# kpreid/all-is-cubes

Hardware: AMD Instinct MI355X
Metric: Mrays/s (higher is better)
Workload: dtype f64

## Files before the change

### all_is_cubes_amd/abi.py

```python
from __future__ import annotations

import ctypes as C
import math
from pathlib import Path
from typing import Optional

import numpy as np

_PKG = Path(__file__).resolve().parent
LIB_PATH = _PKG / "libaic_hip.so"

AIC_OK = 0
ERR_NAMES = {1: "AIC_ERR_INVALID", 2: "AIC_ERR_NO_DEVICE", 3: "AIC_ERR_OOM", 4: "AIC_ERR_DEVICE", 5: "AIC_ERR_UNSUPPORTED"}
LAYER_WORLD, LAYER_UI = 0, 1
MAX_IN_FLIGHT = 32
FLAW_UNSUPPORTED, FLAW_NO_BLOOM = 1, 2
FRAME_COUNTERS, FRAME_AUX, FRAME_PIXEL_CENTERS, FRAME_OUT_LINEAR, FRAME_OUT_COLORBUF, FRAME_NO_FEEDBACK = 1, 2, 4, 8, 16, 32
FRAME_BLOOM = 64
RAYS_NO_SKY, RAYS_DEVICE = 128, 256
MAX_RAYS = 2048 * 65535
TUNE_QUEUES_SHIFT, TUNE_SUPER_SHIFT, TUNE_VARIANT_SHIFT = 0, 4, 9
VARIANT_AUTO, VARIANT_PLAIN, VARIANT_EXCHANGING, VARIANT_RECORDING = 0, 1, 2, 3
LIGHT_HOOK_SESSION, LIGHT_HOOK_POOL_SHIFT = 1, 8


def bloom_geometry(width: int, height: int):
    rx, ry = (width + 1) // 2, (height + 1) // 2
    levels = min(6, min(rx, ry).bit_length())
    d = 1 << levels
    return levels, ((rx + d - 1) // d * d, (ry + d - 1) // d * d)


def tuning(queues=None, super_shift=None, variant=None) -> int:
    t = 0
    if queues is not None:
        t |= (int(queues) & 15) << TUNE_QUEUES_SHIFT
    if super_shift is not None:
        t |= ((int(super_shift) + 1) & 31) << TUNE_SUPER_SHIFT
    if variant is not None:
        t |= (int(variant) & 3) << TUNE_VARIANT_SHIFT
    return t

ABI_SYMBOLS = [
    "aic_abi_version", "aic_create", "aic_destroy", "aic_last_error", "aic_device_name", "aic_upload_space",
    "aic_clear_space", "aic_update_cubes", "aic_update_light_volume", "aic_replace_block", "aic_replace_blocks", "aic_compact", "aic_set_options",
    "aic_render", "aic_render_submit", "aic_render_wait", "aic_render_submit_batch", "aic_render_wait_batch", "aic_trace_patches", "aic_trace_rays", "aic_partition_rows", "aic_assemble_strips", "aic_assemble_strips_async", "aic_assemble_strips_on", "aic_read_aux", "aic_synchronize", "aic_stream", "aic_wait_event", "aic_stream_wait_frame",
    "aic_probe_raycast", "aic_probe_light_lut", "aic_probe_powf", "aic_probe_expf", "aic_probe_bloom",
    "aic_ortho_image_size", "aic_render_orthographic",
    "aic_evaluate_light", "aic_evaluate_light_submit", "aic_evaluate_light_wait", "aic_evaluate_light_poll", "aic_light_cubes_changed", "aic_read_light_volume", "aic_read_light_cubes", "aic_light_chart", "aic_probe_derived", "aic_probe_log2f",
    "aic_create_multi", "aic_destroy_multi", "aic_multi_device_count", "aic_multi_context", "aic_multi_last_error", "aic_multi_upload_space",
    "aic_multi_clear_space", "aic_multi_update_cubes", "aic_multi_update_light_volume", "aic_multi_evaluate_light", "aic_multi_light_cubes_changed", "aic_multi_replace_blocks", "aic_multi_set_options",
    "aic_multi_render", "aic_multi_render_submit", "aic_multi_render_wait",
]


class AicError(RuntimeError):

    def __init__(self, code: int, message: str):
        super().__init__(f"{ERR_NAMES.get(code, code)}: {message}")
        self.code = code


class BlockDesc(C.Structure):
    _fields_ = [("resolution", C.c_int32), ("vlo", C.c_int32 * 3), ("vsize", C.c_int32 * 3), ("vox_off", C.c_uint32),
                ("pal_off", C.c_uint32), ("pal_len", C.c_uint32), ("flags", C.c_uint32), ("reserved", C.c_int32)]


class LightParams(C.Structure):
    _fields_ = [("maximum_distance", C.c_int32), ("fast", C.c_int32), ("epsilon", C.c_int32), ("batch", C.c_int32),
                ("queue_order", C.c_int32), ("n_queue", C.c_int32), ("lanes_per_cube", C.c_int32), ("hooks", C.c_int32), ("queue_cubes", C.c_void_p), ("queue_priorities", C.c_void_p),
                ("max_updates", C.c_uint64)]


class LightInfo(C.Structure):
    _fields_ = [("updates", C.c_uint64), ("batches", C.c_uint64), ("cost", C.c_uint64), ("device_ms", C.c_double),
                ("total_ms", C.c_double), ("queue_left", C.c_uint32), ("pad", C.c_uint32), ("bundles_visited", C.c_uint64)]


def light_chart():
    lib = load()
    lib.aic_light_chart.restype = C.c_uint32
    lib.aic_light_chart.argtypes = [C.c_void_p, C.c_void_p, C.POINTER(C.c_uint32)]
    depth = C.c_uint32(0)
    n = lib.aic_light_chart(None, None, C.byref(depth))
    w = np.zeros((n, 6), np.float32)
    ch = np.zeros((n, 6), np.uint32)
    lib.aic_light_chart(w.ctypes.data, ch.ctypes.data, C.byref(depth))
    return w, ch, int(depth.value)


class SpaceDesc(C.Structure):
    _fields_ = [("lo", C.c_int32 * 3), ("size", C.c_int32 * 3), ("block_index", C.c_void_p), ("light", C.c_void_p),
                ("n_blocks", C.c_uint32), ("blocks", C.c_void_p), ("voxels", C.c_void_p), ("n_voxels", C.c_uint64),
                ("palette", C.c_void_p), ("n_palette", C.c_uint64), ("sky_kind", C.c_int32), ("sky", (C.c_float * 3) * 8),
                ("block_sky", (C.c_uint8 * 4) * 7)]


class Options(C.Structure):
    _fields_ = [("fog", C.c_int32), ("transparency", C.c_int32), ("threshold", C.c_float), ("lighting", C.c_int32),
                ("bounce_samples", C.c_int32), ("antialiasing", C.c_int32), ("debug_pixel_cost", C.c_int32),
                ("tone_mapping", C.c_int32), ("maximum_intensity", C.c_float), ("bloom_intensity", C.c_float),
                ("view_distance", C.c_double)]


class Camera(C.Structure):
    _fields_ = [("inverse_projection_view", C.c_double * 16), ("exposure", C.c_float), ("reserved", C.c_int32)]


class Partition(C.Structure):
    _fields_ = [("strip_rows", C.c_uint32), ("n_parts", C.c_uint32), ("part", C.c_uint32), ("reserved", C.c_uint32)]


class FrameDesc(C.Structure):
    _fields_ = [("width", C.c_uint32), ("height", C.c_uint32), ("world", Camera), ("ui", Camera), ("backdrop", C.c_float * 4),
                ("partition", Partition), ("flags", C.c_uint32), ("tuning", C.c_uint32)]


class FrameInfo(C.Structure):
    _fields_ = [("cubes_traced", C.c_uint64), ("n_outer", C.c_uint64), ("n_inner", C.c_uint64), ("n_hits", C.c_uint64),
                ("n_light", C.c_uint64), ("kernel_ms", C.c_float), ("total_ms", C.c_float), ("rows_rendered", C.c_uint32),
                ("flaws", C.c_uint32), ("variant", C.c_uint32), ("tile_queues", C.c_uint32)]


PIXEL_AUX_DTYPE = np.dtype(
    [("hit", "<i4"), ("cube", "<i4", (3,)), ("voxel", "<i4", (3,)), ("resolution", "<i4"), ("face", "<i4"),
     ("block_index", "<i4"), ("cubes_traced", "<u4"), ("layer", "<u4"), ("t_distance", "<f8")],
    align=True,
)
RC_STEP_DTYPE = np.dtype([("cube", "<i4", (3,)), ("face", "<i4"), ("t_distance", "<f8"), ("intersection_point", "<f8", (3,))], align=True)

_lib: Optional[C.CDLL] = None


def load() -> C.CDLL:
    global _lib
    if _lib is None:
        if not LIB_PATH.exists():
            raise ImportError(f"{LIB_PATH} is missing: build it with __graft_entry__.build() (hipcc, gfx950)")
        try:
            import torch
        except ImportError:
            pass
        lib = C.CDLL(str(LIB_PATH))
        lib.aic_create.restype = C.c_void_p
        lib.aic_create.argtypes = [C.c_int, C.POINTER(C.c_int)]
        lib.aic_destroy.argtypes = [C.c_void_p]
        lib.aic_destroy.restype = None
        lib.aic_last_error.restype = C.c_char_p
        lib.aic_last_error.argtypes = [C.c_void_p]
        lib.aic_stream.restype = C.c_void_p
        lib.aic_stream.argtypes = [C.c_void_p]
        lib.aic_partition_rows.restype = C.c_uint32
        lib.aic_partition_rows.argtypes = [C.c_uint32, C.POINTER(Partition)]
        lib.aic_upload_space.argtypes = [C.c_void_p, C.c_int, C.POINTER(SpaceDesc)]
        lib.aic_clear_space.argtypes = [C.c_void_p, C.c_int]
        lib.aic_compact.argtypes = [C.c_void_p, C.c_int]
        lib.aic_update_cubes.argtypes = [C.c_void_p, C.c_int, C.c_uint32, C.c_void_p, C.c_void_p, C.c_void_p]
        lib.aic_update_light_volume.argtypes = [C.c_void_p, C.c_int, C.c_void_p]
        lib.aic_replace_block.argtypes = [C.c_void_p, C.c_int, C.c_uint32, C.POINTER(BlockDesc), C.c_void_p, C.c_void_p]
        lib.aic_replace_blocks.argtypes = [C.c_void_p, C.c_int, C.c_uint32, C.c_void_p, C.c_void_p, C.c_void_p, C.c_void_p]
        lib.aic_set_options.argtypes = [C.c_void_p, C.c_int, C.POINTER(Options)]
        lib.aic_render.argtypes = [C.c_void_p, C.POINTER(FrameDesc), C.c_void_p, C.c_int, C.POINTER(FrameInfo)]
        lib.aic_render_submit.argtypes = [C.c_void_p, C.POINTER(FrameDesc), C.c_void_p, C.c_uint32]
        lib.aic_render_wait.argtypes = [C.c_void_p, C.c_uint32, C.POINTER(FrameInfo)]
        lib.aic_render_submit_batch.argtypes = [C.c_void_p, C.c_uint32, C.POINTER(FrameDesc), C.POINTER(C.c_void_p), C.c_uint32]
        lib.aic_render_wait_batch.argtypes = [C.c_void_p, C.c_uint32, C.c_uint32, C.POINTER(FrameInfo)]
        lib.aic_trace_patches.argtypes = [C.c_void_p, C.POINTER(FrameDesc), C.c_uint32, C.c_void_p, C.c_void_p, C.c_void_p, C.POINTER(FrameInfo)]
        lib.aic_trace_rays.argtypes = [C.c_void_p, C.c_int, C.c_uint32, C.c_void_p, C.c_uint32, C.c_float, C.c_void_p, C.c_void_p, C.POINTER(FrameInfo)]
        lib.aic_assemble_strips.argtypes = [C.c_void_p, C.c_void_p, C.c_void_p, C.c_uint32, C.c_uint32, C.c_uint32, C.c_uint32]
        lib.aic_assemble_strips_async.argtypes = [C.c_void_p, C.c_void_p, C.c_void_p, C.c_uint32, C.c_uint32, C.c_uint32, C.c_uint32]
        lib.aic_read_aux.argtypes = [C.c_void_p, C.c_void_p, C.c_uint64]
        lib.aic_synchronize.argtypes = [C.c_void_p]
        lib.aic_wait_event.argtypes = [C.c_void_p, C.c_void_p]
        lib.aic_stream_wait_frame.argtypes = [C.c_void_p, C.c_uint32, C.c_void_p]
        lib.aic_device_name.argtypes = [C.c_void_p, C.c_char_p, C.c_uint32]
        lib.aic_probe_raycast.argtypes = [C.c_void_p, C.c_void_p, C.c_void_p, C.c_int, C.c_void_p, C.c_void_p, C.c_int,
                                          C.c_uint32, C.c_void_p, C.POINTER(C.c_uint32), C.POINTER(C.c_int)]
        lib.aic_probe_light_lut.argtypes = [C.c_void_p, C.c_void_p]
        lib.aic_probe_powf.argtypes = [C.c_void_p, C.c_void_p, C.c_void_p, C.c_uint32, C.c_void_p]
        lib.aic_probe_expf.argtypes = [C.c_void_p, C.c_void_p, C.c_uint32, C.c_void_p]
        lib.aic_probe_bloom.argtypes = [C.c_void_p, C.c_uint32, C.c_uint32, C.c_void_p, C.c_float, C.POINTER(Options), C.c_void_p, C.c_void_p,
                                        C.POINTER(C.c_uint32 * 2)]
        lib.aic_evaluate_light.argtypes = [C.c_void_p, C.c_int, C.POINTER(LightParams), C.POINTER(LightInfo)]
        lib.aic_evaluate_light_submit.argtypes = [C.c_void_p, C.c_int, C.POINTER(LightParams)]
        lib.aic_evaluate_light_wait.argtypes = [C.c_void_p, C.c_int, C.POINTER(LightInfo)]
        lib.aic_evaluate_light_poll.argtypes = [C.c_void_p, C.c_int, C.POINTER(C.c_int)]
        lib.aic_read_light_volume.argtypes = [C.c_void_p, C.c_int, C.c_void_p]
        lib.aic_read_light_cubes.argtypes = [C.c_void_p, C.c_int, C.c_uint32, C.c_void_p, C.c_void_p]
        lib.aic_light_cubes_changed.argtypes = [C.c_void_p, C.c_int, C.c_uint32, C.c_void_p, C.c_int]
        lib.aic_probe_derived.argtypes = [C.c_void_p, C.c_int, C.c_void_p, C.c_void_p]
        lib.aic_probe_log2f.argtypes = [C.c_void_p, C.c_void_p, C.c_uint32, C.c_void_p]
        assert C.sizeof(BlockDesc) == 48
        _lib = lib
    return _lib


def packed_light_scalar_in(value: float) -> int:
    v = np.float32(value)
    if not v > 0:
        return 0
    x = float(np.float32(np.float32(np.log2(v)) * np.float32(10.0)) + np.float32(144.0))
    x = float(np.float32(x))
    r = math.floor(abs(x) + 0.5) * (1 if x >= 0 else -1)
    return int(min(max(r, 0), 255))


def block_sky_texels(sky_kind: int, sky: np.ndarray) -> np.ndarray:
    sky = np.asarray(sky, np.float32).reshape(8, 3)
    out = np.zeros((7, 4), np.uint8)
    out[:, 3] = 255

    def some(rgb):
        return [packed_light_scalar_in(float(c)) for c in rgb]

    if sky_kind == 0:
        out[:, 0:3] = some(sky[0])
        return out
    bases = {
        0: ((0, 1, 0), (0, 0, 1), (1, 0, 0)),
        1: ((0, 0, 1), (1, 0, 0), (0, 1, 0)),
        2: ((1, 0, 0), (0, 1, 0), (0, 0, 1)),
        3: ((0, -1, 0), (0, 0, 1), (-1, 0, 0)),
        4: ((0, 0, 1), (-1, 0, 0), (0, -1, 0)),
        5: ((1, 0, 0), (0, -1, 0), (0, 0, -1)),
    }
    pts = [(-1, -1, -1), (-1, 1, -1), (1, -1, -1), (1, 1, -1)]
    for f in range(6):
        bx, by, bz = (np.array(v) for v in bases[f])
        acc = np.zeros(3, np.float32)
        for p in pts:
            d = p[0] * bx + p[1] * by + p[2] * bz
            idx = ((1 if d[0] >= 0 else 0) << 2) + ((1 if d[1] >= 0 else 0) << 1) + (1 if d[2] >= 0 else 0)
            acc = (acc + sky[idx]).astype(np.float32)
        out[f, 0:3] = some(acc * np.float32(0.25))
    acc = np.zeros(3, np.float32)
    for k in range(8):
        acc = (acc + sky[k]).astype(np.float32)
    out[6, 0:3] = some(acc * np.float32(1.0 / 8.0))
    return out


def make_options(fog=1, transparency=1, threshold=0.5, lighting=3, bounce_samples=0, antialiasing=0, debug_pixel_cost=False,
                 tone_mapping=0, maximum_intensity=float("inf"), bloom_intensity=0.125, view_distance=200.0) -> Options:
    o = Options()
    o.fog, o.transparency, o.threshold, o.lighting = fog, transparency, threshold, lighting
    o.bounce_samples, o.antialiasing, o.debug_pixel_cost = bounce_samples, antialiasing, int(debug_pixel_cost)
    o.tone_mapping, o.maximum_intensity, o.bloom_intensity = tone_mapping, maximum_intensity, bloom_intensity
    o.view_distance = min(max(view_distance, 1.0), 10000.0)
    return o


def unaltered_colors(**kw) -> Options:
    base = dict(fog=0, lighting=0, transparency=1, bloom_intensity=0.0)
    base.update(kw)
    return make_options(**base)


def _ptr(a: Optional[np.ndarray]):
    return None if a is None or a.size == 0 else a.ctypes.data


class Context:

    def __init__(self, device_id: int = -1):
        self._lib = load()
        st = C.c_int(0)
        self._h = self._lib.aic_create(device_id, C.byref(st))
        if not self._h:
            raise AicError(st.value, "aic_create failed (no usable MI355X / HIP device?)")

    def close(self) -> None:
        if getattr(self, "_h", None):
            self._lib.aic_destroy(self._h)
            self._h = None

    def __del__(self):
        try:
            self.close()
        except Exception:
            pass

    def __enter__(self):
        return self

    def __exit__(self, *exc):
        self.close()

    def _check(self, rc: int) -> None:
        if rc != AIC_OK:
            raise AicError(rc, self._lib.aic_last_error(self._h).decode())

    @property
    def device_name(self) -> str:
        buf = C.create_string_buffer(256)
        self._check(self._lib.aic_device_name(self._h, buf, 256))
        return buf.value.decode()

    @property
    def stream(self) -> int:
        return int(self._lib.aic_stream(self._h) or 0)

    @staticmethod
    def _space_desc(flat_space):
        p = flat_space.pack() if hasattr(flat_space, "pack") else flat_space
# ... 29 lines not shown
        xyz = np.ascontiguousarray(xyz, np.int32).reshape(-1, 3)
        bi = None if block_index is None else np.ascontiguousarray(block_index, np.uint16)
        lt = None if light is None else np.ascontiguousarray(light, np.uint8).reshape(-1, 4)
        self._check(self._lib.aic_update_cubes(self._h, layer, len(xyz), _ptr(xyz), _ptr(bi), _ptr(lt)))

    def update_light_volume(self, layer: int, light: np.ndarray) -> None:
        lt = np.ascontiguousarray(light, np.uint8)
        self._check(self._lib.aic_update_light_volume(self._h, layer, _ptr(lt)))

    def replace_block(self, layer: int, index: int, block) -> None:
        from . import flat

        d = BlockDesc()
        d.resolution = block.resolution
        d.vlo[:] = list(block.vlo)
        d.vsize[:] = list(block.voxels.shape)
        d.pal_len = len(block.palette)
        d.flags = (flat.FLAG_ONE if block.is_one else 0) | (flat.FLAG_AIR if block.is_air else 0)
        vox = np.ascontiguousarray(block.voxels, np.uint16)
        pal = np.ascontiguousarray(block.palette, np.float32)
        self._check(self._lib.aic_replace_block(self._h, layer, index, C.byref(d), _ptr(vox), _ptr(pal)))

    def render_orthographic(self, layer: int = LAYER_WORLD, resolution: int = 32):
        f = self._lib.aic_render_orthographic
        f.argtypes = [C.c_void_p, C.c_int, C.c_int, C.c_void_p, C.c_int, C.POINTER(C.c_uint32), C.POINTER(C.c_uint32), C.c_void_p]
        w, h = C.c_uint32(0), C.c_uint32(0)
        self._check(f(self._h, layer, resolution, None, 0, C.byref(w), C.byref(h), None))
        out = np.zeros((h.value, w.value, 4), np.uint8)
        info = FrameInfo()
        self._check(f(self._h, layer, resolution, _ptr(out), 0, C.byref(w), C.byref(h), C.byref(info)))
        return {"rgba8": out, "info": info}

    def compact(self, layer: int) -> None:
        self._check(self._lib.aic_compact(self._h, C.c_int(layer)))

    def replace_blocks(self, layer: int, items) -> None:
        n = len(items)
        idx = np.ascontiguousarray([i for i, _ in items], np.uint32)
        descs = (BlockDesc * max(n, 1))()
        keep, vp, pp = [], (C.c_void_p * max(n, 1))(), (C.c_void_p * max(n, 1))()
        for k, (_, block) in enumerate(items):
            d = descs[k]
            d.resolution = block.resolution
            d.vlo[:] = list(block.vlo)
            d.vsize[:] = list(block.voxels.shape)
            d.pal_len = len(block.palette)
            d.flags = (flat.FLAG_ONE if block.is_one else 0) | (flat.FLAG_AIR if block.is_air else 0)
            vox = np.ascontiguousarray(block.voxels, np.uint16)
            pal = np.ascontiguousarray(block.palette, np.float32)
            keep += [vox, pal]
            vp[k], pp[k] = vox.ctypes.data, pal.ctypes.data
        self._check(self._lib.aic_replace_blocks(self._h, layer, n, _ptr(idx), C.cast(descs, C.c_void_p), C.cast(vp, C.c_void_p), C.cast(pp, C.c_void_p)))

    def set_options(self, layer: int, options: Options) -> None:
        self._check(self._lib.aic_set_options(self._h, layer, C.byref(options)))

    @staticmethod
    def make_frame(width, height, world_inv=None, ui_inv=None, exposure=1.0, ui_exposure=1.0, backdrop=(0, 0, 0, 0),
                   partition=None, flags=0, tuning=0) -> FrameDesc:
        f = FrameDesc()
        f.width, f.height = int(width), int(height)
        ident = np.eye(4).reshape(16)
        w = ident if world_inv is None else np.ascontiguousarray(world_inv, np.float64).reshape(16)
        u = ident if ui_inv is None else np.ascontiguousarray(ui_inv, np.float64).reshape(16)
        f.world.inverse_projection_view[:] = [float(v) for v in w]
        f.ui.inverse_projection_view[:] = [float(v) for v in u]
        f.world.exposure, f.ui.exposure = exposure, ui_exposure
        f.backdrop[:] = [float(v) for v in backdrop]
        if partition is not None:
            f.partition.strip_rows, f.partition.n_parts, f.partition.part = (int(v) for v in partition)
        f.flags = flags
        f.tuning = int(tuning)
        return f

    def partition_rows(self, height: int, partition) -> int:
        p = Partition(int(partition[0]), int(partition[1]), int(partition[2]), 0)
        return int(self._lib.aic_partition_rows(height, C.byref(p)))

    def render(self, frame: FrameDesc, want_aux: bool = False, counters: bool = False):
        keep_flags = frame.flags
        if want_aux:
            frame.flags |= FRAME_AUX
        if counters:
            frame.flags |= FRAME_COUNTERS
        rows = int(self._lib.aic_partition_rows(frame.height, C.byref(frame.partition)))
        floats = bool(frame.flags & (FRAME_OUT_LINEAR | FRAME_OUT_COLORBUF))
        out = np.zeros((rows, frame.width, 4), np.float32 if floats else np.uint8)
        info = FrameInfo()
        try:
            self._check(self._lib.aic_render(self._h, C.byref(frame), _ptr(out), 0, C.byref(info)))
        finally:
            frame.flags = keep_flags
        aux = None
        if want_aux:
            aux = np.zeros((rows, frame.width), PIXEL_AUX_DTYPE)
            if aux.size:
                self._check(self._lib.aic_read_aux(self._h, _ptr(aux), aux.size))
        return {"rgba8": out, "info": info, "aux": aux}

    def render_to_device(self, frame: FrameDesc, device_ptr: int) -> FrameInfo:
        info = FrameInfo()
        self._check(self._lib.aic_render(self._h, C.byref(frame), C.c_void_p(device_ptr), 1, C.byref(info)))
        return info

    def trace_patches(self, frame: FrameDesc, rects, want_aux: bool = False):
        r = np.ascontiguousarray(rects, np.float64).reshape(-1, 4)
        out = np.zeros((len(r), 4), np.float32 if frame.flags & (FRAME_OUT_LINEAR | FRAME_OUT_COLORBUF) else np.uint8)
        aux = np.zeros(len(r), PIXEL_AUX_DTYPE) if want_aux else None
        info = FrameInfo()
        self._check(self._lib.aic_trace_patches(self._h, C.byref(frame), len(r), _ptr(r), _ptr(out), _ptr(aux), C.byref(info)))
        return {"rgba8": out, "aux": aux, "info": info}

    def trace_rays(self, layer: int, rays, include_sky: bool = True, flags: int = 0, exposure: float = 1.0, want_aux: bool = False):
        r = np.ascontiguousarray(rays, np.float64).reshape(-1, 6)
        flags = (int(flags) & ~RAYS_DEVICE) | (0 if include_sky else RAYS_NO_SKY)
        out = np.zeros((len(r), 4), np.float32 if flags & (FRAME_OUT_LINEAR | FRAME_OUT_COLORBUF) else np.uint8)
        aux = np.zeros(len(r), PIXEL_AUX_DTYPE) if want_aux else None
        info = FrameInfo()
        self._check(self._lib.aic_trace_rays(self._h, int(layer), len(r), _ptr(r), flags, float(exposure), _ptr(out), _ptr(aux), C.byref(info)))
        return {"rgba8": out, "aux": aux, "info": info}

    def trace_rays_device(self, layer: int, n: int, rays_ptr: int, out_ptr: int, aux_ptr: int = 0, include_sky: bool = True, flags: int = 0,
                          exposure: float = 1.0) -> FrameInfo:
        flags = int(flags) | RAYS_DEVICE | (0 if include_sky else RAYS_NO_SKY)
        info = FrameInfo()
        self._check(self._lib.aic_trace_rays(self._h, int(layer), int(n), C.c_void_p(rays_ptr), flags, float(exposure), C.c_void_p(out_ptr),
                                             C.c_void_p(aux_ptr or None), C.byref(info)))
        return info

    def render_submit(self, frame: FrameDesc, device_ptr: int, slot: int) -> None:
        self._check(self._lib.aic_render_submit(self._h, C.byref(frame), C.c_void_p(device_ptr), int(slot)))

    def render_submit_batch(self, frames, device_ptrs, slot: int) -> None:
        arr = (FrameDesc * len(frames))(*frames)
        ptrs = (C.c_void_p * len(frames))(*[int(p) for p in device_ptrs])
        self._check(self._lib.aic_render_submit_batch(self._h, len(frames), arr, ptrs, slot))

    def render_wait_batch(self, slot: int, n_frames: int):
        infos = (FrameInfo * n_frames)()
        self._check(self._lib.aic_render_wait_batch(self._h, slot, n_frames, infos))
        return list(infos)

    def render_wait(self, slot: int) -> FrameInfo:
        info = FrameInfo()
        self._check(self._lib.aic_render_wait(self._h, int(slot), C.byref(info)))
        return info

    def assemble_strips(self, gathered_ptr: int, out_ptr: int, width: int, height: int, strip_rows: int, n_parts: int) -> None:
        self._check(self._lib.aic_assemble_strips(self._h, C.c_void_p(gathered_ptr), C.c_void_p(out_ptr), width, height, strip_rows, n_parts))

    def synchronize(self) -> None:
        self._check(self._lib.aic_synchronize(self._h))

    def stream_wait_frame(self, slot: int, hip_stream: int) -> None:
        self._check(self._lib.aic_stream_wait_frame(self._h, int(slot), C.c_void_p(hip_stream)))

    def wait_event(self, hip_event: int) -> None:
        self._check(self._lib.aic_wait_event(self._h, C.c_void_p(hip_event)))

    def probe_raycast(self, origin, direction, bounds=None, include_exit=True, max_steps=64):
        o = np.ascontiguousarray(origin, np.float64).reshape(3)
        d = np.ascontiguousarray(direction, np.float64).reshape(3)
        lo = np.zeros(3, np.int32) if bounds is None else np.ascontiguousarray(bounds[0], np.int32)
        hi = np.zeros(3, np.int32) if bounds is None else np.ascontiguousarray(bounds[1], np.int32)
        out = np.zeros(max_steps, RC_STEP_DTYPE)
        n = C.c_uint32(0)
        ended = C.c_int(0)
        self._check(self._lib.aic_probe_raycast(self._h, o.ctypes.data, d.ctypes.data, int(bounds is not None), lo.ctypes.data,
                                                hi.ctypes.data, int(include_exit), max_steps, out.ctypes.data, C.byref(n), C.byref(ended)))
        return out[: n.value], bool(ended.value)

    def probe_powf(self, x, y) -> np.ndarray:
        x = np.ascontiguousarray(x, np.float32)
        y = np.ascontiguousarray(y, np.float32)
        out = np.zeros(x.shape, np.float32)
        self._check(self._lib.aic_probe_powf(self._h, _ptr(x), _ptr(y), x.size, _ptr(out)))
        return out

    def probe_expf(self, x) -> np.ndarray:
        x = np.ascontiguousarray(x, np.float32)
        out = np.zeros(x.shape, np.float32)
        self._check(self._lib.aic_probe_expf(self._h, _ptr(x), x.size, _ptr(out)))
        return out

    def probe_bloom(self, colorbuf, exposure: float, options: "Options", want_mip0: bool = False):
        cb = np.ascontiguousarray(colorbuf, np.float32)
        if cb.ndim != 3 or cb.shape[2] != 4:
            raise ValueError("colorbuf must be [h][w][4]")
        h, w = cb.shape[:2]
        out = np.zeros((h, w, 4), np.uint8)
        size = (C.c_uint32 * 2)()
        t0 = bloom_geometry(w, h)[1]
        mip0 = np.zeros((t0[1], t0[0], 4), np.float16) if want_mip0 else None
        self._check(self._lib.aic_probe_bloom(self._h, w, h, _ptr(cb), float(exposure), C.byref(options), _ptr(out),
                                              _ptr(mip0) if mip0 is not None else None, C.byref(size)))
        assert (size[0], size[1]) == t0, ((size[0], size[1]), t0)
        return (out, mip0) if want_mip0 else out

    def evaluate_light(self, layer: int, maximum_distance: int, fast: bool = True, epsilon: int = 1, batch: int = 32,
                       queue_order: int = 16, queue=None, max_updates: int = 0, lanes_per_cube: int = 0, session: bool = False,
                       dep_pool_chunks: int = 0) -> LightInfo:
        hooks = (LIGHT_HOOK_SESSION if session else 0) | ((int(dep_pool_chunks) & 0xffff) << LIGHT_HOOK_POOL_SHIFT)
        p = LightParams(maximum_distance, int(fast), epsilon, batch, queue_order, -1, lanes_per_cube, hooks, None, None, max_updates)
        keep = []
        if queue is not None:
            qc = np.ascontiguousarray([q[0] for q in queue], np.int32).reshape(-1, 3)
            qp = np.ascontiguousarray([q[1] for q in queue], np.int32)
            keep = [qc, qp]
            p.n_queue = len(qp)
            p.queue_cubes = qc.ctypes.data
            p.queue_priorities = qp.ctypes.data
        info = LightInfo()
        self._check(self._lib.aic_evaluate_light(self._h, layer, C.byref(p), C.byref(info)))
        del keep
        return info

    def evaluate_light_submit(self, layer: int, maximum_distance: int, fast: bool = True, epsilon: int = 1, batch: int = 32, queue_order: int = 16,
                              queue=None, max_updates: int = 0, lanes_per_cube: int = 0) -> None:
        p = LightParams(maximum_distance, int(fast), epsilon, batch, queue_order, -1, lanes_per_cube, 0, None, None, max_updates)
        keep = []
        if queue is not None:
            qc = np.ascontiguousarray([q[0] for q in queue], np.int32).reshape(-1, 3)
            qp = np.ascontiguousarray([q[1] for q in queue], np.int32)
            keep = [qc, qp]
            p.n_queue = len(qp)
            p.queue_cubes = qc.ctypes.data
            p.queue_priorities = qp.ctypes.data
        self._check(self._lib.aic_evaluate_light_submit(self._h, layer, C.byref(p)))
        del keep

    def evaluate_light_done(self, layer: int) -> bool:
        d = C.c_int(1)
        self._check(self._lib.aic_evaluate_light_poll(self._h, layer, C.byref(d)))
        return bool(d.value)

    def evaluate_light_wait(self, layer: int) -> LightInfo:
        info = LightInfo()
        self._check(self._lib.aic_evaluate_light_wait(self._h, layer, C.byref(info)))
        return info

    def light_cubes_changed(self, layer: int, xyz, queue_order: int = 16) -> None:
        xyz = np.ascontiguousarray(xyz, np.int32).reshape(-1, 3)
        self._check(self._lib.aic_light_cubes_changed(self._h, layer, len(xyz), _ptr(xyz), queue_order))

    def read_light_volume(self, layer: int, shape) -> np.ndarray:
        out = np.zeros(tuple(shape) + (4,), np.uint8)
        self._check(self._lib.aic_read_light_volume(self._h, layer, out.ctypes.data))
        return out

    def read_light_cubes(self, layer: int, xyz) -> np.ndarray:
        xyz = np.ascontiguousarray(xyz, np.int32).reshape(-1, 3)
        out = np.zeros((len(xyz), 4), np.uint8)
        self._check(self._lib.aic_read_light_cubes(self._h, layer, len(xyz), _ptr(xyz), out.ctypes.data))
        return out

    def probe_derived(self, layer: int, n_blocks: int):
        out = np.zeros((n_blocks, 32), np.float32)
        opq = np.zeros((n_blocks, 6), np.uint8)
        self._check(self._lib.aic_probe_derived(self._h, layer, out.ctypes.data, opq.ctypes.data))
        return out, opq

    def probe_log2f(self, x) -> np.ndarray:
        x = np.ascontiguousarray(x, np.float32)
        out = np.zeros(x.shape, np.float32)
        self._check(self._lib.aic_probe_log2f(self._h, _ptr(x), x.size, _ptr(out)))
        return out

    def probe_light_lut(self) -> np.ndarray:
        out = np.zeros(256, np.float32)
        self._check(self._lib.aic_probe_light_lut(self._h, out.ctypes.data))
        return out


class MultiContext:

    def __init__(self, device_ids):
        self._lib = load()
        lib = self._lib
        lib.aic_create_multi.restype = C.c_void_p
        lib.aic_create_multi.argtypes = [C.c_int, C.c_void_p, C.POINTER(C.c_int)]
        lib.aic_destroy_multi.argtypes = [C.c_void_p]
        lib.aic_multi_last_error.restype = C.c_char_p
        lib.aic_multi_last_error.argtypes = [C.c_void_p]
        lib.aic_multi_device_count.argtypes = [C.c_void_p]
        lib.aic_multi_upload_space.argtypes = [C.c_void_p, C.c_int, C.c_void_p]
        lib.aic_multi_clear_space.argtypes = [C.c_void_p, C.c_int]
        lib.aic_multi_set_options.argtypes = [C.c_void_p, C.c_int, C.c_void_p]
        lib.aic_multi_update_light_volume.argtypes = [C.c_void_p, C.c_int, C.c_void_p]
        lib.aic_multi_evaluate_light.argtypes = [C.c_void_p, C.c_int, C.POINTER(LightParams), C.POINTER(LightInfo)]
        lib.aic_multi_light_cubes_changed.argtypes = [C.c_void_p, C.c_int, C.c_uint32, C.c_void_p, C.c_int]
        lib.aic_multi_update_cubes.argtypes = [C.c_void_p, C.c_int, C.c_uint32, C.c_void_p, C.c_void_p, C.c_void_p]
        lib.aic_multi_render.argtypes = [C.c_void_p, C.c_void_p, C.c_void_p, C.c_int, C.c_void_p]
        lib.aic_multi_render_submit.argtypes = [C.c_void_p, C.c_void_p, C.c_void_p, C.c_int, C.c_uint32]
        lib.aic_multi_render_wait.argtypes = [C.c_void_p, C.c_uint32, C.c_void_p]
        ids = np.ascontiguousarray(device_ids, np.int32)
        st = C.c_int(0)
        self._h = lib.aic_create_multi(len(ids), _ptr(ids), C.byref(st))
        if not self._h:
            raise AicError(st.value, "aic_create_multi failed (no usable MI355X?)")

    def close(self) -> None:
        if self._h:
            self._lib.aic_destroy_multi(self._h)
            self._h = None

    def __enter__(self):
# ... 59 lines not shown
```

### all_is_cubes_amd/csrc/aic_abi.cpp

```cpp

#include <hip/hip_runtime.h>

#include <chrono>
#include <cmath>
#include <condition_variable>
#include <mutex>
#include <thread>
#include <cstdio>
#include <cstdlib>
#include <cstring>
#include <initializer_list>
#include <string>
#include <utility>
#include <vector>

#include "../../include/aic_hip.h"
#include "aic_bloom.h"
#include "aic_ctx.h"
#include "aic_device.h"

namespace aic {
void launch_trace_image(const DevFrame &F, bool diag, hipStream_t stream);
size_t trace_ray_cold_bytes(uint32_t n_cus, uint32_t *groups);
void launch_scatter_cubes(uint16_t *grid, uint32_t *light, const int32_t *xyz, const uint16_t *bi, const uint32_t *lt,
                          uint32_t n, const int lo[3], const int size[3], const uint32_t *cls, hipStream_t stream);
void launch_probe_powf(const float *x, const float *y, float *out, uint32_t n, hipStream_t stream);
void launch_probe_expf(const float *x, float *out, uint32_t n, hipStream_t stream);
void launch_order_tiles(const uint32_t *cost, uint32_t *order, uint32_t n_tiles, uint32_t macros_x, uint32_t sb_shift, uint32_t n_queues, uint32_t *queue_start,
                        hipStream_t stream, bool clear_cost = false, uint32_t *clear_words = nullptr, uint32_t n_clear_words = 0);
void launch_order_tiles_jobs(const OrderJobs &jobs, uint32_t n_jobs, uint32_t n_tiles, uint32_t macros_x, uint32_t sb_shift, uint32_t n_queues, hipStream_t stream,
                             bool clear_cost, uint32_t n_clear_words);
void launch_tag_cubes(uint16_t *grid, size_t n, const uint32_t *cls, int from_tagged, int to_tagged, hipStream_t stream);
void launch_assemble_strips(const uint32_t *gathered, uint32_t *out, uint32_t w, uint32_t h, uint32_t strip_rows,
                            uint32_t n_parts, uint32_t max_rows, hipStream_t stream);
void launch_probe_raycast(const double *od, int use_bounds, const int *lohi, int include_exit, uint32_t max_steps,
                          double *out_rec, uint32_t *n_out, int *ended, hipStream_t stream);
}

using namespace aic;

static_assert(sizeof(aic_pixel_aux) == sizeof(DevAux), "aux record layout");

static_assert(sizeof(aic_block_desc) == 48, "aic_block_desc is 48 bytes");

namespace {

constexpr uint64_t kMaxPoolElems = 0x7ffffff0ull;
constexpr uint64_t kMaxLightTexels = 0x3ffffff0ull;

aic_options default_options() {
    aic_options o;
    std::memset(&o, 0, sizeof(o));
    o.fog = 1;
    o.transparency = 1;
    o.threshold = 0.5f;
    o.lighting = 3;
    o.maximum_intensity = INFINITY;
    o.bloom_intensity = 0.125f;
    o.view_distance = 200.0;
    return o;
}

enum DumpTag : uint32_t { DUMP_UPLOAD = 1, DUMP_CLEAR = 2, DUMP_CUBES = 3, DUMP_LIGHT = 4, DUMP_BLOCK = 5, DUMP_OPTIONS = 6, DUMP_FRAME = 7 };
struct DumpPart { const void *p; size_t n; };
void dump_record(aic_ctx *c, uint32_t tag, uint32_t layer, std::initializer_list<DumpPart> parts) {
    if (!c || !c->dump) return;
    uint64_t total = 0;
    for (const DumpPart &d : parts) total += d.p ? d.n : 0;
    std::fwrite(&tag, 4, 1, c->dump);
    std::fwrite(&layer, 4, 1, c->dump);
    std::fwrite(&total, 8, 1, c->dump);
    for (const DumpPart &d : parts)
        if (d.p && d.n) std::fwrite(d.p, 1, d.n, c->dump);
    std::fflush(c->dump);
}

}

namespace aic {

thread_local std::string *tl_err_sink = nullptr;
int fail(aic_ctx *c, int code, const char *what, hipError_t e) {
    if (c) {
        std::string &dst = tl_err_sink ? *tl_err_sink : c->err;
        dst = what;
        if (e != hipSuccess) {
            dst += ": ";
            dst += hipGetErrorString(e);
        }
    }
    return code;
}

int hip_fail(aic_ctx *c, const char *what, hipError_t e) {
    return fail(c, e == hipErrorOutOfMemory ? AIC_ERR_OOM : AIC_ERR_DEVICE, what, e);
}

int take_light_spare(aic_ctx *c, Layer &l, int layer, size_t n, int *index) {
    auto in_use = [&](const DevBuf<uint32_t> &b) {
        for (uint32_t i = 0; i < AIC_MAX_IN_FLIGHT; i++)
            if (c->slots[i].busy && b.p && c->slots[i].light_used[layer] == (const void *)b.p) return true;
        return false;
    };
    int pick = -1;
    for (int k = 0; k < Layer::kLightSpares && pick < 0; k++)
        if (l.light_spare[k].p && l.light_spare[k].cap >= n && !in_use(l.light_spare[k])) pick = k;
    for (int k = 0; k < Layer::kLightSpares && pick < 0; k++)
        if (!l.light_spare[k].p || (l.light_spare[k].cap < n && !in_use(l.light_spare[k]))) pick = k;
    if (pick < 0) {
        pick = 0;
        for (uint32_t i = 0; i < AIC_MAX_IN_FLIGHT; i++)
            if (c->slots[i].busy && c->slots[i].light_used[layer] == (const void *)l.light_spare[0].p) {
                const hipError_t e = hipStreamSynchronize(c->slots[i].stream);
                if (e != hipSuccess) return fail(c, AIC_ERR_DEVICE, "waiting for a frame that reads a spare light volume", e);
            }
    }
    const hipError_t e = l.light_spare[pick].ensure(n);
    if (e != hipSuccess) return fail(c, e == hipErrorOutOfMemory ? AIC_ERR_OOM : AIC_ERR_DEVICE, "alloc light (spare volume)", e);
    *index = pick;
    return AIC_OK;
}

int quiesce(aic_ctx *c) {
    { const int rc = light_job_finish(c); if (rc != AIC_OK) return rc; }
    for (uint32_t i = 0; i < AIC_MAX_IN_FLIGHT; i++)
        if (c->slots[i].busy) HIP_TRY(c, hipStreamSynchronize(c->slots[i].stream));
    return AIC_OK;
}

}

namespace {

bool valid_resolution(int r) { return r >= 1 && r <= 128 && (r & (r - 1)) == 0; }

inline uint32_t block_class(const DevBlock &b) { return (b.kind & 255u) ? 2u : ((b.kind & 0x80000000u) ? 0u : 1u); }
inline void set_class(std::vector<uint32_t> &cls, uint32_t index, uint32_t c2) {
    if (cls.size() <= index / 16u) cls.resize(index / 16u + 1u, 0u);
    cls[index / 16u] = (cls[index / 16u] & ~(3u << ((index & 15u) * 2u))) | (c2 << ((index & 15u) * 2u));
}

inline bool invisible(const float *e) { return e[3] == 0.f && e[4] == 0.f && e[5] == 0.f && e[6] == 0.f; }

int convert_block(aic_ctx *c, const aic_block_desc &d, const uint16_t *voxels, const float *palette, uint32_t vox_off,
                  uint32_t pal_off, DevBlock *out, std::vector<uint16_t> *vox_out, std::vector<DevPaletteEntry> *pal_out) {
    std::memset(out, 0, sizeof(*out));
    if (!valid_resolution(d.resolution)) return fail(c, AIC_ERR_INVALID, "block resolution must be a power of two in 1..128");
    const bool one = (d.flags & AIC_BLOCK_ONE) != 0;
    size_t nvox = one ? 1 : (size_t)d.vsize[0] * (size_t)d.vsize[1] * (size_t)d.vsize[2];
    for (int a = 0; a < 3 && !one; a++) {
        if (d.vsize[a] < 0 || d.vlo[a] < 0 || d.vlo[a] + d.vsize[a] > d.resolution)
            return fail(c, AIC_ERR_INVALID, "block voxel bounds exceed GridAab::for_block(resolution)");
    }
    if (d.pal_len == 0 && nvox > 0) return fail(c, AIC_ERR_INVALID, "block has voxels but an empty palette");
    if (!palette && (one || d.pal_len > 0)) return fail(c, AIC_ERR_INVALID, "block has a palette length but no palette");
    if (!voxels && !one && nvox > 0) return fail(c, AIC_ERR_INVALID, "block has a voxel volume but no voxels");
    for (uint32_t i = 0; i < (one ? 1u : d.pal_len) && palette; i++) {
        const float *e = palette + 8 * (size_t)i;
        for (int k = 0; k < 7; k++)
            if (!(e[k] >= 0.f)) return fail(c, AIC_ERR_INVALID, "palette entry has a negative or NaN component");
        if (!(e[3] <= 1.f)) return fail(c, AIC_ERR_INVALID, "palette entry has alpha above 1");
    }
    if (one || d.resolution == 1) {
        const float *e = nullptr;
        static const float air[8] = {0, 0, 0, 0, 0, 0, 0, 0};
        if (one) e = palette;
        else {
            bool inb = nvox > 0 && d.vlo[0] <= 0 && d.vlo[1] <= 0 && d.vlo[2] <= 0 && d.vlo[0] + d.vsize[0] > 0 &&
                       d.vlo[1] + d.vsize[1] > 0 && d.vlo[2] + d.vsize[2] > 0;
            if (inb) {
                size_t i = ((size_t)(0 - d.vlo[0]) * d.vsize[1] + (size_t)(0 - d.vlo[1])) * d.vsize[2] + (size_t)(0 - d.vlo[2]);
                uint16_t idx = voxels[i];
                if (idx >= d.pal_len) return fail(c, AIC_ERR_INVALID, "voxel index exceeds palette");
                e = palette + 8 * (size_t)idx;
            } else e = air;
        }
        out->kind = invisible(e) ? 0x80000000u : 0u;
        for (int k = 0; k < 4; k++) out->color[k] = e[k] + 0.0f;
        for (int k = 0; k < 3; k++) out->emission[k] = e[4 + k] + 0.0f;
        return AIC_OK;
    }
    std::vector<uint32_t> remap(d.pal_len);
    uint32_t n_inv = 0;
    for (uint32_t i = 0; i < d.pal_len; i++)
        if (invisible(palette + 8 * (size_t)i)) n_inv++;
    uint32_t next_inv = 0, next_vis = n_inv;
    size_t pal_base = pal_out->size();
    pal_out->resize(pal_base + d.pal_len);
    for (uint32_t i = 0; i < d.pal_len; i++) {
        const float *e = palette + 8 * (size_t)i;
        uint32_t dst = invisible(e) ? next_inv++ : next_vis++;
        remap[i] = dst;
        DevPaletteEntry &pe = (*pal_out)[pal_base + dst];
        for (int k = 0; k < 4; k++) pe.color[k] = e[k] + 0.0f;
        for (int k = 0; k < 3; k++) pe.emission[k] = e[4 + k] + 0.0f;
        pe.pad = 0.f;
    }
    size_t vox_base = vox_out->size();
    vox_out->resize(vox_base + nvox);
    for (size_t i = 0; i < nvox; i++) {
        uint16_t idx = voxels[i];
        if (idx >= d.pal_len) return fail(c, AIC_ERR_INVALID, "voxel index exceeds palette");
        (*vox_out)[vox_base + i] = (uint16_t)remap[idx];
    }
    out->kind = (uint32_t)d.resolution;
    out->vlo_packed = (uint32_t)d.vlo[0] | ((uint32_t)d.vlo[1] << 8) | ((uint32_t)d.vlo[2] << 16);
    out->vsize_packed = (uint32_t)d.vsize[0] | ((uint32_t)d.vsize[1] << 8) | ((uint32_t)d.vsize[2] << 16);
    out->vox_off = vox_off;
    out->pal_off = pal_off;
    out->n_invisible = n_inv;
    return AIC_OK;
}

void fill_dev_layer(const aic_ctx *c, const Layer &l, const aic_camera &cam, DevLayer *d, uint32_t *flaws) {
    std::memset(d, 0, sizeof(*d));
    d->present = l.present ? 1 : 0;
    d->pool = l.pool.p;
    d->cls = l.cls.p;
    d->n_blocks = (uint32_t)l.host_blocks.size();
    d->light = l.light.p;
    d->blocks = l.blocks.p;
    d->palette = l.palette.p;
    for (int a = 0; a < 3; a++) { d->lo[a] = l.lo[a]; d->size[a] = l.size[a]; }
    d->air_index = l.air_index;
    d->sky_kind = l.sky_kind;
    std::memcpy(d->sky, l.sky, sizeof(d->sky));
    std::memcpy(d->block_sky, l.block_sky, sizeof(d->block_sky));
    const aic_options o = l.opt_set ? l.opt : default_options();
    d->opt.fog = o.fog;
    d->opt.transparency = o.transparency;
    d->opt.threshold = o.threshold;
    d->opt.lighting = o.lighting;
    d->opt.bounce_samples = o.bounce_samples;
    d->opt.antialiasing = o.antialiasing;
    d->opt.debug_pixel_cost = o.debug_pixel_cost;
    d->opt.tone_mapping = o.tone_mapping;
    d->opt.maximum_intensity = o.maximum_intensity;
    d->opt.view_distance = o.view_distance;
    std::memcpy(d->inv, cam.inverse_projection_view, sizeof(d->inv));
    d->exposure = cam.exposure + 0.0f;
    d->cls_in_code = l.cls_in_code ? 1u : 0u;
    (void)c;
}

}

extern "C" {

int aic_abi_version(void) { return AIC_ABI_VERSION; }

aic_ctx *aic_create(int device_id, int *status) {
    int st_dummy;
    if (!status) status = &st_dummy;
    int n = 0;
    hipError_t e = hipGetDeviceCount(&n);
    if (e != hipSuccess || n <= 0) {
        *status = AIC_ERR_NO_DEVICE;
        return nullptr;
    }
    if (device_id < 0) {
        if (hipGetDevice(&device_id) != hipSuccess) device_id = 0;
    }
    if (device_id >= n) {
        *status = AIC_ERR_INVALID;
        return nullptr;
    }
    if (hipSetDevice(device_id) != hipSuccess) {
        *status = AIC_ERR_DEVICE;
        return nullptr;
    }
    aic_ctx *c = new aic_ctx();
    c->device = device_id;
    hipDeviceProp_t prop;
    if (hipGetDeviceProperties(&prop, device_id) == hipSuccess) c->n_cus = prop.multiProcessorCount > 0 ? (uint32_t)prop.multiProcessorCount : 256u;
    if (hipGetDeviceProperties(&prop, device_id) == hipSuccess) std::snprintf(c->devname, sizeof(c->devname), "%s (%s)", prop.name, prop.gcnArchName);
    {
        auto env_int = [](const char *name, int dflt) { const char *e = std::getenv(name); return e ? std::atoi(e) : dflt; };
        c->sw.tile = env_int("AIC_TILE", 0);
        c->sw.macro = env_int("AIC_MACRO", 0);
        c->sw.feedback = env_int("AIC_TILE_FEEDBACK", 1) != 0;
        c->sw.wait_whole_stream = env_int("AIC_WAIT_WHOLE_STREAM", 0) != 0;
        c->sw.tiles_per_wave = (uint32_t)std::max(0, env_int("AIC_TILES_PER_WAVE", 0));
        if (const char *p = std::getenv("AIC_WAVE_PROF")) c->sw.wave_prof = p;
    }
    if (const char *path = std::getenv("AIC_DUMP")) {
        static int n_dumps = 0;
        std::string pth = path;
        if (n_dumps > 0) pth += "." + std::to_string(n_dumps);
        n_dumps++;
        c->dump = std::fopen(pth.c_str(), "wb");
        if (c->dump) std::fwrite("AICDUMP1", 1, 8, c->dump);
    }
    bool ok = hipStreamCreateWithFlags(&c->stream, hipStreamNonBlocking) == hipSuccess;
    for (uint32_t i = 0; ok && i < 8u && i < AIC_MAX_IN_FLIGHT; i++) {
        aic_ctx::FrameSlot &fs = c->slots[i];
        if (i == 0) fs.stream = c->stream;
        else ok = hipStreamCreateWithFlags(&fs.stream, hipStreamNonBlocking) == hipSuccess;
        ok = ok && hipEventCreate(&fs.ev0) == hipSuccess && hipEventCreate(&fs.ev1) == hipSuccess && hipEventCreate(&fs.ev2) == hipSuccess && fs.sub[0].counters.ensure(1) == hipSuccess;
    }
    ok = ok && hipStreamCreateWithFlags(&c->upload_stream, hipStreamNonBlocking) == hipSuccess;
    float lut[256];
    lut[0] = 0.f;
    for (int v = 1; v < 256; v++) {
        float arg = ((float)v - 144.0f) / 10.0f;
        lut[v] = (float)std::exp2((double)arg);
    }
    ok = ok && c->lut.ensure(256) == hipSuccess && hipMemcpy(c->lut.p, lut, sizeof(lut), hipMemcpyHostToDevice) == hipSuccess;
    {
        auto enc = [](float cc) -> int {
            float v = cc <= 0.0031308f ? cc * (323.f / 25.f) : (211.f * std::pow(cc, 5.f / 12.f) - 11.f) / 200.f;
            float r = std::round(v * 255.f);
            if (!(r > 0.f)) return 0;
            return r >= 255.f ? 255 : (int)r;
        };
        float thr[256];
        thr[0] = 0.f;
        for (int k = 1; k < 256; k++) {
            uint32_t lo_b = 0u, hi_b = 0x40000000u;
            while (hi_b - lo_b > 1u) {
                const uint32_t mid = lo_b + (hi_b - lo_b) / 2u;
                float f;
                std::memcpy(&f, &mid, 4);
                if (enc(f) >= k) hi_b = mid; else lo_b = mid;
            }
            for (int back = 0; back < 8 && hi_b > 1u; back++) {
                uint32_t probe = hi_b - 1u;
                float f;
                std::memcpy(&f, &probe, 4);
                bool lower_found = false;
                for (uint32_t d = 0; d < 8u && probe > d; d++) {
                    const uint32_t q = probe - d;
                    std::memcpy(&f, &q, 4);
                    if (enc(f) >= k) { hi_b = q; lower_found = true; }
                }
                if (!lower_found) break;
            }
            std::memcpy(&thr[k], &hi_b, 4);
        }
        ok = ok && c->srgb_thr.ensure(256) == hipSuccess && hipMemcpy(c->srgb_thr.p, thr, sizeof(thr), hipMemcpyHostToDevice) == hipSuccess;
    }
    if (!ok) {
        *status = AIC_ERR_DEVICE;
        aic_destroy(c);
        return nullptr;
    }
    for (auto &l : c->layers) l.opt = default_options();
    *status = AIC_OK;
    return c;
}

void aic_destroy(aic_ctx *c) {
    if (!c) return;
    (void)hipSetDevice(c->device);
    (void)light_job_finish(c);
    if (c->ljob.worker.joinable()) {
        { std::lock_guard<std::mutex> lk(c->ljob.mu); c->ljob.quit = true; }
        c->ljob.cv.notify_all();
        c->ljob.worker.join();
    }
    if (c->stream) (void)hipStreamSynchronize(c->stream);
    for (uint32_t i = 0; i < AIC_MAX_IN_FLIGHT; i++) {
        aic_ctx::FrameSlot &fs = c->slots[i];
        if (fs.stream) (void)hipStreamSynchronize(fs.stream);
        for (auto &sb : fs.sub) sb.release();
        fs.ray_cold.release(); fs.edges.release();
        if (fs.ev0) (void)hipEventDestroy(fs.ev0);
        if (fs.ev1) (void)hipEventDestroy(fs.ev1);
        if (fs.ev2) (void)hipEventDestroy(fs.ev2);
        fs.tile_static.release(); fs.queue_static.release();
        if (i > 0 && fs.stream) (void)hipStreamDestroy(fs.stream);
    }
    for (auto &l : c->layers) l.release();
    c->lut.release(); c->srgb_thr.release(); c->out.release(); c->aux.release(); c->staging.release(); c->ortho_views.release();
    if (c->dump) std::fclose(c->dump);
    if (c->upload_stream) (void)hipStreamDestroy(c->upload_stream);
    if (c->stream) (void)hipStreamDestroy(c->stream);
    delete c;
}

const char *aic_last_error(const aic_ctx *c) { return c ? c->err.c_str() : "no context"; }

int aic_device_name(const aic_ctx *c, char *buf, uint32_t buf_len) {
    if (!c || !buf || !buf_len) return AIC_ERR_INVALID;
    std::snprintf(buf, buf_len, "%s", c->devname);
    return AIC_OK;
}

int aic_upload_space(aic_ctx *c, int layer, const aic_space_desc *s) {
    if (!c || !s || !valid_layer(layer)) return fail(c, AIC_ERR_INVALID, "aic_upload_space: bad argument");
    HIP_TRY(c, hipSetDevice(c->device));
    { int qrc = quiesce(c); if (qrc != AIC_OK) return qrc; }
    for (int a = 0; a < 3; a++)
        if (s->size[a] < 0 || (int64_t)s->lo[a] + s->size[a] > 2147483647LL) return fail(c, AIC_ERR_INVALID, "space bounds out of range");
    Layer &l = c->layers[layer];
    const size_t n = (size_t)s->size[0] * (size_t)s->size[1] * (size_t)s->size[2];
    if (n && (!s->block_index || !s->light)) return fail(c, AIC_ERR_INVALID, "space has cubes but no block_index/light");
    if (s->n_blocks > 65536) return fail(c, AIC_ERR_INVALID, "more than 65536 blocks");
    if (n + s->n_voxels > kMaxPoolElems) return fail(c, AIC_ERR_INVALID, "space too large (cube grid + voxel pool must stay within 4 GiB)");
    if (n > kMaxLightTexels) return fail(c, AIC_ERR_INVALID, "space too large (the light volume, 4 bytes per cube, must stay within 4 GiB)");
    if (s->n_blocks && !s->blocks) return fail(c, AIC_ERR_INVALID, "blocks is null");
    for (int o = 0; o < 8; o++)
        for (int k = 0; k < 3; k++)
            if (!(s->sky[o][k] >= 0.f)) return fail(c, AIC_ERR_INVALID, "sky colour has a negative or NaN component");

    std::vector<DevBlock> blocks(s->n_blocks);
    std::vector<uint32_t> vox_cap(s->n_blocks, 0u), pal_cap(s->n_blocks, 0u), vox_base(s->n_blocks, 0u), pal_base(s->n_blocks, 0u);
    std::vector<uint16_t> vox;
    std::vector<DevPaletteEntry> pal;
    vox.reserve((size_t)s->n_voxels);
    pal.reserve((size_t)s->n_palette);
    int32_t air_index = -1;
    for (uint32_t i = 0; i < s->n_blocks; i++) {
        const aic_block_desc &d = s->blocks[i];
        const bool one = (d.flags & AIC_BLOCK_ONE) != 0;
        size_t nvox = one ? 1 : (size_t)(d.vsize[0] > 0 ? d.vsize[0] : 0) * (size_t)(d.vsize[1] > 0 ? d.vsize[1] : 0) * (size_t)(d.vsize[2] > 0 ? d.vsize[2] : 0);
        if ((uint64_t)d.vox_off + nvox > s->n_voxels || (uint64_t)d.pal_off + d.pal_len > s->n_palette)
            return fail(c, AIC_ERR_INVALID, "block voxel/palette range exceeds the pools");
        if (n + vox.size() + nvox > kMaxPoolElems || pal.size() + d.pal_len > 0xfffffff0ull) return fail(c, AIC_ERR_INVALID, "pool too large");
        const size_t vb = vox.size(), pb = pal.size();
        int rc = convert_block(c, d, s->voxels ? s->voxels + d.vox_off : nullptr, s->palette ? s->palette + 8 * (size_t)d.pal_off : nullptr,
                               (uint32_t)(n + vox.size()), (uint32_t)pal.size(), &blocks[i], &vox, &pal);
        if (rc != AIC_OK) return rc;
        vox_cap[i] = (uint32_t)(vox.size() - vb);
        pal_cap[i] = (uint32_t)(pal.size() - pb);
        vox_base[i] = (uint32_t)(n + vb);
        pal_base[i] = (uint32_t)pb;
        if ((d.flags & AIC_BLOCK_AIR) && air_index < 0) air_index = (int32_t)i;
    }
    for (size_t i = 0; i < n; i++)
        if (s->block_index[i] >= s->n_blocks) return fail(c, AIC_ERR_INVALID, "cube block index out of range");

    hipError_t e;
    std::vector<uint32_t> cls;
    for (uint32_t i = 0; i < s->n_blocks; i++) set_class(cls, i, block_class(blocks[i]));
    if (cls.empty()) cls.push_back(0u);
    if ((e = l.pool.ensure(n + vox.size())) != hipSuccess) return hip_fail(c, "alloc pool", e);
    if ((e = l.cls.ensure(cls.size())) != hipSuccess) return hip_fail(c, "alloc classes", e);
    if ((e = l.light.ensure(n)) != hipSuccess) return hip_fail(c, "alloc light", e);
    if ((e = l.blocks.ensure(blocks.size())) != hipSuccess) return hip_fail(c, "alloc blocks", e);
    if ((e = l.palette.ensure(pal.size())) != hipSuccess) return hip_fail(c, "alloc palette", e);
    if (n) {
        HIP_TRY(c, hipMemcpyAsync(l.pool.p, s->block_index, n * sizeof(uint16_t), hipMemcpyHostToDevice, c->stream));
        HIP_TRY(c, hipMemcpyAsync(l.light.p, s->light, n * 4, hipMemcpyHostToDevice, c->stream));
    }
    if (!blocks.empty()) HIP_TRY(c, hipMemcpyAsync(l.blocks.p, blocks.data(), blocks.size() * sizeof(DevBlock), hipMemcpyHostToDevice, c->stream));
    if (!vox.empty()) HIP_TRY(c, hipMemcpyAsync(l.pool.p + n, vox.data(), vox.size() * sizeof(uint16_t), hipMemcpyHostToDevice, c->stream));
    HIP_TRY(c, hipMemcpyAsync(l.cls.p, cls.data(), cls.size() * sizeof(uint32_t), hipMemcpyHostToDevice, c->stream));
    const bool cls_in_code = s->n_blocks <= kCubeIndexMask + 1u;
    if (cls_in_code) launch_tag_cubes(l.pool.p, n, l.cls.p, 0, 1, c->stream);
    if (!pal.empty()) HIP_TRY(c, hipMemcpyAsync(l.palette.p, pal.data(), pal.size() * sizeof(DevPaletteEntry), hipMemcpyHostToDevice, c->stream));
    HIP_TRY(c, hipStreamSynchronize(c->stream));

    for (int a = 0; a < 3; a++) { l.lo[a] = s->lo[a]; l.size[a] = s->size[a]; }
    l.host_blocks.swap(blocks);
    l.host_cls.swap(cls);
    l.vox_cap.swap(vox_cap);
    l.pal_cap.swap(pal_cap);
    l.vox_base.swap(vox_base);
    l.pal_base.swap(pal_base);
    l.garbage_vox = l.garbage_pal = 0;
    l.air_index = air_index;
    l.sky_kind = s->sky_kind;
    for (int o = 0; o < 8; o++)
        for (int k = 0; k < 3; k++) l.sky[o][k] = s->sky[o][k] + 0.0f;
    for (int f = 0; f < 7; f++)
        l.block_sky[f] = (uint32_t)s->block_sky[f][0] | ((uint32_t)s->block_sky[f][1] << 8) | ((uint32_t)s->block_sky[f][2] << 16) |
                         ((uint32_t)s->block_sky[f][3] << 24);
    l.cls_in_code = cls_in_code;
    l.present = true;
    l.version++;
    l.upload_serial++;
    if (c->dump) {
        struct { int32_t lo[3], size[3]; uint32_t n_blocks; int32_t sky_kind; uint64_t n_voxels, n_palette; float sky[8][3]; uint8_t block_sky[7][4]; } h;
        std::memset(&h, 0, sizeof(h));
        for (int a = 0; a < 3; a++) { h.lo[a] = s->lo[a]; h.size[a] = s->size[a]; }
        h.n_blocks = s->n_blocks; h.sky_kind = s->sky_kind; h.n_voxels = s->n_voxels; h.n_palette = s->n_palette;
        std::memcpy(h.sky, s->sky, sizeof(h.sky));
        std::memcpy(h.block_sky, s->block_sky, sizeof(h.block_sky));
        dump_record(c, DUMP_UPLOAD, (uint32_t)layer,
                    {{&h, sizeof(h)}, {s->block_index, n * 2}, {s->light, n * 4}, {s->blocks, (size_t)s->n_blocks * sizeof(aic_block_desc)},
                     {s->voxels, (size_t)s->n_voxels * 2}, {s->palette, (size_t)s->n_palette * 32}});
    }
    return AIC_OK;
}

int aic_clear_space(aic_ctx *c, int layer) {
    if (!c || !valid_layer(layer)) return fail(c, AIC_ERR_INVALID, "aic_clear_space: bad argument");
    { int qrc = quiesce(c); if (qrc != AIC_OK) return qrc; }
    c->layers[layer].present = false;
    dump_record(c, DUMP_CLEAR, (uint32_t)layer, {});
    return AIC_OK;
}

int aic_update_cubes(aic_ctx *c, int layer, uint32_t n, const int32_t *xyz, const uint16_t *block_index, const uint8_t *light) {
    if (!c || !valid_layer(layer) || (n && !xyz)) return fail(c, AIC_ERR_INVALID, "aic_update_cubes: bad argument");
    Layer &l = c->layers[layer];
    if (!l.present) return fail(c, AIC_ERR_INVALID, "aic_update_cubes: no space uploaded for this layer");
    if (!n) return AIC_OK;
    HIP_TRY(c, hipSetDevice(c->device));
    { int qrc = quiesce(c); if (qrc != AIC_OK) return qrc; }
    if (block_index)
        for (uint32_t i = 0; i < n; i++)
            if (block_index[i] >= l.host_blocks.size()) return fail(c, AIC_ERR_INVALID, "cube block index out of range");
    const size_t b_xyz = (size_t)n * 12, b_bi = block_index ? (((size_t)n * 2 + 15) & ~(size_t)15) : 0, b_lt = light ? (size_t)n * 4 : 0;
    hipError_t e = c->staging.ensure(b_xyz + b_bi + b_lt + 64);
    if (e != hipSuccess) return hip_fail(c, "alloc staging", e);
    unsigned char *base = c->staging.p;
    HIP_TRY(c, hipMemcpyAsync(base, xyz, b_xyz, hipMemcpyHostToDevice, c->stream));
    if (block_index) HIP_TRY(c, hipMemcpyAsync(base + b_xyz, block_index, (size_t)n * 2, hipMemcpyHostToDevice, c->stream));
    if (light) HIP_TRY(c, hipMemcpyAsync(base + b_xyz + b_bi, light, b_lt, hipMemcpyHostToDevice, c->stream));
    l.version++;
    light_state_cubes_updated(l.lstate, l.version - 1, l.version, n, xyz, block_index, light);
    launch_scatter_cubes(l.pool.p, l.light.p, (const int32_t *)base, block_index ? (const uint16_t *)(base + b_xyz) : nullptr,
                         light ? (const uint32_t *)(base + b_xyz + b_bi) : nullptr, n, l.lo, l.size, l.cls_in_code ? l.cls.p : nullptr, c->stream);
    HIP_TRY(c, hipGetLastError());
    HIP_TRY(c, hipStreamSynchronize(c->stream));
    {
        const uint32_t h[4] = {n, block_index ? 1u : 0u, light ? 1u : 0u, 0u};
        dump_record(c, DUMP_CUBES, (uint32_t)layer, {{h, sizeof(h)}, {xyz, (size_t)n * 12}, {block_index, (size_t)n * 2}, {light, (size_t)n * 4}});
    }
    return AIC_OK;
}

int aic_update_light_volume(aic_ctx *c, int layer, const uint8_t *light) {
// ... 85 lines not shown
    if (fits) {
        vox_off = l.vox_base[index];
        pal_off = l.pal_base[index];
    } else {
        vox_off = (uint32_t)l.pool.n;
        pal_off = (uint32_t)l.palette.n;
        if ((uint64_t)vox_off + vox.size() > kMaxPoolElems || (uint64_t)pal_off + pal.size() > 0xfffffff0ull)
            return fail(c, AIC_ERR_INVALID, "voxel pool too large");
        if (!vox.empty() && (e = l.pool.ensure(vox_off + vox.size(), true, c->stream)) != hipSuccess) return hip_fail(c, "grow pool", e);
        if (!pal.empty() && (e = l.palette.ensure(pal_off + pal.size(), true, c->stream)) != hipSuccess) return hip_fail(c, "grow palette", e);
        if (exists) { l.garbage_vox += l.vox_cap[index]; l.garbage_pal += l.pal_cap[index]; }
    }
    if (!vox.empty()) {
        db.vox_off = vox_off;
        HIP_TRY(c, hipMemcpy(l.pool.p + vox_off, vox.data(), vox.size() * sizeof(uint16_t), hipMemcpyHostToDevice));
    }
    if (!pal.empty()) {
        db.pal_off = pal_off;
        HIP_TRY(c, hipMemcpy(l.palette.p + pal_off, pal.data(), pal.size() * sizeof(DevPaletteEntry), hipMemcpyHostToDevice));
    }
    bool class_changed = false;
    if (!exists) {
        l.host_blocks.push_back(db);
        l.vox_cap.push_back((uint32_t)vox.size());
        l.pal_cap.push_back((uint32_t)pal.size());
        l.vox_base.push_back(vox_off);
        l.pal_base.push_back(pal_off);
        if ((e = l.blocks.ensure(l.host_blocks.size(), true, c->stream)) != hipSuccess) return hip_fail(c, "grow blocks", e);
    } else {
        class_changed = block_class(l.host_blocks[index]) != block_class(db);
        l.host_blocks[index] = db;
        if (!fits) {
            l.vox_cap[index] = (uint32_t)vox.size(); l.pal_cap[index] = (uint32_t)pal.size();
            l.vox_base[index] = vox_off; l.pal_base[index] = pal_off;
        }
    }
    HIP_TRY(c, hipMemcpy(l.blocks.p + index, &db, sizeof(db), hipMemcpyHostToDevice));
    set_class(l.host_cls, index, block_class(db));
    if ((e = l.cls.ensure(l.host_cls.size(), true, c->stream)) != hipSuccess) return hip_fail(c, "grow classes", e);
    HIP_TRY(c, hipMemcpy(l.cls.p + index / 16u, &l.host_cls[index / 16u], sizeof(uint32_t), hipMemcpyHostToDevice));
    if (l.cls_in_code) {
        if (l.host_blocks.size() > kCubeIndexMask + 1u) {
            launch_tag_cubes(l.pool.p, l.n_cubes(), l.cls.p, 1, 0, c->stream);
            l.cls_in_code = false;
        } else if (class_changed) {
            launch_tag_cubes(l.pool.p, l.n_cubes(), l.cls.p, 1, 1, c->stream);
        }
        HIP_TRY(c, hipGetLastError());
    }
    if (desc->flags & AIC_BLOCK_AIR) {
        if (l.air_index < 0) l.air_index = (int32_t)index;
    } else if (l.air_index == (int32_t)index) {
        l.air_index = -1;
    }
    {
        const bool one = (desc->flags & AIC_BLOCK_ONE) != 0;
        const uint64_t nvox = one ? 0 : (uint64_t)(desc->vsize[0] > 0 ? desc->vsize[0] : 0) * (uint64_t)(desc->vsize[1] > 0 ? desc->vsize[1] : 0) * (uint64_t)(desc->vsize[2] > 0 ? desc->vsize[2] : 0);
        const uint64_t h[2] = {index, nvox};
        dump_record(c, DUMP_BLOCK, (uint32_t)layer, {{h, sizeof(h)}, {desc, sizeof(*desc)}, {voxels, (size_t)nvox * 2}, {palette, (size_t)desc->pal_len * 32}});
    }
    return AIC_OK;
}

}

int aic_replace_blocks(aic_ctx *c, int layer, uint32_t n, const uint32_t *indices, const aic_block_desc *descs, const uint16_t *const *voxels,
                       const float *const *palettes) {
    if (!c || !valid_layer(layer) || (n && (!indices || !descs || !voxels || !palettes))) return fail(c, AIC_ERR_INVALID, "aic_replace_blocks: bad argument");
    Layer &l = c->layers[layer];
    if (!l.present) return fail(c, AIC_ERR_INVALID, "aic_replace_block: no space uploaded for this layer");
    HIP_TRY(c, hipSetDevice(c->device));
    { int qrc = quiesce(c); if (qrc != AIC_OK) return qrc; }
    int rc = AIC_OK;
    for (uint32_t k = 0; k < n && rc == AIC_OK; k++) rc = replace_one(c, layer, l, indices[k], &descs[k], voxels[k], palettes[k]);
    HIP_TRY(c, hipStreamSynchronize(c->stream));
    if (rc != AIC_OK) return rc;
    const bool big_vox = l.garbage_vox * 4 > l.pool.n && l.garbage_vox > (1u << 17);
    const bool big_pal = l.garbage_pal * 4 > l.palette.n && l.garbage_pal > (1u << 13);
    if (big_vox || big_pal) return compact_pools(c, l);
    return AIC_OK;
}

int aic_compact(aic_ctx *c, int layer) {
    if (!c || !valid_layer(layer)) return fail(c, AIC_ERR_INVALID, "aic_compact: bad argument");
    Layer &l = c->layers[layer];
    if (!l.present) return AIC_OK;
    HIP_TRY(c, hipSetDevice(c->device));
    { int qrc = quiesce(c); if (qrc != AIC_OK) return qrc; }
    return compact_pools(c, l);
}

int aic_replace_block(aic_ctx *c, int layer, uint32_t index, const aic_block_desc *desc, const uint16_t *voxels, const float *palette) {
    if (!desc) return fail(c, AIC_ERR_INVALID, "aic_replace_block: bad argument");
    return aic_replace_blocks(c, layer, 1u, &index, desc, &voxels, &palette);
}

int aic_set_options(aic_ctx *c, int layer, const aic_options *o) {
    if (!c || !valid_layer(layer) || !o) return fail(c, AIC_ERR_INVALID, "aic_set_options: bad argument");
    if (o->fog < 0 || o->fog > 3 || o->transparency < 0 || o->transparency > 2 || o->lighting < 0 || o->lighting > 5 ||
        o->antialiasing < 0 || o->antialiasing > 2 || o->tone_mapping < 0 || o->tone_mapping > 1 || !(o->view_distance > 0.0))
        return fail(c, AIC_ERR_INVALID, "aic_set_options: enum or view_distance out of range");
    c->layers[layer].opt = *o;
    c->layers[layer].opt_set = true;
    dump_record(c, DUMP_OPTIONS, (uint32_t)layer, {{o, sizeof(*o)}});
    return AIC_OK;
}

uint32_t aic_partition_rows(uint32_t height, const aic_partition *p) {
    if (!p || p->n_parts <= 1 || p->strip_rows == 0) return height;
    if (p->part >= p->n_parts) return 0;
    uint32_t rows = 0;
    const uint32_t n_strips = (height + p->strip_rows - 1) / p->strip_rows;
    for (uint32_t s = p->part; s < n_strips; s += p->n_parts) {
        uint32_t r0 = s * p->strip_rows;
        uint32_t r1 = r0 + p->strip_rows;
        if (r1 > height) r1 = height;
        rows += r1 - r0;
    }
    return rows;
}

namespace {

bool cameras_close(const double a[16], const double b[16]) {
    auto unproject = [](const double m[16], double x, double y, double z, double out[3]) {
        const double w = x * m[3] + y * m[7] + z * m[11] + m[15];
        for (int k = 0; k < 3; k++) out[k] = (x * m[k] + y * m[4 + k] + z * m[8 + k] + m[12 + k]) / w;
    };
    static const double pts[3][2] = {{0.0, 0.0}, {1.0, 1.0}, {-1.0, -1.0}};
    for (const auto &p : pts) {
        double na[3], fa[3], nb[3], fb[3];
        unproject(a, p[0], p[1], 0.0, na); unproject(a, p[0], p[1], 1.0, fa);
        unproject(b, p[0], p[1], 0.0, nb); unproject(b, p[0], p[1], 1.0, fb);
        double da[3], db[3], la = 0, lb = 0, dot = 0, move = 0;
        for (int k = 0; k < 3; k++) {
            da[k] = fa[k] - na[k]; db[k] = fb[k] - nb[k];
            la += da[k] * da[k]; lb += db[k] * db[k]; dot += da[k] * db[k];
            move += (na[k] - nb[k]) * (na[k] - nb[k]);
        }
        if (!(la > 0) || !(lb > 0)) return false;
        if (!(dot / std::sqrt(la * lb) >= 0.99985)) return false;
        if (!(move <= 0.0625)) return false;
    }
    return true;
}

struct RayBatch {
    const double *rays;
    uint32_t n;
    bool no_sky;
    uint32_t layer;
    DevAux *aux_target;
};
int submit_frames(aic_ctx *c, uint32_t k, const aic_frame_desc *frames, uint32_t *const *out_devices, uint32_t slot, bool allow_aux, const double *patches = nullptr,
                  uint32_t n_patches = 0, const DevOrthoView *ortho = nullptr, int32_t ortho_n = 0, const RayBatch *rb = nullptr) {
    if (rb) n_patches = rb->n;
    aic_ctx::FrameSlot &fs = c->slots[slot];
    const aic_frame_desc *f = &frames[0];
    fs.t_begin = std::chrono::steady_clock::now();
    fs.n_sub = k;
    aic_partition part = f->partition;
    if (part.n_parts <= 1 || part.strip_rows == 0) {
        part.n_parts = 1;
        part.part = 0;
        part.strip_rows = f->height ? f->height : 1;
    }
    if (part.part >= part.n_parts) return fail(c, AIC_ERR_INVALID, "aic_render: partition.part >= n_parts");
    if (f->flags & AIC_FRAME_BLOOM) {
        if (f->flags & (AIC_FRAME_OUT_LINEAR | AIC_FRAME_OUT_COLORBUF)) return fail(c, AIC_ERR_INVALID, "aic_render: AIC_FRAME_BLOOM is for RGBA8 output only");
        if (part.n_parts > 1u) return fail(c, AIC_ERR_UNSUPPORTED, "aic_render: AIC_FRAME_BLOOM needs the whole frame (partition.n_parts = 1)");
        if (patches || ortho_n || rb) return fail(c, AIC_ERR_UNSUPPORTED, "AIC_FRAME_BLOOM: not for patches, rays or orthographic views");
    }
    const uint32_t local_rows = aic_partition_rows(f->height, &part);
    const size_t npix = (size_t)f->width * local_rows;
    for (uint32_t j = 0; j < k; j++)
        if (npix && !out_devices[j]) return fail(c, AIC_ERR_INVALID, "aic_render: output buffer is null");
    if (!patches && !rb)
        for (uint32_t j = 0; j < k; j++) dump_record(c, DUMP_FRAME, slot, {{&frames[j], sizeof(frames[j])}});
    if (f->width > 65535u || local_rows > 65535u) return fail(c, AIC_ERR_INVALID, "aic_render: frame dimensions above 65535 are not supported");
    for (uint32_t j = 0; j < k; j++)
        if (!(frames[j].world.exposure >= 0.f) || !(frames[j].ui.exposure >= 0.f)) return fail(c, AIC_ERR_INVALID, "aic_render: exposure is negative or NaN");

    uint32_t flaws = 0;
    DevFrame F;
    std::memset(&F, 0, sizeof(F));
    DevLayer hl[2];
    fill_dev_layer(c, c->layers[AIC_LAYER_WORLD], f->world, &hl[0], &flaws);
    fill_dev_layer(c, c->layers[AIC_LAYER_UI], f->ui, &hl[1], &flaws);
    const aic_options &bloom_opt = c->layers[AIC_LAYER_WORLD].opt;
    const bool bloom = (f->flags & AIC_FRAME_BLOOM) && bloom_opt.bloom_intensity > 0.0f;
    if (bloom_opt.bloom_intensity != 0.0f && !bloom) flaws |= AIC_FLAW_NO_BLOOM;
    F.width = f->width;
    F.height = f->height;
    F.n_sub = k;
    F.pixel_centers = (f->flags & AIC_FRAME_PIXEL_CENTERS) && !patches ? 1 : 0;
    F.out_mode = (f->flags & AIC_FRAME_OUT_LINEAR) ? 1 : ((f->flags & AIC_FRAME_OUT_COLORBUF) || bloom ? 2 : 0);
    F.patches = patches;
    F.n_patches = n_patches;
    F.ortho = ortho;
    F.ortho_n = ortho_n;
    F.rays = rb ? rb->rays : nullptr;
    F.bare_trace = (ortho_n || rb) ? 1 : 0;
    if (rb) hl[1].present = 0;
    if (ortho_n) {
        hl[1].present = 0;
        DevOptions &o = hl[0].opt;
        o.fog = 0; o.transparency = 1; o.lighting = 0; o.antialiasing = 0; o.debug_pixel_cost = 0; o.tone_mapping = 0;
        o.maximum_intensity = INFINITY; o.view_distance = 200.0;
        hl[0].exposure = 1.0f;
        flaws = 0;
    }
    F.antialias = (hl[0].opt.antialiasing == 2 && !F.pixel_centers && !rb) ? 1 : 0;
    F.maximum_intensity = hl[0].opt.maximum_intensity;
    F.tone_mapping = hl[0].opt.tone_mapping;
    F.strip_rows = part.strip_rows;
    F.n_parts = part.n_parts;
    F.part = part.part;
    F.local_rows = local_rows;
    {
        const int forced = c->sw.tile;
        F.tile = (forced == 8 || forced == 16) ? (uint32_t)forced : 8u;
        F.tiles_x = (f->width + F.tile - 1) / F.tile;
        F.tiles_y = (local_rows + F.tile - 1) / F.tile;
        const int macro_env = c->sw.macro;
        F.macro = (macro_env == 1 || macro_env == 2 || macro_env == 4 || macro_env == 8 || macro_env == 16) ? (uint32_t)macro_env : 2u;
        F.macros_x = (F.tiles_x + F.macro - 1) / F.macro;
        F.macros_y = (F.tiles_y + F.macro - 1) / F.macro;
    }
    F.light_lut = c->lut.p;
    F.n_cus = c->n_cus;
    F.tiles_per_wave = c->sw.tiles_per_wave ? c->sw.tiles_per_wave : (c->streaming_submit ? 4u : 1u);
    if (!c->sw.tiles_per_wave && c->streaming_submit && k == 1u) {
        uint32_t busy_others = 0;
        for (uint32_t i = 0; i < AIC_MAX_IN_FLIGHT; i++) busy_others += (i != slot && c->slots[i].busy) ? 1u : 0u;
        const uint32_t resident_waves = (uint32_t)c->n_cus * 16u;
        const uint32_t tpw_full = (F.tiles_x * F.tiles_y + resident_waves - 1u) / resident_waves;
        if (tpw_full >= 4u && busy_others > 0u) {
            const uint32_t t = tpw_full * (busy_others < 4u ? busy_others : 4u);
            F.tiles_per_wave = t < 32u ? t : (tpw_full > 32u ? tpw_full : 32u);
        }
    }
    F.srgb_thr = c->srgb_thr.p;

    const bool want_aux = allow_aux && (f->flags & AIC_FRAME_AUX) != 0;
    const bool diag = want_aux || (f->flags & AIC_FRAME_COUNTERS) != 0;
    fs.diag = diag;
    fs.flaws = flaws;
    fs.light_used[0] = hl[0].light;
    fs.light_used[1] = hl[1].light;
    fs.local_rows = local_rows;
    fs.npix = npix;
    fs.variant = fs.tile_queues = 0;
    if (allow_aux) c->aux_records = 0;
    if (!npix) return AIC_OK;
    hipError_t e;
    if (want_aux) {
        if (rb && rb->aux_target) {
            F.aux = rb->aux_target;
        } else {
            if ((e = c->aux.ensure(npix)) != hipSuccess) return hip_fail(c, "alloc aux", e);
            F.aux = c->aux.p;
        }
    }
    const bool ui = hl[1].present != 0;
    const uint32_t n_tiles = F.macros_x * F.macros_y;
    const int queues_env = (int)((f->tuning >> AIC_TUNE_QUEUES_SHIFT) & 15u);
    const int super_env = (int)((f->tuning >> AIC_TUNE_SUPER_SHIFT) & 31u) - 1;
    uint32_t n_queues = queues_env > 0 ? (uint32_t)queues_env : (uint32_t)c->n_cus / 32u;
    if (n_queues > kMaxTileQueues) n_queues = kMaxTileQueues;
    if (n_queues < 2u || patches || rb || ortho_n || !n_tiles) n_queues = 0u;
    const uint32_t macro_log2 = F.macro >= 16 ? 4u : (F.macro >= 8 ? 3u : (F.macro >= 4 ? 2u : (F.macro >= 2 ? 1u : 0u)));
    const uint32_t tile_log2 = F.tile >= 16 ? 4u : 3u;
    uint32_t sb_px_log2 = 0;
    while ((2u << sb_px_log2) <= std::max(1u, local_rows / 8u)) sb_px_log2++;
    const uint32_t sb_shift = super_env >= 0 ? (uint32_t)std::min(super_env, 12) : (sb_px_log2 > macro_log2 + tile_log2 ? sb_px_log2 - macro_log2 - tile_log2 : 0u);
    const bool use_feedback = c->sw.feedback && n_tiles && !patches && !rb && !ortho_n && !(f->flags & AIC_FRAME_NO_FEEDBACK);
    const uint32_t sig[4] = {f->width, local_rows, (part.n_parts << 16) | part.part, (part.strip_rows << 8) | (F.macro << 4) | (F.tile >> 3)};
    uint32_t order_key[6] = {sig[0], sig[1], sig[2], sig[3], n_queues, sb_shift};
    const bool ordered = use_feedback || n_queues;
    F.n_queues = ordered ? n_queues : 0u;
    if (ordered && n_queues) {
        bool any_static = false;
        for (uint32_t j = 0; j < k; j++) {
            aic_ctx::SubSlot &sb = fs.sub[j];
            const bool same = use_feedback && sb.record_ready && std::memcmp(order_key, sb.order_key, sizeof(order_key)) == 0 && sb.tile_order.n >= n_tiles &&
                              cameras_close(frames[j].world.inverse_projection_view, sb.cost_cam);
            any_static = any_static || !same;
        }
        if (any_static && (!fs.static_ready || std::memcmp(order_key, fs.static_key, sizeof(order_key)) != 0 || fs.tile_static.n < n_tiles)) {
            fs.static_ready = false;
            if ((e = fs.tile_static.ensure(n_tiles)) != hipSuccess || (e = fs.queue_static.ensure(kMaxTileQueues + 1)) != hipSuccess) return hip_fail(c, "alloc tile queues", e);
            launch_order_tiles(nullptr, fs.tile_static.p, n_tiles, F.macros_x, sb_shift, n_queues, fs.queue_static.p, fs.stream);
            HIP_TRY(c, hipGetLastError());
            std::memcpy(fs.static_key, order_key, sizeof(order_key));
            fs.static_ready = true;
        }
    }
    for (uint32_t j = 0; j < k; j++) {
        aic_ctx::SubSlot &sb = fs.sub[j];
        DevSub &S = F.sub[j];
        std::memcpy(S.backdrop, frames[j].backdrop, sizeof(S.backdrop));
        S.has_backdrop = !(frames[j].backdrop[0] == 0.f && frames[j].backdrop[1] == 0.f && frames[j].backdrop[2] == 0.f && frames[j].backdrop[3] == 0.f);
        S.exposure = ortho_n ? 1.0f : frames[j].world.exposure + 0.0f;
        S.out = out_devices[j];
        if (bloom) {
            if ((e = sb.bloom_cb.ensure(npix)) != hipSuccess || (e = sb.bloom_mips.ensure(bloom_geometry(f->width, f->height).texels)) != hipSuccess)
                return hip_fail(c, "alloc bloom scratch", e);
            S.out = reinterpret_cast<uint32_t *>(sb.bloom_cb.p);
        }
        if ((e = sb.counters.ensure(1)) != hipSuccess) return hip_fail(c, "alloc frame counters", e);
        S.counters = sb.counters.p;
        if (!sb.host_counters) {
            HIP_TRY(c, hipHostMalloc((void **)&sb.host_counters, sizeof(DevCounters), hipHostMallocDefault));
            std::memset(sb.host_counters, 0, sizeof(DevCounters));
        }
        if (!sb.counters_clean) HIP_TRY(c, hipMemsetAsync(sb.counters.p, 0, sizeof(DevCounters), fs.stream));
        sb.counters_clean = false;
        if (ordered) {
            bool same = use_feedback && sb.record_ready && std::memcmp(order_key, sb.order_key, sizeof(order_key)) == 0 && sb.tile_order.n >= n_tiles;
            if (same) {
                same = cameras_close(frames[j].world.inverse_projection_view, sb.cost_cam);
            }
            if (same) {
                S.tile_order = sb.tile_order.p;
                S.queue_start = n_queues ? sb.queue_start.p : nullptr;
            } else if (n_queues) {
                S.tile_order = fs.tile_static.p;
                S.queue_start = fs.queue_static.p;
            }
            if (use_feedback) {
                const uint32_t *const before = sb.tile_cost.p;
                if ((e = sb.tile_cost.ensure(n_tiles)) != hipSuccess) return hip_fail(c, "alloc tile feedback", e);
                if (sb.tile_cost.p != before) sb.cost_clean_n = 0;
                if (sb.cost_clean_n < n_tiles) HIP_TRY(c, hipMemsetAsync(sb.tile_cost.p, 0, (size_t)n_tiles * sizeof(uint32_t), fs.stream));
                sb.cost_clean_n = 0;
                S.tile_cost = sb.tile_cost.p;
                std::memcpy(sb.cost_sig, sig, sizeof(sig));
            }
        }
        if (ui) {
            const size_t samples = F.antialias ? 4 : 1;
            if ((e = sb.acc.ensure(samples * npix)) != hipSuccess) return hip_fail(c, "alloc accumulators", e);
            S.acc_buf = sb.acc.p;
        }
    }
    if (!patches && !rb && !ortho_n) {
        if (fs.edges_w != f->width || fs.edges_h != f->height || !fs.edges.p) {
            std::vector<double> host((size_t)f->width + 1 + (size_t)f->height + 1);
            for (uint32_t x = 0; x <= f->width; x++) host[x] = ((double)x) / (double)f->width * 2.0 - 1.0;
            for (uint32_t y = 0; y <= f->height; y++) host[(size_t)f->width + 1 + y] = -(((double)y) / (double)f->height * 2.0 - 1.0);
            fs.edges_w = fs.edges_h = 0;
            if ((e = fs.edges.ensure(host.size())) != hipSuccess) return hip_fail(c, "alloc pixel edges", e);
            HIP_TRY(c, hipMemcpyAsync(fs.edges.p, host.data(), host.size() * sizeof(double), hipMemcpyHostToDevice, fs.stream));
            HIP_TRY(c, hipStreamSynchronize(fs.stream));
            fs.edges_w = f->width; fs.edges_h = f->height;
        }
        F.edge_x = fs.edges.p;
        F.edge_y = fs.edges.p + (size_t)f->width + 1;
    }
    if (!diag) {
        uint32_t groups = 0;
        const size_t bytes = trace_ray_cold_bytes(c->n_cus, &groups);
        if (bytes) {
            const uint32_t asked = (f->tuning >> AIC_TUNE_VARIANT_SHIFT) & 3u;
            const double resident_waves = (double)c->n_cus * 16.0 / (double)k;
            const double need = c->streaming_submit ? 1.9 : 5.0;
            F.exchange = asked == AIC_VARIANT_EXCHANGING ? 1u : (asked == AIC_VARIANT_PLAIN ? 0u : (((double)F.tiles_x * (double)F.tiles_y >= need * resident_waves) ? 1u : 0u));
            if (F.exchange && F.antialias) {
                if ((e = fs.ray_cold.ensure(bytes / sizeof(uint4))) != hipSuccess) return hip_fail(c, "alloc ray state", e);
                F.ray_cold = fs.ray_cold.p;
                F.ray_cold_groups = groups;
            }
        }
    }
    HIP_TRY(c, hipEventRecord(fs.ev0, fs.stream));
    if (ui) {
        F.pass = 1;
        F.hit_layer = 1u;
        F.use_init = 0;
        F.layer = hl[1];
        F.layer_transparency = hl[1].opt.transparency;
        F.layer_lighting = hl[1].opt.lighting;
        DevSub keep[kMaxSub];
        std::memcpy(keep, F.sub, sizeof(keep));
        const uint32_t queues_keep = F.n_queues;
        for (uint32_t j = 0; j < k; j++) {
            std::memcpy(F.sub[j].inv, frames[j].ui.inverse_projection_view, sizeof(F.sub[j].inv));
            F.sub[j].tile_order = nullptr;
            F.sub[j].tile_cost = nullptr;
            F.sub[j].queue_start = nullptr;
            F.sub[j].host_counters = nullptr;
        }
        F.n_queues = 0u;
        launch_trace_image(F, diag, fs.stream);
        std::memcpy(F.sub, keep, sizeof(keep));
        F.n_queues = queues_keep;
        for (uint32_t j = 0; j < k; j++) HIP_TRY(c, hipMemsetAsync(&fs.sub[j].counters.p->tile_next, 0, sizeof(uint32_t), fs.stream));
        F.use_init = 1;
    }
    F.pass = (rb && rb->no_sky) ? 2 : 0;
    F.hit_layer = rb ? rb->layer : 0u;
    for (uint32_t j = 0; j < k; j++) {
        std::memcpy(F.sub[j].inv, ortho_n ? hl[0].inv : frames[j].world.inverse_projection_view, sizeof(F.sub[j].inv));
#ifndef AIC_PROFILE
        F.sub[j].host_counters = reinterpret_cast<unsigned long long *>(fs.sub[j].host_counters);
#endif
    }
    F.layer = hl[0];
    F.layer_transparency = hl[0].opt.transparency;
    F.layer_lighting = hl[0].opt.lighting;
    fs.variant = diag ? AIC_VARIANT_RECORDING : ((F.exchange && hl[0].opt.lighting != 5 && (F.ray_cold || !F.antialias)) ? AIC_VARIANT_EXCHANGING : AIC_VARIANT_PLAIN);
    fs.tile_queues = F.n_queues;
    launch_trace_image(F, diag, fs.stream);
    HIP_TRY(c, hipGetLastError());
    if (bloom) {
        const BloomGeom geom = bloom_geometry(f->width, f->height);
        for (uint32_t j = 0; j < k; j++) {
            BloomParams bp;
            bp.colorbuf = fs.sub[j].bloom_cb.p;
            bp.mips = fs.sub[j].bloom_mips.p;
            bp.out = out_devices[j];
            bp.exposure = F.sub[j].exposure;
            bp.intensity = bloom_opt.bloom_intensity;
            bp.tone_mapping = F.tone_mapping;
            bp.maximum_intensity = F.maximum_intensity;
            bp.srgb_thr = c->srgb_thr.p;
            launch_bloom(geom, bp, fs.stream);
        }
        HIP_TRY(c, hipGetLastError());
    }
    HIP_TRY(c, hipEventRecord(fs.ev1, fs.stream));
#ifdef AIC_PROFILE
    for (uint32_t j = 0; j < k; j++) HIP_TRY(c, hipMemcpyAsync(fs.sub[j].host_counters, fs.sub[j].counters.p, sizeof(DevCounters), hipMemcpyDeviceToHost, fs.stream));
#endif
    HIP_TRY(c, hipEventRecord(fs.ev2, fs.stream));
    fs.busy = true;
    bool cleared = false;
    if (use_feedback && n_tiles) {
        OrderJobs jobs;
        std::memset(&jobs, 0, sizeof(jobs));
        bool ok = true;
        for (uint32_t j = 0; j < k; j++) {
            aic_ctx::SubSlot &sb = fs.sub[j];
            sb.record_ready = false;
            sb.cost_clean_n = 0;
            ok = ok && sb.tile_order.ensure(n_tiles) == hipSuccess && sb.queue_start.ensure(kMaxTileQueues + 1) == hipSuccess;
            jobs.cost[j] = sb.tile_cost.p; jobs.order[j] = sb.tile_order.p; jobs.queue_start[j] = sb.queue_start.p;
            jobs.clear_words[j] = reinterpret_cast<uint32_t *>(sb.counters.p);
        }
        if (ok) {
            launch_order_tiles_jobs(jobs, k, n_tiles, F.macros_x, sb_shift, n_queues ? n_queues : 1u, fs.stream, true, (uint32_t)(sizeof(DevCounters) / 4));
            if (hipGetLastError() == hipSuccess) {
                cleared = true;
                for (uint32_t j = 0; j < k; j++) {
                    aic_ctx::SubSlot &sb = fs.sub[j];
                    sb.cost_clean_n = n_tiles;
                    std::memcpy(sb.order_key, order_key, sizeof(order_key));
                    std::memcpy(sb.cost_cam, frames[j].world.inverse_projection_view, sizeof(sb.cost_cam));
                    sb.record_ready = true;
                }
            }
        }
    }
    if (!cleared) {
        cleared = true;
        for (uint32_t j = 0; j < k; j++) cleared = (hipMemsetAsync(fs.sub[j].counters.p, 0, sizeof(DevCounters), fs.stream) == hipSuccess) && cleared;
    }
    for (uint32_t j = 0; j < k; j++) fs.sub[j].counters_clean = cleared;
    if (want_aux && !(rb && rb->aux_target)) c->aux_records = npix;
    return AIC_OK;
}
int submit_frame(aic_ctx *c, const aic_frame_desc *f, uint32_t *out_device, uint32_t slot, bool allow_aux, const double *patches = nullptr,
                 uint32_t n_patches = 0, const DevOrthoView *ortho = nullptr, int32_t ortho_n = 0) {
    uint32_t *const outs[1] = {out_device};
    return submit_frames(c, 1, f, outs, slot, allow_aux, patches, n_patches, ortho, ortho_n);
}

int wait_frame(aic_ctx *c, uint32_t slot, aic_frame_info *info, bool whole_stream = false, aic_frame_info *infos = nullptr, uint32_t n_infos = 0) {
    aic_ctx::FrameSlot &fs = c->slots[slot];
    if (info) std::memset(info, 0, sizeof(*info));
    for (uint32_t j = 0; infos && j < n_infos; j++) std::memset(&infos[j], 0, sizeof(infos[j]));
    float kernel_ms = 0.f;
    const uint32_t k = fs.n_sub ? fs.n_sub : 1u;
    if (fs.busy) {
        fs.busy = false;
        if (whole_stream || c->sw.wait_whole_stream) HIP_TRY(c, hipStreamSynchronize(fs.stream));
        else HIP_TRY(c, hipEventSynchronize(fs.ev2));
        HIP_TRY(c, hipEventElapsedTime(&kernel_ms, fs.ev0, fs.ev1));
        for (uint32_t j = 0; j < k; j++) {
            DevCounters hc;
            std::memcpy(&hc, fs.sub[j].host_counters, sizeof(hc));
            if (hc.bailed) return fail(c, AIC_ERR_DEVICE, "trace kernel: a wave gave up waiting for rays in transit between waves; the frame has unwritten pixels");
            if (info) {
                info->cubes_traced += hc.cubes_traced;
                info->n_outer += hc.n_outer;
                info->n_inner += hc.n_inner;
                info->n_hits += hc.n_hits;
                info->n_light += hc.n_light;
            }
            if (infos && j < n_infos) {
                infos[j].cubes_traced = hc.cubes_traced; infos[j].n_outer = hc.n_outer; infos[j].n_inner = hc.n_inner;
                infos[j].n_hits = hc.n_hits; infos[j].n_light = hc.n_light;
            }
#ifdef AIC_PROFILE
            { static const char *names[40] = {"max_lifetime","max_until_dry","cyc_until_dry","cyc_lifetime","shade_ph","shade_ln","enter_ph","enter_ln","ray_ph","ray_ln","step_iters","step_lanes","cyc_step","cyc_shade_rest","cyc_enter","cyc_newray","cyc_finish","cyc_refill","cyc_shade_light","cyc_sched","fast_iters","fast_lanes","trips","trip_lanes","pass_hl_lanes","pass_fast_eligible","leave_blocks","leave_lanes","apply_blocks","apply_lanes","pass_needed_lanes","xchg_rounds","xchg_lanes","cyc_xchg","xchg_picked","xchg_parked","idle_spins","xchg_claims_lost","xchg_empty","-"};
              if (!fs.diag) for (int i = 0; i < 39; i++) std::fprintf(stderr, "PROF %s %llu\n", names[i], hc.prof[i]);
              if (const char *path = (fs.diag || c->sw.wave_prof.empty()) ? nullptr : c->sw.wave_prof.c_str()) {
                  if (FILE *fp = std::fopen(path, "w")) {
                      for (int w = 0; w < 2048; w++) std::fprintf(fp, "%u %u %u %u\n", hc.wave_prof[w][0], hc.wave_prof[w][1], hc.wave_prof[w][2], hc.wave_prof[w][3]);
                      std::fclose(fp);
                  }
              } }
#endif
        }
    }
    const float total_ms = std::chrono::duration<float, std::milli>(std::chrono::steady_clock::now() - fs.t_begin).count();
    auto fill = [&](aic_frame_info *o) {
        o->kernel_ms = kernel_ms;
        o->rows_rendered = fs.local_rows;
        o->flaws = fs.flaws;
        o->variant = fs.npix ? fs.variant : 0u;
        o->tile_queues = fs.npix ? fs.tile_queues : 0u;
        o->total_ms = total_ms;
    };
    if (info) fill(info);
    for (uint32_t j = 0; infos && j < n_infos && j < k; j++) fill(&infos[j]);
    return AIC_OK;
}

}

int aic_render(aic_ctx *c, const aic_frame_desc *f, void *out_rgba8, int out_is_device, aic_frame_info *info) {
    if (!c || !f) return fail(c, AIC_ERR_INVALID, "aic_render: bad argument");
    if (info) std::memset(info, 0, sizeof(*info));
    HIP_TRY(c, hipSetDevice(c->device));
    if (c->slots[0].busy) return fail(c, AIC_ERR_INVALID, "aic_render: a submitted frame still occupies slot 0 (aic_render_wait it first)");
    uint32_t *target = (uint32_t *)out_rgba8;
    const size_t px_words = (f->flags & (AIC_FRAME_OUT_LINEAR | AIC_FRAME_OUT_COLORBUF)) ? 4 : 1;
    if (!out_is_device && out_rgba8) {
        aic_partition part = f->partition;
        if (part.n_parts <= 1 || part.strip_rows == 0) { part.n_parts = 1; part.part = 0; part.strip_rows = f->height ? f->height : 1; }
        const size_t npix = (size_t)f->width * (part.part < part.n_parts ? aic_partition_rows(f->height, &part) : 0);
        hipError_t e;
        if (npix && (e = c->out.ensure(npix * px_words)) != hipSuccess) return hip_fail(c, "alloc output", e);
        target = c->out.p;
    }
    int rc = submit_frame(c, f, target, 0, true);
    if (rc != AIC_OK) return rc;
    if (!out_is_device && c->slots[0].npix)
        HIP_TRY(c, hipMemcpyAsync(out_rgba8, c->out.p, c->slots[0].npix * px_words * 4, hipMemcpyDeviceToHost, c->slots[0].stream));
    return wait_frame(c, 0, info, !out_is_device);
}

namespace {

struct Mat4h { double m[16]; };
Mat4h mat_identity() { Mat4h t{}; t.m[0] = t.m[5] = t.m[10] = t.m[15] = 1.0; return t; }
Mat4h mat_then(const Mat4h &a, const Mat4h &b) {
    Mat4h o{};
    for (int r = 0; r < 4; r++)
        for (int cc = 0; cc < 4; cc++)
            o.m[r * 4 + cc] = a.m[r * 4 + 0] * b.m[0 * 4 + cc] + a.m[r * 4 + 1] * b.m[1 * 4 + cc] + a.m[r * 4 + 2] * b.m[2 * 4 + cc] + a.m[r * 4 + 3] * b.m[3 * 4 + cc];
    return o;
}
void ortho_view(int resolution, const int32_t lo[3], const int32_t size[3], int viewed_face , DevOrthoView *out) {
    const int axis = (viewed_face - 1) % 3;
    const int32_t ub[3] = {lo[0] + size[0], lo[1] + size[1], lo[2] + size[2]};
    out->w = (uint32_t)(axis == 0 ? size[2] : size[0]) * (uint32_t)resolution;
    out->h = (uint32_t)(axis == 1 ? size[2] : size[1]) * (uint32_t)resolution;
    double ot[3];
    int bx[3], by[3], bz[3];
    auto set = [](int v[3], int x, int y, int z) { v[0] = x; v[1] = y; v[2] = z; };
    switch (viewed_face) {
        case 1: ot[0] = lo[0]; ot[1] = ub[1]; ot[2] = lo[2]; set(bx, 0, 0, 1); set(by, 0, 1, 0); set(bz, -1, 0, 0); break;
        case 2: ot[0] = lo[0]; ot[1] = lo[1]; ot[2] = ub[2]; set(bx, 1, 0, 0); set(by, 0, 0, 1); set(bz, 0, -1, 0); break;
        case 3: ot[0] = ub[0]; ot[1] = ub[1]; ot[2] = lo[2]; set(bx, -1, 0, 0); set(by, 0, 1, 0); set(bz, 0, 0, -1); break;
        case 4: ot[0] = ub[0]; ot[1] = ub[1]; ot[2] = ub[2]; set(bx, 0, 0, -1); set(by, 0, 1, 0); set(bz, 1, 0, 0); break;
        case 5: ot[0] = lo[0]; ot[1] = ub[1]; ot[2] = lo[2]; set(bx, 1, 0, 0); set(by, 0, 0, -1); set(bz, 0, 1, 0); break;
        default: ot[0] = lo[0]; ot[1] = ub[1]; ot[2] = ub[2]; set(bx, 1, 0, 0); set(by, 0, 1, 0); set(bz, 0, 0, 1); break;
    }
    Mat4h t = mat_identity();
    t.m[12] = 0.5; t.m[13] = 0.5;
    Mat4h flip = mat_identity();
    flip.m[5] = -1.0;
    t = mat_then(t, flip);
    Mat4h sc = mat_identity();
    sc.m[0] = sc.m[5] = sc.m[10] = 1.0 / (double)resolution;
    t = mat_then(t, sc);
    Mat4h rot{};
    for (int a = 0; a < 3; a++) { rot.m[0 + a] = bx[a]; rot.m[4 + a] = by[a]; rot.m[8 + a] = bz[a]; }
    rot.m[15] = 1.0;
    t = mat_then(t, rot);
    Mat4h tr = mat_identity();
    tr.m[12] = ot[0]; tr.m[13] = ot[1]; tr.m[14] = ot[2];
    t = mat_then(t, tr);
    std::memcpy(out->m, t.m, sizeof(t.m));
    for (int a = 0; a < 3; a++) { const double d = -t.m[8 + a]; out->dir[a] = d > 0.0 ? 1.0 : (d < 0.0 ? -1.0 : 0.0); }
}
void multi_ortho(int resolution, const int32_t lo[3], const int32_t size[3], DevOrthoView v[5], uint32_t *w, uint32_t *h) {
    ortho_view(resolution, lo, size, 5, &v[0]);
    ortho_view(resolution, lo, size, 1, &v[1]);
    ortho_view(resolution, lo, size, 6, &v[2]);
    ortho_view(resolution, lo, size, 4, &v[3]);
    ortho_view(resolution, lo, size, 2, &v[4]);
    v[0].x0 = v[1].w + 1; v[0].y0 = 0;
    v[1].x0 = 0; v[1].y0 = v[0].h + 1;
    v[2].x0 = v[1].w + 1; v[2].y0 = v[0].h + 1;
    v[3].x0 = v[1].w + v[2].w + 2; v[3].y0 = v[0].h + 1;
    v[4].x0 = v[1].w + 1; v[4].y0 = v[0].h + v[2].h + 2;
    *w = *h = 0;
    for (int i = 0; i < 5; i++) {
        if (v[i].x0 + v[i].w > *w) *w = v[i].x0 + v[i].w;
        if (v[i].y0 + v[i].h > *h) *h = v[i].y0 + v[i].h;
    }
}
bool valid_ortho_resolution(int r) { return r >= 1 && r <= 128 && (r & (r - 1)) == 0; }

}

int aic_ortho_image_size(const int32_t lo[3], const int32_t size[3], int resolution, uint32_t *width, uint32_t *height) {
    if (!lo || !size || !width || !height || !valid_ortho_resolution(resolution) || size[0] < 0 || size[1] < 0 || size[2] < 0) return AIC_ERR_INVALID;
    DevOrthoView v[5];
    multi_ortho(resolution, lo, size, v, width, height);
    return AIC_OK;
}

int aic_render_orthographic(aic_ctx *c, int layer, int resolution, void *out_rgba8, int out_is_device, uint32_t *width, uint32_t *height,
                            aic_frame_info *info) {
    if (!c || !valid_layer(layer) || !valid_ortho_resolution(resolution)) return fail(c, AIC_ERR_INVALID, "aic_render_orthographic: bad argument");
    if (info) std::memset(info, 0, sizeof(*info));
    Layer &l = c->layers[layer];
    if (!l.present) return fail(c, AIC_ERR_INVALID, "aic_render_orthographic: no space uploaded for this layer");
    HIP_TRY(c, hipSetDevice(c->device));
    if (c->slots[0].busy) return fail(c, AIC_ERR_INVALID, "aic_render_orthographic: a submitted frame still occupies slot 0");
    DevOrthoView v[5];
    uint32_t w = 0, h = 0;
    multi_ortho(resolution, l.lo, l.size, v, &w, &h);
    if (width) *width = w;
    if (height) *height = h;
    if (!out_rgba8 || !w || !h) return AIC_OK;
    hipError_t e;
    if ((e = c->ortho_views.ensure(5)) != hipSuccess) return hip_fail(c, "alloc ortho views", e);
    HIP_TRY(c, hipMemcpy(c->ortho_views.p, v, sizeof(v), hipMemcpyHostToDevice));
    aic_frame_desc f;
    std::memset(&f, 0, sizeof(f));
    f.width = w;
    f.height = h;
    static const double ident[16] = {1, 0, 0, 0, 0, 1, 0, 0, 0, 0, 1, 0, 0, 0, 0, 1};
    std::memcpy(f.world.inverse_projection_view, ident, sizeof(ident));
    std::memcpy(f.ui.inverse_projection_view, ident, sizeof(ident));
    f.world.exposure = f.ui.exposure = 1.0f;
    uint32_t *target = (uint32_t *)out_rgba8;
    const size_t npix = (size_t)w * h;
    if (!out_is_device) {
        if ((e = c->out.ensure(npix)) != hipSuccess) return hip_fail(c, "alloc output", e);
        target = c->out.p;
    }
    const bool swap_layers = layer != AIC_LAYER_WORLD;
    if (swap_layers) std::swap(c->layers[AIC_LAYER_WORLD], c->layers[layer]);
    int rc = submit_frame(c, &f, target, 0, false, nullptr, 0, c->ortho_views.p, 5);
    if (swap_layers) std::swap(c->layers[AIC_LAYER_WORLD], c->layers[layer]);
    if (rc != AIC_OK) return rc;
    if (!out_is_device) HIP_TRY(c, hipMemcpyAsync(out_rgba8, c->out.p, npix * 4, hipMemcpyDeviceToHost, c->slots[0].stream));
    return wait_frame(c, 0, info, !out_is_device);
}

int aic_trace_patches(aic_ctx *c, const aic_frame_desc *f, uint32_t n, const double *rects, void *out_rgba8, aic_pixel_aux *aux,
                      aic_frame_info *info) {
    if (!c || !f || (n && (!rects || !out_rgba8))) return fail(c, AIC_ERR_INVALID, "aic_trace_patches: bad argument");
    if (info) std::memset(info, 0, sizeof(*info));
    if (!n) return AIC_OK;
    HIP_TRY(c, hipSetDevice(c->device));
    if (c->slots[0].busy) return fail(c, AIC_ERR_INVALID, "aic_trace_patches: a submitted frame still occupies slot 0 (aic_render_wait it first)");
    if (f->flags & AIC_FRAME_BLOOM) return fail(c, AIC_ERR_UNSUPPORTED, "aic_trace_patches: AIC_FRAME_BLOOM needs a whole frame");
    aic_frame_desc g = *f;
    g.width = n < 2048u ? n : 2048u;
    g.height = (n + g.width - 1u) / g.width;
    if (g.height > 65535u) return fail(c, AIC_ERR_INVALID, "aic_trace_patches: more than 2048 x 65535 rectangles in one call");
    g.partition = aic_partition{0, 1, 0, 0};
    g.flags = (f->flags & (AIC_FRAME_COUNTERS | AIC_FRAME_OUT_LINEAR | AIC_FRAME_OUT_COLORBUF)) | (aux ? AIC_FRAME_AUX : 0u);
    const size_t npix = (size_t)g.width * g.height;
    hipError_t e;
    const size_t px_words = (f->flags & (AIC_FRAME_OUT_LINEAR | AIC_FRAME_OUT_COLORBUF)) ? 4 : 1;
    if ((e = c->out.ensure(npix * px_words)) != hipSuccess) return hip_fail(c, "alloc output", e);
    if ((e = c->staging.ensure((size_t)n * 32)) != hipSuccess) return hip_fail(c, "alloc staging", e);
    HIP_TRY(c, hipMemcpyAsync(c->staging.p, rects, (size_t)n * 32, hipMemcpyHostToDevice, c->slots[0].stream));
    int rc = submit_frame(c, &g, c->out.p, 0, true, (const double *)c->staging.p, n);
    if (rc != AIC_OK) return rc;
    HIP_TRY(c, hipMemcpyAsync(out_rgba8, c->out.p, (size_t)n * px_words * 4, hipMemcpyDeviceToHost, c->slots[0].stream));
    rc = wait_frame(c, 0, info, true);
    if (rc != AIC_OK) return rc;
    if (aux) {
        HIP_TRY(c, hipMemcpy(aux, c->aux.p, (size_t)n * sizeof(aic_pixel_aux), hipMemcpyDeviceToHost));
    }
    if (info) info->rows_rendered = n;
    return AIC_OK;
}

int aic_trace_rays(aic_ctx *c, int layer, uint32_t n, const double *rays, uint32_t flags, float exposure, void *out, aic_pixel_aux *aux,
                   aic_frame_info *info) {
    if (!c || !valid_layer(layer) || (n && (!rays || !out))) return fail(c, AIC_ERR_INVALID, "aic_trace_rays: bad argument");
    if (info) std::memset(info, 0, sizeof(*info));
    if (flags & AIC_FRAME_BLOOM) return fail(c, AIC_ERR_UNSUPPORTED, "aic_trace_rays: AIC_FRAME_BLOOM needs a whole frame");
    if ((flags & AIC_FRAME_OUT_LINEAR) && (flags & AIC_FRAME_OUT_COLORBUF)) return fail(c, AIC_ERR_INVALID, "aic_trace_rays: AIC_FRAME_OUT_LINEAR and AIC_FRAME_OUT_COLORBUF exclude each other");
    if (!(exposure >= 0.f)) return fail(c, AIC_ERR_INVALID, "aic_trace_rays: exposure is negative or NaN");
    if (!n) return AIC_OK;
    HIP_TRY(c, hipSetDevice(c->device));
    if (c->slots[0].busy) return fail(c, AIC_ERR_INVALID, "aic_trace_rays: a submitted frame still occupies slot 0 (aic_render_wait it first)");
    if (!c->layers[layer].present) return fail(c, AIC_ERR_INVALID, "aic_trace_rays: no space uploaded for this layer");
    const bool on_device = (flags & AIC_RAYS_DEVICE) != 0;
    const size_t px_words = (flags & (AIC_FRAME_OUT_LINEAR | AIC_FRAME_OUT_COLORBUF)) ? 4 : 1;
    if (on_device && (((uintptr_t)rays & 15u) || ((uintptr_t)out & (px_words * 4u - 1u)) || ((uintptr_t)aux & 7u)))
        return fail(c, AIC_ERR_INVALID, "aic_trace_rays: AIC_RAYS_DEVICE wants rays at a 16-byte boundary, out and aux at their element's");
    aic_frame_desc g;
    std::memset(&g, 0, sizeof(g));
    g.width = n < 2048u ? n : 2048u;
    g.height = (n + g.width - 1u) / g.width;
    if (g.height > 65535u) return fail(c, AIC_ERR_INVALID, "aic_trace_rays: more than 2048 x 65535 rays in one call");
    g.partition = aic_partition{0, 1, 0, 0};
    g.flags = (flags & (AIC_FRAME_COUNTERS | AIC_FRAME_OUT_LINEAR | AIC_FRAME_OUT_COLORBUF)) | (aux ? AIC_FRAME_AUX : 0u);
    g.tuning = flags & (3u << AIC_TUNE_VARIANT_SHIFT);
    g.world.exposure = exposure;
    g.ui.exposure = 1.0f;
    hipError_t e;
    RayBatch rb{rays, n, (flags & AIC_RAYS_NO_SKY) != 0, (uint32_t)layer, on_device ? reinterpret_cast<DevAux *>(aux) : nullptr};
    uint32_t *target = (uint32_t *)out;
    hipStream_t stream = c->slots[0].stream;
    if (!on_device) {
        if ((e = c->out.ensure((size_t)n * px_words)) != hipSuccess) return hip_fail(c, "alloc output", e);
        if ((e = c->staging.ensure((size_t)n * 48)) != hipSuccess) return hip_fail(c, "alloc staging", e);
        HIP_TRY(c, hipMemcpyAsync(c->staging.p, rays, (size_t)n * 48, hipMemcpyHostToDevice, stream));
        rb.rays = (const double *)c->staging.p;
        target = c->out.p;
    }
    const bool swap_layers = layer != AIC_LAYER_WORLD;
    if (swap_layers) std::swap(c->layers[AIC_LAYER_WORLD], c->layers[layer]);
    int rc = submit_frames(c, 1, &g, &target, 0, true, nullptr, 0, nullptr, 0, &rb);
    if (swap_layers) std::swap(c->layers[AIC_LAYER_WORLD], c->layers[layer]);
    if (rc != AIC_OK) return rc;
    if (!on_device) HIP_TRY(c, hipMemcpyAsync(out, c->out.p, (size_t)n * px_words * 4, hipMemcpyDeviceToHost, stream));
    rc = wait_frame(c, 0, info, !on_device);
    if (rc != AIC_OK) return rc;
    if (aux && !on_device) HIP_TRY(c, hipMemcpy(aux, c->aux.p, (size_t)n * sizeof(aic_pixel_aux), hipMemcpyDeviceToHost));
    if (info) info->rows_rendered = n;
    return AIC_OK;
}

static int ensure_slot(aic_ctx *c, uint32_t slot) {
    aic_ctx::FrameSlot &fs = c->slots[slot];
    if (fs.stream && fs.ev0 && fs.ev1 && fs.ev2 && fs.sub[0].counters.p) return AIC_OK;
    if (!fs.stream) {
        HIP_TRY(c, hipStreamCreateWithFlags(&fs.stream, hipStreamNonBlocking));
        hipEvent_t ev = nullptr;
        HIP_TRY(c, hipEventCreateWithFlags(&ev, hipEventDisableTiming));
        hipError_t e1 = hipEventRecord(ev, c->stream);
        if (e1 == hipSuccess) e1 = hipStreamWaitEvent(fs.stream, ev, 0);
        (void)hipEventDestroy(ev);
        if (e1 != hipSuccess) return hip_fail(c, "order a new slot's stream behind the context's waits", e1);
    }
    if (!fs.ev0) HIP_TRY(c, hipEventCreate(&fs.ev0));
    if (!fs.ev1) HIP_TRY(c, hipEventCreate(&fs.ev1));
    if (!fs.ev2) HIP_TRY(c, hipEventCreate(&fs.ev2));
    hipError_t e = fs.sub[0].counters.ensure(1);
    if (e != hipSuccess) return hip_fail(c, "alloc frame counters", e);
    return AIC_OK;
}

int aic_render_submit(aic_ctx *c, const aic_frame_desc *f, void *out_device, uint32_t slot) {
    if (!c || !f || slot >= AIC_MAX_IN_FLIGHT) return fail(c, AIC_ERR_INVALID, "aic_render_submit: bad argument");
    HIP_TRY(c, hipSetDevice(c->device));
    if (c->slots[slot].busy) return fail(c, AIC_ERR_INVALID, "aic_render_submit: slot busy (aic_render_wait it first)");
    { const int rs = ensure_slot(c, slot); if (rs != AIC_OK) return rs; }
    c->streaming_submit = true;
    const int rc = submit_frame(c, f, (uint32_t *)out_device, slot, false);
    c->streaming_submit = false;
    return rc;
}

int aic_render_submit_batch(aic_ctx *c, uint32_t n_frames, const aic_frame_desc *frames, void *const *out_devices, uint32_t slot) {
    if (!c || !frames || !out_devices || slot >= AIC_MAX_IN_FLIGHT) return fail(c, AIC_ERR_INVALID, "aic_render_submit_batch: bad argument");
    if (n_frames != 1u && n_frames != 2u && n_frames != 4u && n_frames != 8u) return fail(c, AIC_ERR_INVALID, "aic_render_submit_batch: 1, 2, 4 or 8 frames per launch");
    for (uint32_t j = 1; j < n_frames; j++) {
        const aic_frame_desc &a = frames[0], &b = frames[j];
        if (a.width != b.width || a.height != b.height || a.flags != b.flags || a.tuning != b.tuning || std::memcmp(&a.partition, &b.partition, sizeof(a.partition)) != 0)
            return fail(c, AIC_ERR_INVALID, "aic_render_submit_batch: the frames of a batch share size, partition, flags and tuning");
    }
    HIP_TRY(c, hipSetDevice(c->device));
    if (c->slots[slot].busy) return fail(c, AIC_ERR_INVALID, "aic_render_submit_batch: slot busy (aic_render_wait it first)");
    { const int rs = ensure_slot(c, slot); if (rs != AIC_OK) return rs; }
    uint32_t *outs[kMaxSub];
    for (uint32_t j = 0; j < n_frames; j++) outs[j] = (uint32_t *)out_devices[j];
    c->streaming_submit = true;
    const int rc = submit_frames(c, n_frames, frames, outs, slot, false);
    c->streaming_submit = false;
    return rc;
}

int aic_render_wait(aic_ctx *c, uint32_t slot, aic_frame_info *info) {
    if (!c || slot >= AIC_MAX_IN_FLIGHT) return fail(c, AIC_ERR_INVALID, "aic_render_wait: bad argument");
    HIP_TRY(c, hipSetDevice(c->device));
    return wait_frame(c, slot, info);
}

int aic_render_wait_batch(aic_ctx *c, uint32_t slot, uint32_t n_frames, aic_frame_info *infos) {
    if (!c || slot >= AIC_MAX_IN_FLIGHT || (n_frames && !infos)) return fail(c, AIC_ERR_INVALID, "aic_render_wait_batch: bad argument");
    HIP_TRY(c, hipSetDevice(c->device));
    return wait_frame(c, slot, nullptr, false, infos, n_frames);
}

int aic_assemble_strips_on(aic_ctx *c, const void *gathered_device, void *out_device, uint32_t width, uint32_t height,
                           uint32_t strip_rows, uint32_t n_parts, void *hip_stream) {
    if (!c || !gathered_device || !out_device || !strip_rows || !n_parts) return fail(c, AIC_ERR_INVALID, "aic_assemble_strips: bad argument");
    HIP_TRY(c, hipSetDevice(c->device));
    uint32_t max_rows = 0;
    for (uint32_t p = 0; p < n_parts; p++) {
        aic_partition pp = {strip_rows, n_parts, p, 0};
        uint32_t r = aic_partition_rows(height, &pp);
        if (r > max_rows) max_rows = r;
    }
    launch_assemble_strips((const uint32_t *)gathered_device, (uint32_t *)out_device, width, height, strip_rows, n_parts, max_rows, hip_stream ? (hipStream_t)hip_stream : c->stream);
    HIP_TRY(c, hipGetLastError());
    return AIC_OK;
}

int aic_assemble_strips_async(aic_ctx *c, const void *gathered_device, void *out_device, uint32_t width, uint32_t height,
                              uint32_t strip_rows, uint32_t n_parts) {
    return aic_assemble_strips_on(c, gathered_device, out_device, width, height, strip_rows, n_parts, nullptr);
}

int aic_assemble_strips(aic_ctx *c, const void *gathered_device, void *out_device, uint32_t width, uint32_t height,
                        uint32_t strip_rows, uint32_t n_parts) {
    const int rc = aic_assemble_strips_async(c, gathered_device, out_device, width, height, strip_rows, n_parts);
    if (rc != AIC_OK) return rc;
    HIP_TRY(c, hipStreamSynchronize(c->stream));
    return AIC_OK;
}

int aic_read_aux(aic_ctx *c, aic_pixel_aux *out, uint64_t n_records) {
    if (!c || !out) return fail(c, AIC_ERR_INVALID, "aic_read_aux: bad argument");
    if (n_records > c->aux_records) return fail(c, AIC_ERR_INVALID, "aic_read_aux: more records requested than the last frame produced");
    HIP_TRY(c, hipSetDevice(c->device));
    HIP_TRY(c, hipMemcpy(out, c->aux.p, n_records * sizeof(aic_pixel_aux), hipMemcpyDeviceToHost));
    return AIC_OK;
}

int aic_synchronize(aic_ctx *c) {
    if (!c) return AIC_ERR_INVALID;
    HIP_TRY(c, hipSetDevice(c->device));
    HIP_TRY(c, hipStreamSynchronize(c->stream));
    for (uint32_t i = 1; i < AIC_MAX_IN_FLIGHT; i++)
        if (c->slots[i].stream) HIP_TRY(c, hipStreamSynchronize(c->slots[i].stream));
    return AIC_OK;
}

void *aic_stream(aic_ctx *c) { return c ? (void *)c->stream : nullptr; }

int aic_wait_event(aic_ctx *c, void *hip_event) {
    if (!c || !hip_event) return fail(c, AIC_ERR_INVALID, "aic_wait_event: bad argument");
    HIP_TRY(c, hipSetDevice(c->device));
    HIP_TRY(c, hipStreamWaitEvent(c->stream, (hipEvent_t)hip_event, 0));
    for (uint32_t i = 1; i < AIC_MAX_IN_FLIGHT; i++)
        if (c->slots[i].stream) HIP_TRY(c, hipStreamWaitEvent(c->slots[i].stream, (hipEvent_t)hip_event, 0));
    return AIC_OK;
}

int aic_stream_wait_frame(aic_ctx *c, uint32_t slot, void *hip_stream) {
    if (!c || slot >= AIC_MAX_IN_FLIGHT) return fail(c, AIC_ERR_INVALID, "aic_stream_wait_frame: bad argument");
    HIP_TRY(c, hipSetDevice(c->device));
    aic_ctx::FrameSlot &fs = c->slots[slot];
    if (!fs.busy || !fs.npix) return AIC_OK;
    HIP_TRY(c, hipStreamWaitEvent((hipStream_t)hip_stream, fs.ev1, 0));
    return AIC_OK;
}

int aic_probe_raycast(aic_ctx *c, const double origin[3], const double direction[3], int use_bounds, const int32_t lo[3],
                      const int32_t hi[3], int include_exit, uint32_t max_steps, aic_rc_step *out, uint32_t *n_out, int *ended) {
    if (!c || !origin || !direction || !out || !n_out || !ended) return fail(c, AIC_ERR_INVALID, "aic_probe_raycast: bad argument");
    HIP_TRY(c, hipSetDevice(c->device));
    const size_t bytes = 6 * sizeof(double) + 8 * sizeof(int) + (size_t)max_steps * 8 * sizeof(double) + 64;
    hipError_t e = c->staging.ensure(bytes);
    if (e != hipSuccess) return hip_fail(c, "alloc staging", e);
    unsigned char *base = c->staging.p;
    double od[6] = {origin[0], origin[1], origin[2], direction[0], direction[1], direction[2]};
    int lohi[8] = {0, 0, 0, 0, 0, 0, 0, 0};
    if (use_bounds && lo && hi) {
        for (int a = 0; a < 3; a++) { lohi[a] = lo[a]; lohi[3 + a] = hi[a]; }
    }
    double *d_od = (double *)base;
    int *d_lohi = (int *)(base + 48);
    uint32_t *d_n = (uint32_t *)(base + 48 + 24);
    int *d_end = (int *)(base + 48 + 28);
    double *d_rec = (double *)(base + 48 + 32);
    HIP_TRY(c, hipMemcpyAsync(d_od, od, sizeof(od), hipMemcpyHostToDevice, c->stream));
    HIP_TRY(c, hipMemcpyAsync(d_lohi, lohi, 24, hipMemcpyHostToDevice, c->stream));
    launch_probe_raycast(d_od, use_bounds, d_lohi, include_exit, max_steps, d_rec, d_n, d_end, c->stream);
    HIP_TRY(c, hipGetLastError());
    std::vector<double> rec((size_t)max_steps * 8);
    uint32_t n = 0;
    int en = 0;
    HIP_TRY(c, hipMemcpyAsync(&n, d_n, 4, hipMemcpyDeviceToHost, c->stream));
    HIP_TRY(c, hipMemcpyAsync(&en, d_end, 4, hipMemcpyDeviceToHost, c->stream));
    if (max_steps) HIP_TRY(c, hipMemcpyAsync(rec.data(), d_rec, rec.size() * sizeof(double), hipMemcpyDeviceToHost, c->stream));
    HIP_TRY(c, hipStreamSynchronize(c->stream));
    for (uint32_t i = 0; i < n && i < max_steps; i++) {
        const double *r = rec.data() + 8 * (size_t)i;
        out[i].cube[0] = (int32_t)r[0]; out[i].cube[1] = (int32_t)r[1]; out[i].cube[2] = (int32_t)r[2];
        out[i].face = (int32_t)r[3];
        out[i].t_distance = r[4];
        out[i].intersection_point[0] = r[5]; out[i].intersection_point[1] = r[6]; out[i].intersection_point[2] = r[7];
    }
    *n_out = n;
    *ended = en;
    return AIC_OK;
}

int aic_probe_powf(aic_ctx *c, const float *x, const float *y, uint32_t n, float *out) {
    if (!c || (n && (!x || !y || !out))) return fail(c, AIC_ERR_INVALID, "aic_probe_powf: bad argument");
    if (!n) return AIC_OK;
    HIP_TRY(c, hipSetDevice(c->device));
    hipError_t e = c->staging.ensure((size_t)n * 12);
    if (e != hipSuccess) return hip_fail(c, "alloc staging", e);
    float *dx = (float *)c->staging.p, *dy = dx + n, *dout = dy + n;
    HIP_TRY(c, hipMemcpyAsync(dx, x, (size_t)n * 4, hipMemcpyHostToDevice, c->stream));
    HIP_TRY(c, hipMemcpyAsync(dy, y, (size_t)n * 4, hipMemcpyHostToDevice, c->stream));
    launch_probe_powf(dx, dy, dout, n, c->stream);
    HIP_TRY(c, hipGetLastError());
    HIP_TRY(c, hipMemcpyAsync(out, dout, (size_t)n * 4, hipMemcpyDeviceToHost, c->stream));
    HIP_TRY(c, hipStreamSynchronize(c->stream));
    return AIC_OK;
}

int aic_probe_expf(aic_ctx *c, const float *x, uint32_t n, float *out) {
    if (!c || (n && (!x || !out))) return fail(c, AIC_ERR_INVALID, "aic_probe_expf: bad argument");
    if (!n) return AIC_OK;
    for (uint32_t i = 0; i < n; i++)
        if (!(std::fabs(x[i]) < 88.0f)) return fail(c, AIC_ERR_INVALID, "aic_probe_expf: x outside (-88, 88)");
    HIP_TRY(c, hipSetDevice(c->device));
    hipError_t e = c->staging.ensure((size_t)n * 8);
    if (e != hipSuccess) return hip_fail(c, "alloc staging", e);
    float *dx = (float *)c->staging.p, *dout = dx + n;
    HIP_TRY(c, hipMemcpyAsync(dx, x, (size_t)n * 4, hipMemcpyHostToDevice, c->stream));
    launch_probe_expf(dx, dout, n, c->stream);
    HIP_TRY(c, hipGetLastError());
    HIP_TRY(c, hipMemcpyAsync(out, dout, (size_t)n * 4, hipMemcpyDeviceToHost, c->stream));
    HIP_TRY(c, hipStreamSynchronize(c->stream));
    return AIC_OK;
}

int aic_probe_bloom(aic_ctx *c, uint32_t width, uint32_t height, const float *colorbuf, float exposure, const aic_options *options, uint8_t *out_rgba8,
                    uint16_t *out_mip0, uint32_t mip0_size[2]) {
    if (!c || !colorbuf || !options || !out_rgba8 || !width || !height) return fail(c, AIC_ERR_INVALID, "aic_probe_bloom: bad argument");
    if (width > 65535u || height > 65535u) return fail(c, AIC_ERR_INVALID, "aic_probe_bloom: frame dimensions above 65535 are not supported");
    if (!(exposure >= 0.f) || !(options->bloom_intensity >= 0.f)) return fail(c, AIC_ERR_INVALID, "aic_probe_bloom: exposure or bloom_intensity is negative or NaN");
    HIP_TRY(c, hipSetDevice(c->device));
    if (c->slots[0].busy) return fail(c, AIC_ERR_INVALID, "aic_probe_bloom: a submitted frame still occupies slot 0 (aic_render_wait it first)");
    const BloomGeom geom = bloom_geometry(width, height);
    const size_t npix = (size_t)width * height;
    aic_ctx::SubSlot &sb = c->slots[0].sub[0];
    hipError_t e;
    if ((e = sb.bloom_cb.ensure(npix)) != hipSuccess || (e = sb.bloom_mips.ensure(geom.texels)) != hipSuccess || (e = c->out.ensure(npix)) != hipSuccess)
        return hip_fail(c, "alloc bloom scratch", e);
    HIP_TRY(c, hipMemcpyAsync(sb.bloom_cb.p, colorbuf, npix * 16, hipMemcpyHostToDevice, c->stream));
    BloomParams bp;
    bp.colorbuf = sb.bloom_cb.p;
    bp.mips = sb.bloom_mips.p;
    bp.out = c->out.p;
    bp.exposure = exposure + 0.0f;
    bp.intensity = options->bloom_intensity;
    bp.tone_mapping = options->tone_mapping;
    bp.maximum_intensity = options->maximum_intensity;
    bp.srgb_thr = c->srgb_thr.p;
    launch_bloom(geom, bp, c->stream);
    HIP_TRY(c, hipGetLastError());
    HIP_TRY(c, hipMemcpyAsync(out_rgba8, c->out.p, npix * 4, hipMemcpyDeviceToHost, c->stream));
    if (out_mip0) HIP_TRY(c, hipMemcpyAsync(out_mip0, sb.bloom_mips.p, (size_t)geom.mw[0] * geom.mh[0] * 8, hipMemcpyDeviceToHost, c->stream));
    HIP_TRY(c, hipStreamSynchronize(c->stream));
    if (mip0_size) { mip0_size[0] = geom.mw[0]; mip0_size[1] = geom.mh[0]; }
    return AIC_OK;
}

int aic_probe_light_lut(aic_ctx *c, float out[256]) {
    if (!c || !out) return AIC_ERR_INVALID;
    HIP_TRY(c, hipSetDevice(c->device));
    HIP_TRY(c, hipMemcpy(out, c->lut.p, 256 * sizeof(float), hipMemcpyDeviceToHost));
    return AIC_OK;
}

}
```

### all_is_cubes_amd/csrc/aic_ctx.h

```cpp
#pragma once

#include <hip/hip_runtime.h>

#include <chrono>
#include <condition_variable>
#include <cstdio>
#include <mutex>
#include <string>
#include <thread>
#include <vector>

#include "../../include/aic_hip.h"
#include "aic_device.h"

namespace aic {

template <typename T>
struct DevBuf {
    T *p = nullptr;
    size_t n = 0;
    size_t cap = 0;
    hipError_t ensure(size_t count, bool keep = false, hipStream_t stream = nullptr) {
        if (count <= cap) { n = count; return hipSuccess; }
        size_t new_cap = count + count / 4 + 16;
        T *np_ = nullptr;
        hipError_t e = hipMalloc((void **)&np_, new_cap * sizeof(T));
        if (e != hipSuccess) return e;
        if (keep && p && cap) {
            e = hipMemcpyAsync(np_, p, cap * sizeof(T), hipMemcpyDeviceToDevice, stream);
            if (e == hipSuccess) e = hipStreamSynchronize(stream);
            if (e != hipSuccess) {
                (void)hipFree(np_);
                return e;
            }
        }
        if (p) (void)hipFree(p);
        p = np_;
        cap = new_cap;
        n = count;
        return hipSuccess;
    }
    void release() {
        if (p) (void)hipFree(p);
        p = nullptr;
        n = cap = 0;
    }
};

struct LightState;
void light_state_free(LightState *s);
void light_state_cubes_updated(LightState *s, uint64_t version_before, uint64_t version_after, uint32_t n, const int32_t *xyz, const uint16_t *block_index,
                               const uint8_t *light);

struct Layer {
    bool present = false;
    int32_t lo[3] = {0, 0, 0}, size[3] = {0, 0, 0};
    DevBuf<uint16_t> pool;
    DevBuf<uint32_t> cls;
    std::vector<uint32_t> host_cls;
    DevBuf<uint32_t> light;
    static constexpr int kLightSpares = 7;
    DevBuf<uint32_t> light_spare[kLightSpares];
    DevBuf<DevBlock> blocks;
    DevBuf<DevPaletteEntry> palette;
    std::vector<DevBlock> host_blocks;
    std::vector<uint32_t> vox_cap, pal_cap, vox_base, pal_base;
    uint64_t garbage_vox = 0, garbage_pal = 0;
    int32_t air_index = -1;
    int32_t sky_kind = 0;
    float sky[8][3] = {};
    uint32_t block_sky[7] = {};
    aic_options opt;
    bool opt_set = false;
    bool cls_in_code = false;
    uint64_t version = 0;
    uint64_t upload_serial = 0;
    LightState *lstate = nullptr;
    size_t n_cubes() const { return (size_t)size[0] * (size_t)size[1] * (size_t)size[2]; }
    void release() {
        pool.release(); cls.release(); light.release(); blocks.release(); palette.release();
        for (auto &sp : light_spare) sp.release();
        host_blocks.clear(); host_cls.clear(); vox_cap.clear(); pal_cap.clear(); vox_base.clear(); pal_base.clear();
        garbage_vox = garbage_pal = 0;
        present = false;
        version++;
        light_state_free(lstate);
        lstate = nullptr;
    }
};

}

using namespace aic;

struct aic_ctx {
    int device = 0;
    hipStream_t stream = nullptr;
    hipStream_t upload_stream = nullptr;
    Layer layers[2];
    DevBuf<float> lut;
    DevBuf<float> srgb_thr;
    DevBuf<uint32_t> out;
    DevBuf<DevAux> aux;
    DevBuf<unsigned char> staging;
    DevBuf<DevOrthoView> ortho_views;
    uint64_t aux_records = 0;
    bool streaming_submit = false;
    struct SubSlot {
        DevBuf<DevCounters> counters;
        DevCounters *host_counters = nullptr;
        bool counters_clean = false;
        size_t cost_clean_n = 0;
        bool record_ready = false;
        uint32_t order_key[6] = {0, 0, 0, 0, 0, 0};
        DevBuf<float4> acc;
        DevBuf<uint32_t> tile_cost, tile_order, queue_start;
        DevBuf<float4> bloom_cb;
        DevBuf<uint2> bloom_mips;
        uint32_t cost_sig[4] = {0, 0, 0, 0};
        double cost_cam[16] = {0};
        void release() {
            counters.release(); acc.release(); tile_cost.release(); tile_order.release(); queue_start.release(); bloom_cb.release(); bloom_mips.release();
            if (host_counters) (void)hipHostFree(host_counters);
            host_counters = nullptr;
            counters_clean = record_ready = false; cost_clean_n = 0;
        }
    };
    struct FrameSlot {
        hipStream_t stream = nullptr;
        hipEvent_t ev0 = nullptr, ev1 = nullptr;
        hipEvent_t ev2 = nullptr;
        SubSlot sub[kMaxSub];
        uint32_t n_sub = 1;
        bool static_ready = false;
        uint32_t static_key[6] = {0, 0, 0, 0, 0, 0};
        DevBuf<uint32_t> tile_static, queue_static;
        DevBuf<uint4> ray_cold;
        DevBuf<double> edges;
        uint32_t edges_w = 0, edges_h = 0;
        bool busy = false;
        bool diag = false;
        uint32_t variant = 0, tile_queues = 0;
        const void *light_used[2] = {nullptr, nullptr};
        uint32_t flaws = 0, local_rows = 0;
        size_t npix = 0;
        std::chrono::steady_clock::time_point t_begin;
    } slots[AIC_MAX_IN_FLIGHT];
    std::string err;
    std::FILE *dump = nullptr;
    char devname[256] = {0};
    uint32_t n_cus = 256;
    struct LightJob {
        std::thread worker;
        std::mutex mu;
        std::condition_variable cv;
        bool has_work = false, quit = false;
        bool running = false;
        bool pending = false;
        bool result_ready = false;
        int layer = 0, spare = -1;
        aic_light_params params;
        std::vector<int32_t> queue_cubes, queue_priorities;
        int rc = AIC_OK;
        aic_light_info info;
        std::string err;
    } ljob;
    struct Switches {
        int tile = 0, macro = 0;
        bool feedback = true;
        bool wait_whole_stream = false;
        uint32_t tiles_per_wave = 0;
        std::string wave_prof;
    } sw;
};

namespace aic {

extern thread_local std::string *tl_err_sink;
int fail(aic_ctx *c, int code, const char *what, hipError_t e = hipSuccess);
int hip_fail(aic_ctx *c, const char *what, hipError_t e);
#define HIP_TRY(ctx, expr)                                    \
    do {                                                      \
        hipError_t e_ = (expr);                               \
        if (e_ != hipSuccess) return hip_fail(ctx, #expr, e_); \
    } while (0)

inline bool valid_layer(int l) { return l == AIC_LAYER_WORLD || l == AIC_LAYER_UI; }

int take_light_spare(aic_ctx *c, Layer &l, int layer, size_t n, int *index);
int quiesce(aic_ctx *c);
int light_job_finish(aic_ctx *c);

}
```

### all_is_cubes_amd/host/aic_host.hpp

```cpp
#pragma once

#include <array>
#include <cstdint>
#include <functional>
#include <limits>
#include <memory>
#include <set>
#include <stdexcept>
#include <string>
#include <vector>

#include "../../include/aic_hip.h"

namespace aic::host {

struct Vec3 {
    double x = 0, y = 0, z = 0;
};
struct Quat {
    double i = 0, j = 0, k = 0, r = 1;
};
struct Mat4 {
    double m[16] = {1, 0, 0, 0, 0, 1, 0, 0, 0, 0, 1, 0, 0, 0, 0, 1};
    Mat4 then(const Mat4 &other) const;
// ... 112 lines not shown
    static PackedLight some(float r, float g, float b);
    static uint8_t scalar_in(float value);
    static PackedLight one() { return PackedLight{144, 144, 144, 255}; }
    bool operator==(const PackedLight &o) const { return r == o.r && g == o.g && b == o.b && status == o.status; }
};
struct Sky {
    int kind = 0;
    float colors[8][3] = {};
    void for_blocks(uint8_t out[7][4]) const;
};
struct Evoxel {
    float color[4] = {0, 0, 0, 0};
    float emission[3] = {0, 0, 0};
};
struct Evoxels {
    int32_t resolution = 1;
    int32_t vlo[3] = {0, 0, 0}, vsize[3] = {1, 1, 1};
    std::vector<uint16_t> indices;
    std::vector<Evoxel> palette;
    bool is_one = true;
    bool is_air = false;
    std::string display_name;
    static Evoxels from_one(const Evoxel &v);
    static Evoxels air();
};

enum class SpaceChangeKind { EveryBlock, CubeBlock, CubeLight, BlockIndex, BlockEvaluation, EveryLight };
struct SpaceChange {
    SpaceChangeKind kind;
    int32_t cube[3];
    uint32_t block_index;
};
struct SpaceRendererTodo {
    bool everything = true;
    bool every_light = false;
    std::set<uint32_t> blocks;
    std::set<std::array<int32_t, 3>> cubes;
    void receive(const SpaceChange &c);
    void clear() { everything = false; every_light = false; blocks.clear(); cubes.clear(); }
};

class Space {
  public:
    Space(const GridAab &bounds);
    const GridAab &bounds() const { return bounds_; }
    Sky sky;
    uint32_t add_block(const Evoxels &e);
    void set_block_data(uint32_t index, const Evoxels &e);
    size_t n_blocks() const { return blocks_.size(); }
    const Evoxels &block(uint32_t i) const { return blocks_.at(i); }
    void set(int32_t x, int32_t y, int32_t z, uint32_t block_index);
    void set_light(int32_t x, int32_t y, int32_t z, PackedLight l);
    void fill_all(uint32_t block_index);
    void load_contents(const uint16_t *block_index, const uint8_t *light);
    void load_light(const uint8_t *light);
    uint16_t get_block_index(int32_t x, int32_t y, int32_t z) const;
    PackedLight get_light(int32_t x, int32_t y, int32_t z) const;
    const std::vector<uint16_t> &contents() const { return contents_; }
    const std::vector<PackedLight> &light() const { return light_; }
    void listen(const std::shared_ptr<SpaceRendererTodo> &todo);
    size_t index(int32_t x, int32_t y, int32_t z) const;

  private:
    void notify(const SpaceChange &c);
    GridAab bounds_;
    std::vector<uint16_t> contents_;
    std::vector<PackedLight> light_;
    std::vector<Evoxels> blocks_;
    std::vector<std::weak_ptr<SpaceRendererTodo>> listeners_;
};

namespace Flaws {
constexpr uint16_t OTHER = 1 << 0, TOO_COMPLEX = 1 << 1, UNFINISHED = 1 << 2, UNSUPPORTED = 1 << 3;
constexpr uint16_t OUT_OF_TIME = UNFINISHED | (1 << 4), OUT_OF_MEMORY = UNFINISHED | (1 << 5);
constexpr uint16_t NO_ANTIALIASING = UNSUPPORTED | (1 << 7), NO_BLOOM = UNSUPPORTED | (1 << 8), NO_CURSOR = UNSUPPORTED | (1 << 9);
}

struct RenderError : std::runtime_error {
    int code;
    RenderError(int c, const std::string &what) : std::runtime_error(what), code(c) {}
};

struct ImageInfo {
    uint64_t cubes_traced = 0;
    uint64_t n_outer = 0, n_inner = 0, n_hits = 0, n_light = 0;
    float kernel_ms = 0, total_ms = 0;
    uint32_t width = 0, height = 0, rows_rendered = 0;
    std::string status_text() const;
};
struct Rendering {
    uint32_t width = 0, height = 0;
    std::vector<uint8_t> data;
    uint16_t flaws = 0;
    ImageInfo info;
};

void draw_info_text(uint8_t *rgba, uint32_t width, uint32_t height, const uint8_t outline[4], const uint8_t foreground[4], const std::string &text);
void encode_paint(const class Camera &camera, float exposure, const float rgb[3], uint8_t out[4]);

struct UiViewState {
    std::shared_ptr<Space> space;
    ViewTransform view_transform;
    float backdrop[4] = {0, 0, 0, 0};
    GraphicsOptions graphics_options;
};
struct StandardCameras {
    GraphicsOptions graphics_options;
    Viewport viewport;
    std::shared_ptr<Space> world_space;
    ViewTransform world_view_transform;
    float measured_exposure = 1.0f;
    UiViewState ui;
};
struct Cursor {};

class HeadlessRenderer {
  public:
    virtual ~HeadlessRenderer() = default;
    virtual void update(const Cursor *cursor) = 0;
    virtual Rendering draw(const std::string &info_text) = 0;
};

class HipRtRenderer : public HeadlessRenderer {
  public:
    using SizePolicy = std::function<Viewport(Viewport)>;
    HipRtRenderer(std::shared_ptr<StandardCameras> cameras, SizePolicy size_policy = nullptr, int device_id = -1);
    ~HipRtRenderer() override;
    HipRtRenderer(const HipRtRenderer &) = delete;
    HipRtRenderer &operator=(const HipRtRenderer &) = delete;

    bool update_scene(const Cursor *cursor);
    void update(const Cursor *cursor) override { (void)update_scene(cursor); }
    Rendering draw(const std::string &info_text) override { return draw_rgba(info_text); }
    Rendering draw_rgba(const std::string &info_text);
    void set_bloom(bool on) { bloom_ = on; }
    bool bloom() const { return bloom_; }
    void set_world_camera_override(const double *inverse_projection_view, float exposure);
    std::string draw_text(const std::string &line_ending = "\n");
    struct RayResults {
        std::vector<std::array<float, 4>> colors;
        std::vector<aic_pixel_aux> hits;
        ImageInfo info;
    };
    RayResults trace_rays(int layer, const std::vector<Ray> &rays, bool include_sky = true);
    ImageInfo draw_rows_to_device(void *device_out, uint32_t strip_rows, uint32_t n_parts, uint32_t part, bool counters = false,
                                  bool no_feedback = false);
    uint32_t partition_rows(uint32_t strip_rows, uint32_t n_parts, uint32_t part) const;
    void assemble_strips(const void *gathered_device, void *out_device, uint32_t strip_rows, uint32_t n_parts, bool wait = true);
    void submit_rows_to_device(void *device_out, uint32_t strip_rows, uint32_t n_parts, uint32_t part, uint32_t slot);
    void submit_rows_batch_to_device(const std::vector<void *> &device_outs, uint32_t strip_rows, uint32_t n_parts, uint32_t part, uint32_t slot,
                                     const std::vector<std::array<double, 16>> &inverse_projection_views = {});
    ImageInfo wait_rows(uint32_t slot);
    void synchronize();
    Viewport modified_viewport() const;
    const StandardCameras &cameras() const { return *cameras_; }
    std::string device_name() const;
    void *stream() const;
    void wait_event(void *hip_event);
    void stream_wait_rows(uint32_t slot, void *hip_stream);
    struct LightUpdateInfo { uint64_t updates, batches, cost; double device_ms, total_ms; uint32_t queue_left; uint64_t bundles_visited; };
    void evaluate_light_submit(int maximum_distance, bool fast, int epsilon, int batch, int queue_order, int lanes_per_cube = 0, bool continue_queue = false,
                               uint64_t max_updates = 0);
    LightUpdateInfo evaluate_light_wait();
    bool evaluate_light_done();
    LightUpdateInfo evaluate_light(int maximum_distance, bool fast = true, int epsilon = 1, int batch = 32, int queue_order = 16, int lanes_per_cube = 0,
                                   bool continue_queue = false, uint64_t max_updates = 0);
    bool device_light = false;
    int device_light_queue_order = 16;
    bool enable_counters = false;

  private:
    struct LayerState {
        std::shared_ptr<Space> space;
        std::shared_ptr<SpaceRendererTodo> todo;
        GraphicsOptions options;
        bool options_valid = false;
    };
    bool sync_space(int layer, const std::shared_ptr<Space> &space, const GraphicsOptions &options);
    void upload_full(int layer, const Space &space);
    void check(int rc, const char *what);
    aic_frame_desc make_frame() const;
    std::shared_ptr<StandardCameras> cameras_;
    SizePolicy size_policy_;
    aic_ctx *ctx_ = nullptr;
    LayerState layers_[2];
    bool cam_override_ = false;
    double cam_override_inv_[16] = {0};
    float cam_override_exposure_ = 1.0f;
    bool had_cursor_ = false;
    bool bloom_ = false;
    Camera world_camera_, ui_camera_;
    float backdrop_[4] = {0, 0, 0, 0};
    bool show_ui_ = true;
};

inline HipRtRenderer::RayResults HipRtRenderer::trace_rays(int layer, const std::vector<Ray> &rays, bool include_sky) {
    static_assert(sizeof(Ray) == 6 * sizeof(double), "a Ray is the ABI's six doubles: origin, then direction");
    if (rays.size() > 2048u * 65535u) throw RenderError(AIC_ERR_INVALID, "trace_rays: more than 2048 x 65535 rays in one call");
    RayResults out;
    out.colors.resize(rays.size());
    out.hits.resize(rays.size());
    aic_frame_info fi;
    const uint32_t flags = AIC_FRAME_OUT_COLORBUF | (enable_counters ? AIC_FRAME_COUNTERS : 0u) | (include_sky ? 0u : AIC_RAYS_NO_SKY);
    check(aic_trace_rays(ctx_, layer, (uint32_t)rays.size(), rays.empty() ? nullptr : &rays[0].origin.x, flags, 1.0f, out.colors.data(), out.hits.data(), &fi),
          "aic_trace_rays");
    ImageInfo &i = out.info;
    i.cubes_traced = fi.cubes_traced; i.n_outer = fi.n_outer; i.n_inner = fi.n_inner; i.n_hits = fi.n_hits; i.n_light = fi.n_light;
    i.kernel_ms = fi.kernel_ms; i.total_ms = fi.total_ms; i.width = (uint32_t)rays.size(); i.height = 1; i.rows_rendered = fi.rows_rendered;
    return out;
}

}
```

### all_is_cubes_amd/host/py_module.cpp

```cpp
#include <pybind11/functional.h>
#include <pybind11/numpy.h>
#include <pybind11/pybind11.h>
#include <pybind11/stl.h>

#include <cstring>

#include "aic_host.hpp"

namespace py = pybind11;
using namespace aic::host;

static Vec3 v3(const std::array<double, 3> &a) { return Vec3{a[0], a[1], a[2]}; }
static std::array<double, 3> a3(const Vec3 &v) { return {v.x, v.y, v.z}; }
static py::array_t<double> mat(const Mat4 &m) {
    py::array_t<double> out({4, 4});
    std::memcpy(out.mutable_data(), m.m, sizeof(m.m));
    return out;
}

PYBIND11_MODULE(_host, m) {
    m.doc() = "C++ host mirror of the all-is-cubes raytracer interface above the MI355X C ABI";

    py::register_exception<RenderError>(m, "RenderError");

// ... 82 lines not shown
        .def("as_texel", [](const PackedLight &p) { return std::array<int, 4>{p.r, p.g, p.b, p.status}; });

    py::class_<Sky>(m, "Sky")
        .def(py::init<>())
        .def_readwrite("kind", &Sky::kind)
        .def("set_uniform", [](Sky &s, const std::array<float, 3> &c) { s.kind = 0; std::memset(s.colors, 0, sizeof(s.colors)); for (int i = 0; i < 3; i++) s.colors[0][i] = c[i]; })
        .def("set_octants", [](Sky &s, py::array_t<float, py::array::c_style | py::array::forcecast> c) {
            if (c.size() != 24) throw std::invalid_argument("octants needs 8x3 floats");
            s.kind = 1;
            std::memcpy(s.colors, c.data(), sizeof(s.colors));
        })
        .def("for_blocks", [](const Sky &s) {
            uint8_t out[7][4];
            s.for_blocks(out);
            py::array_t<uint8_t> a({7, 4});
            std::memcpy(a.mutable_data(), out, sizeof(out));
            return a;
        });

    py::class_<Evoxels>(m, "Evoxels")
        .def_static("from_one", [](const std::array<float, 4> &rgba, const std::array<float, 3> &em) {
            Evoxel v;
            for (int i = 0; i < 4; i++) v.color[i] = rgba[i];
            for (int i = 0; i < 3; i++) v.emission[i] = em[i];
            return Evoxels::from_one(v);
        }, py::arg("rgba"), py::arg("emission") = std::array<float, 3>{0, 0, 0})
        .def_static("air", &Evoxels::air)
        .def_static("paletted", [](int resolution, const std::array<int32_t, 3> &vlo, py::array_t<uint16_t, py::array::c_style | py::array::forcecast> idx,
                                   py::array_t<float, py::array::c_style | py::array::forcecast> pal) {
            if (idx.ndim() != 3) throw std::invalid_argument("indices must be 3-D");
            if (pal.ndim() != 2 || pal.shape(1) != 8) throw std::invalid_argument("palette must be [n][8]");
            Evoxels e;
            e.resolution = resolution;
            e.is_one = false;
            for (int a = 0; a < 3; a++) { e.vlo[a] = vlo[a]; e.vsize[a] = (int32_t)idx.shape(a); }
            e.indices.assign(idx.data(), idx.data() + idx.size());
            e.palette.resize((size_t)pal.shape(0));
            for (size_t i = 0; i < e.palette.size(); i++) {
                const float *p = pal.data() + 8 * i;
                std::memcpy(e.palette[i].color, p, 16);
                std::memcpy(e.palette[i].emission, p + 4, 12);
            }
            return e;
        })
        .def_readwrite("resolution", &Evoxels::resolution).def_readwrite("is_air", &Evoxels::is_air).def_readwrite("is_one", &Evoxels::is_one)
        .def_readwrite("display_name", &Evoxels::display_name);

    py::class_<Space, std::shared_ptr<Space>>(m, "Space")
        .def(py::init([](const std::array<int32_t, 3> &lo, const std::array<int32_t, 3> &size) {
            return std::make_shared<Space>(GridAab::from_lower_size(lo.data(), size.data()));
        }))
        .def_readwrite("sky", &Space::sky)
        .def("add_block", &Space::add_block).def("set_block_data", &Space::set_block_data).def("n_blocks", &Space::n_blocks)
        .def("set", &Space::set).def("set_light", &Space::set_light).def("fill_all", &Space::fill_all)
        .def("get_block_index", &Space::get_block_index)
        .def("load_contents", [](Space &s, py::array_t<uint16_t, py::array::c_style | py::array::forcecast> bi, py::object light) {
            if ((size_t)bi.size() != s.contents().size()) throw std::invalid_argument("block_index size mismatch");
            const uint8_t *lp = nullptr;
            py::array_t<uint8_t, py::array::c_style | py::array::forcecast> la;
            if (!light.is_none()) {
                la = light.cast<py::array_t<uint8_t, py::array::c_style | py::array::forcecast>>();
                if ((size_t)la.size() != s.contents().size() * 4) throw std::invalid_argument("light size mismatch");
                lp = la.data();
            }
            s.load_contents(bi.data(), lp);
        }, py::arg("block_index"), py::arg("light") = py::none())
        .def("load_light", [](Space &s, py::array_t<uint8_t, py::array::c_style | py::array::forcecast> la) {
            if ((size_t)la.size() != s.contents().size() * 4) throw std::invalid_argument("light size mismatch");
            s.load_light(la.data());
        }, py::arg("light"))
        .def("bounds", [](const Space &s) { const GridAab &b = s.bounds(); return py::make_tuple(std::array<int32_t, 3>{b.lo[0], b.lo[1], b.lo[2]}, std::array<int32_t, 3>{b.hi[0], b.hi[1], b.hi[2]}); });

    py::class_<UiViewState>(m, "UiViewState")
        .def(py::init<>())
        .def_readwrite("space", &UiViewState::space).def_readwrite("view_transform", &UiViewState::view_transform)
        .def_readwrite("graphics_options", &UiViewState::graphics_options)
        .def_property("backdrop", [](const UiViewState &u) { return std::array<float, 4>{u.backdrop[0], u.backdrop[1], u.backdrop[2], u.backdrop[3]}; },
                      [](UiViewState &u, const std::array<float, 4> &b) { for (int i = 0; i < 4; i++) u.backdrop[i] = b[i]; });
    py::class_<StandardCameras, std::shared_ptr<StandardCameras>>(m, "StandardCameras")
        .def(py::init([]() { return std::make_shared<StandardCameras>(); }))
        .def_readwrite("graphics_options", &StandardCameras::graphics_options).def_readwrite("viewport", &StandardCameras::viewport)
        .def_readwrite("world_space", &StandardCameras::world_space).def_readwrite("world_view_transform", &StandardCameras::world_view_transform)
        .def_readwrite("measured_exposure", &StandardCameras::measured_exposure).def_readwrite("ui", &StandardCameras::ui);

    py::class_<ImageInfo>(m, "ImageInfo")
        .def_readonly("cubes_traced", &ImageInfo::cubes_traced).def_readonly("n_outer", &ImageInfo::n_outer).def_readonly("n_inner", &ImageInfo::n_inner)
        .def_readonly("n_hits", &ImageInfo::n_hits).def_readonly("n_light", &ImageInfo::n_light).def_readonly("kernel_ms", &ImageInfo::kernel_ms)
        .def_readonly("total_ms", &ImageInfo::total_ms).def_readonly("width", &ImageInfo::width).def_readonly("height", &ImageInfo::height)
        .def_readonly("rows_rendered", &ImageInfo::rows_rendered).def("status_text", &ImageInfo::status_text);
    py::class_<Rendering>(m, "Rendering")
        .def_readonly("width", &Rendering::width).def_readonly("height", &Rendering::height).def_readonly("flaws", &Rendering::flaws)
        .def_readonly("info", &Rendering::info)
        .def_property_readonly("data", [](const Rendering &r) {
            py::array_t<uint8_t> a({(py::ssize_t)r.height, (py::ssize_t)r.width, (py::ssize_t)4});
            if (!r.data.empty()) std::memcpy(a.mutable_data(), r.data.data(), r.data.size());
            return a;
        });

    auto flaws = m.def_submodule("Flaws");
    flaws.attr("OTHER") = Flaws::OTHER; flaws.attr("UNSUPPORTED") = Flaws::UNSUPPORTED; flaws.attr("NO_BLOOM") = Flaws::NO_BLOOM;
    flaws.attr("NO_CURSOR") = Flaws::NO_CURSOR; flaws.attr("OUT_OF_MEMORY") = Flaws::OUT_OF_MEMORY;

    py::class_<Cursor>(m, "Cursor").def(py::init<>());

    py::class_<HipRtRenderer>(m, "HipRtRenderer")
        .def(py::init([](std::shared_ptr<StandardCameras> cams, py::object policy, int device_id) {
            HipRtRenderer::SizePolicy sp = nullptr;
            if (!policy.is_none()) sp = policy.cast<HipRtRenderer::SizePolicy>();
            return std::make_unique<HipRtRenderer>(std::move(cams), sp, device_id);
        }), py::arg("cameras"), py::arg("size_policy") = py::none(), py::arg("device_id") = -1)
        .def("update", [](HipRtRenderer &r, py::object cursor) { Cursor c; return r.update_scene(cursor.is_none() ? nullptr : &c); }, py::arg("cursor") = py::none())
        .def("draw", [](HipRtRenderer &r, const std::string &t) { py::gil_scoped_release rel; return r.draw(t); }, py::arg("info_text") = "")
        .def("draw_text", [](HipRtRenderer &r, const std::string &le) { py::gil_scoped_release rel; return r.draw_text(le); }, py::arg("line_ending") = "\n")
        .def("trace_rays", [](HipRtRenderer &r, int layer, py::array_t<double, py::array::c_style | py::array::forcecast> rays, bool include_sky) {
            if (rays.size() % 6 != 0) throw std::invalid_argument("rays: [n, 6] doubles");
            std::vector<Ray> v((size_t)rays.size() / 6);
            if (!v.empty()) std::memcpy(&v[0], rays.data(), v.size() * sizeof(Ray));
            HipRtRenderer::RayResults res;
            { py::gil_scoped_release rel; res = r.trace_rays(layer, v, include_sky); }
            py::array_t<float> colors({(py::ssize_t)v.size(), (py::ssize_t)4});
            py::array_t<uint8_t> hits({(py::ssize_t)v.size(), (py::ssize_t)sizeof(aic_pixel_aux)});
            if (!v.empty()) {
                std::memcpy(colors.mutable_data(), res.colors.data(), v.size() * 16);
                std::memcpy(hits.mutable_data(), res.hits.data(), v.size() * sizeof(aic_pixel_aux));
            }
            py::dict d;
            d["colorbuf"] = colors; d["hits"] = hits; d["info"] = res.info;
            return d;
        }, py::arg("layer"), py::arg("rays"), py::arg("include_sky") = true)
        .def("set_world_camera_override", [](HipRtRenderer &r, py::object inv, float exposure) {
            if (inv.is_none()) { r.set_world_camera_override(nullptr, 1.0f); return; }
            const auto m = inv.cast<std::array<double, 16>>();
            r.set_world_camera_override(m.data(), exposure);
        }, py::arg("inverse_projection_view"), py::arg("exposure") = 1.0f)
        .def("draw_rgba", [](HipRtRenderer &r, const std::string &t) { py::gil_scoped_release rel; return r.draw_rgba(t); }, py::arg("info_text") = "")
        .def("set_bloom", &HipRtRenderer::set_bloom, py::arg("on"))
        .def_property_readonly("bloom", &HipRtRenderer::bloom)
        .def("draw_rows_to_device", [](HipRtRenderer &r, uintptr_t ptr, uint32_t strip_rows, uint32_t n_parts, uint32_t part, bool counters, bool no_feedback) {
            py::gil_scoped_release rel;
            return r.draw_rows_to_device(reinterpret_cast<void *>(ptr), strip_rows, n_parts, part, counters, no_feedback);
        }, py::arg("device_ptr"), py::arg("strip_rows"), py::arg("n_parts"), py::arg("part"), py::arg("counters") = false, py::arg("no_feedback") = false)
        .def("partition_rows", &HipRtRenderer::partition_rows)
        .def("submit_rows_to_device", [](HipRtRenderer &r, uintptr_t ptr, uint32_t strip_rows, uint32_t n_parts, uint32_t part, uint32_t slot) {
            r.submit_rows_to_device(reinterpret_cast<void *>(ptr), strip_rows, n_parts, part, slot);
        }, py::arg("device_ptr"), py::arg("strip_rows"), py::arg("n_parts"), py::arg("part"), py::arg("slot"))
        .def("submit_rows_batch_to_device", [](HipRtRenderer &r, const std::vector<uintptr_t> &ptrs, uint32_t strip_rows, uint32_t n_parts, uint32_t part, uint32_t slot,
                                               const std::vector<std::array<double, 16>> &views) {
            std::vector<void *> outs;
            for (uintptr_t p : ptrs) outs.push_back(reinterpret_cast<void *>(p));
            r.submit_rows_batch_to_device(outs, strip_rows, n_parts, part, slot, views);
        }, py::arg("device_ptrs"), py::arg("strip_rows"), py::arg("n_parts"), py::arg("part"), py::arg("slot"), py::arg("inverse_projection_views") = std::vector<std::array<double, 16>>())
        .def("wait_rows", [](HipRtRenderer &r, uint32_t slot) { py::gil_scoped_release rel; return r.wait_rows(slot); }, py::arg("slot"))
        .def("synchronize", [](HipRtRenderer &r) { py::gil_scoped_release rel; r.synchronize(); })
        .def("assemble_strips", [](HipRtRenderer &r, uintptr_t gathered, uintptr_t out, uint32_t strip_rows, uint32_t n_parts, bool wait) {
            r.assemble_strips(reinterpret_cast<const void *>(gathered), reinterpret_cast<void *>(out), strip_rows, n_parts, wait);
        }, py::arg("gathered"), py::arg("out"), py::arg("strip_rows"), py::arg("n_parts"), py::arg("wait") = true)
        .def("modified_viewport", &HipRtRenderer::modified_viewport)
        .def("device_name", &HipRtRenderer::device_name)
        .def("stream", [](const HipRtRenderer &r) { return reinterpret_cast<uintptr_t>(r.stream()); })
        .def("wait_event", [](HipRtRenderer &r, uintptr_t ev) { r.wait_event(reinterpret_cast<void *>(ev)); })
        .def("stream_wait_rows", [](HipRtRenderer &r, uint32_t slot, uintptr_t stream) { r.stream_wait_rows(slot, reinterpret_cast<void *>(stream)); },
             py::arg("slot"), py::arg("hip_stream"))
        .def("evaluate_light", [](HipRtRenderer &r, int maximum_distance, bool fast, int epsilon, int batch, int queue_order, int lanes_per_cube, bool continue_queue,
                                  uint64_t max_updates) {
            const HipRtRenderer::LightUpdateInfo i = r.evaluate_light(maximum_distance, fast, epsilon, batch, queue_order, lanes_per_cube, continue_queue, max_updates);
            py::dict d;
            d["updates"] = i.updates; d["batches"] = i.batches; d["cost"] = i.cost; d["device_ms"] = i.device_ms;
            d["total_ms"] = i.total_ms; d["queue_left"] = i.queue_left; d["bundles_visited"] = i.bundles_visited;
            return d;
        }, py::arg("maximum_distance"), py::arg("fast") = true, py::arg("epsilon") = 1, py::arg("batch") = 32, py::arg("queue_order") = 16, py::arg("lanes_per_cube") = 0, py::arg("continue_queue") = false,
           py::arg("max_updates") = 0)
        .def("evaluate_light_submit", [](HipRtRenderer &r, int maximum_distance, bool fast, int epsilon, int batch, int queue_order, int lanes_per_cube, bool continue_queue,
                                         uint64_t max_updates) { r.evaluate_light_submit(maximum_distance, fast, epsilon, batch, queue_order, lanes_per_cube, continue_queue, max_updates); },
             py::arg("maximum_distance"), py::arg("fast") = true, py::arg("epsilon") = 1, py::arg("batch") = 32, py::arg("queue_order") = 16, py::arg("lanes_per_cube") = 0,
             py::arg("continue_queue") = false, py::arg("max_updates") = 0)
        .def("evaluate_light_done", &HipRtRenderer::evaluate_light_done)
        .def("evaluate_light_wait", [](HipRtRenderer &r) {
            py::gil_scoped_release rel;
            const HipRtRenderer::LightUpdateInfo i = r.evaluate_light_wait();
            py::gil_scoped_acquire acq;
            py::dict d;
            d["updates"] = i.updates; d["batches"] = i.batches; d["cost"] = i.cost; d["device_ms"] = i.device_ms;
            d["total_ms"] = i.total_ms; d["queue_left"] = i.queue_left; d["bundles_visited"] = i.bundles_visited;
            return d;
        })
        .def_readwrite("device_light", &HipRtRenderer::device_light)
        .def_readwrite("device_light_queue_order", &HipRtRenderer::device_light_queue_order)
        .def_readwrite("enable_counters", &HipRtRenderer::enable_counters);
}
```

### include/aic_hip.h

```cpp
#ifndef AIC_HIP_H
#define AIC_HIP_H

#include <stdint.h>

#ifdef __cplusplus
extern "C" {
#endif

#define AIC_ABI_VERSION 3

#define AIC_OK 0
#define AIC_ERR_INVALID 1
#define AIC_ERR_NO_DEVICE 2
#define AIC_ERR_OOM 3
#define AIC_ERR_DEVICE 4
#define AIC_ERR_UNSUPPORTED 5

#define AIC_LAYER_WORLD 0
#define AIC_LAYER_UI 1

#define AIC_FLAW_UNSUPPORTED 1u
#define AIC_FLAW_NO_BLOOM 2u

#define AIC_BLOCK_ONE 1u
#define AIC_BLOCK_AIR 2u

typedef struct aic_block_desc {
    int32_t resolution;
    int32_t vlo[3];
    int32_t vsize[3];
    uint32_t vox_off;
    uint32_t pal_off;
    uint32_t pal_len;
    uint32_t flags;
    int32_t reserved;
} aic_block_desc;

typedef struct aic_space_desc {
    int32_t lo[3];
    int32_t size[3];
    const uint16_t *block_index;
    const uint8_t *light;
    uint32_t n_blocks;
    const aic_block_desc *blocks;
    const uint16_t *voxels;
    uint64_t n_voxels;
    const float *palette;
    uint64_t n_palette;
    int32_t sky_kind;
    float sky[8][3];
    uint8_t block_sky[7][4];
} aic_space_desc;

typedef struct aic_options {
    int32_t fog;
    int32_t transparency;
    float threshold;
    int32_t lighting;
    int32_t bounce_samples;
    int32_t antialiasing;
    int32_t debug_pixel_cost;
    int32_t tone_mapping;
    float maximum_intensity;
    float bloom_intensity;
    double view_distance;
} aic_options;

typedef struct aic_camera {
    double inverse_projection_view[16];
    float exposure;
    int32_t reserved;
} aic_camera;

typedef struct aic_partition {
    uint32_t strip_rows;
    uint32_t n_parts;
    uint32_t part;
    uint32_t reserved;
} aic_partition;

typedef struct aic_frame_desc {
    uint32_t width, height;
    aic_camera world;
    aic_camera ui;
    float backdrop[4];
    aic_partition partition;
    uint32_t flags;
    uint32_t tuning;
} aic_frame_desc;

#define AIC_TUNE_QUEUES_SHIFT 0
#define AIC_TUNE_SUPER_SHIFT 4
#define AIC_TUNE_VARIANT_SHIFT 9
#define AIC_VARIANT_AUTO 0
#define AIC_VARIANT_PLAIN 1
#define AIC_VARIANT_EXCHANGING 2
#define AIC_VARIANT_RECORDING 3

#define AIC_FRAME_COUNTERS 1u
#define AIC_FRAME_AUX 2u
#define AIC_FRAME_OUT_LINEAR 8u
#define AIC_FRAME_OUT_COLORBUF 16u
#define AIC_FRAME_NO_FEEDBACK 32u
#define AIC_FRAME_BLOOM 64u
#define AIC_FRAME_PIXEL_CENTERS 4u

typedef struct aic_frame_info {
    uint64_t cubes_traced;
    uint64_t n_outer;
    uint64_t n_inner;
    uint64_t n_hits;
    uint64_t n_light;
    float kernel_ms;
    float total_ms;
    uint32_t rows_rendered;
    uint32_t flaws;
    uint32_t variant;
    uint32_t tile_queues;
} aic_frame_info;

typedef struct aic_pixel_aux {
    int32_t hit;
    int32_t cube[3];
    int32_t voxel[3];
    int32_t resolution;
    int32_t face;
    int32_t block_index;
    uint32_t cubes_traced;
    uint32_t layer;
    double t_distance;
} aic_pixel_aux;

typedef struct aic_ctx aic_ctx;

aic_ctx *aic_create(int device_id, int *status);
void aic_destroy(aic_ctx *ctx);
const char *aic_last_error(const aic_ctx *ctx);
int aic_abi_version(void);
int aic_device_name(const aic_ctx *ctx, char *buf, uint32_t buf_len);

int aic_upload_space(aic_ctx *ctx, int layer, const aic_space_desc *space);
int aic_clear_space(aic_ctx *ctx, int layer);
int aic_update_cubes(aic_ctx *ctx, int layer, uint32_t n, const int32_t *xyz, const uint16_t *block_index,
                     const uint8_t *light);
int aic_update_light_volume(aic_ctx *ctx, int layer, const uint8_t *light);
int aic_replace_block(aic_ctx *ctx, int layer, uint32_t index, const aic_block_desc *desc, const uint16_t *voxels,
                      const float *palette);
int aic_replace_blocks(aic_ctx *ctx, int layer, uint32_t n, const uint32_t *indices, const aic_block_desc *descs,
                       const uint16_t *const *voxels, const float *const *palettes);
int aic_compact(aic_ctx *ctx, int layer);
int aic_set_options(aic_ctx *ctx, int layer, const aic_options *options);

int aic_render(aic_ctx *ctx, const aic_frame_desc *frame, void *out_rgba8, int out_is_device, aic_frame_info *info);
#define AIC_MAX_IN_FLIGHT 32u
int aic_render_submit(aic_ctx *ctx, const aic_frame_desc *frame, void *out_device, uint32_t slot);
int aic_render_wait(aic_ctx *ctx, uint32_t slot, aic_frame_info *info);
int aic_render_submit_batch(aic_ctx *ctx, uint32_t n_frames, const aic_frame_desc *frames, void *const *out_devices, uint32_t slot);
int aic_render_wait_batch(aic_ctx *ctx, uint32_t slot, uint32_t n_frames, aic_frame_info *infos);
int aic_trace_patches(aic_ctx *ctx, const aic_frame_desc *frame, uint32_t n, const double *rects, void *out_rgba8,
                      aic_pixel_aux *aux, aic_frame_info *info);
#define AIC_RAYS_NO_SKY 128u
#define AIC_RAYS_DEVICE 256u
int aic_trace_rays(aic_ctx *ctx, int layer, uint32_t n, const double *rays, uint32_t flags, float exposure, void *out, aic_pixel_aux *aux,
                   aic_frame_info *info);
uint32_t aic_partition_rows(uint32_t height, const aic_partition *partition);
int aic_assemble_strips(aic_ctx *ctx, const void *gathered_device, void *out_device, uint32_t width, uint32_t height,
                        uint32_t strip_rows, uint32_t n_parts);
int aic_assemble_strips_async(aic_ctx *ctx, const void *gathered_device, void *out_device, uint32_t width, uint32_t height,
                              uint32_t strip_rows, uint32_t n_parts);
int aic_assemble_strips_on(aic_ctx *ctx, const void *gathered_device, void *out_device, uint32_t width, uint32_t height,
                           uint32_t strip_rows, uint32_t n_parts, void *hip_stream);
int aic_read_aux(aic_ctx *ctx, aic_pixel_aux *out, uint64_t n_records);
int aic_synchronize(aic_ctx *ctx);
void *aic_stream(aic_ctx *ctx);
int aic_wait_event(aic_ctx *ctx, void *hip_event);
int aic_stream_wait_frame(aic_ctx *ctx, uint32_t slot, void *hip_stream);

int aic_ortho_image_size(const int32_t lo[3], const int32_t size[3], int resolution, uint32_t *width, uint32_t *height);
int aic_render_orthographic(aic_ctx *ctx, int layer, int resolution, void *out_rgba8, int out_is_device, uint32_t *width,
                            uint32_t *height, aic_frame_info *info);

typedef struct aic_multi aic_multi;
aic_multi *aic_create_multi(int n_devices, const int *device_ids, int *status);
void aic_destroy_multi(aic_multi *m);
int aic_multi_device_count(const aic_multi *m);
aic_ctx *aic_multi_context(aic_multi *m, int i);
const char *aic_multi_last_error(const aic_multi *m);
int aic_multi_upload_space(aic_multi *m, int layer, const aic_space_desc *space);
int aic_multi_clear_space(aic_multi *m, int layer);
int aic_multi_update_cubes(aic_multi *m, int layer, uint32_t n, const int32_t *xyz, const uint16_t *block_index, const uint8_t *light);
int aic_multi_update_light_volume(aic_multi *m, int layer, const uint8_t *light);
int aic_multi_replace_blocks(aic_multi *m, int layer, uint32_t n, const uint32_t *indices, const aic_block_desc *descs,
                             const uint16_t *const *voxels, const float *const *palettes);
int aic_multi_set_options(aic_multi *m, int layer, const aic_options *options);
int aic_multi_render(aic_multi *m, const aic_frame_desc *frame, void *out_rgba8, int out_is_device, aic_frame_info *info);
#define AIC_MULTI_MAX_IN_FLIGHT 8u
int aic_multi_render_submit(aic_multi *m, const aic_frame_desc *frame, void *out_rgba8, int out_is_device, uint32_t slot);
int aic_multi_render_wait(aic_multi *m, uint32_t slot, aic_frame_info *info);

typedef struct aic_rc_step {
    int32_t cube[3];
    int32_t face;
    double t_distance;
    double intersection_point[3];
} aic_rc_step;
int aic_probe_raycast(aic_ctx *ctx, const double origin[3], const double direction[3], int use_bounds,
                      const int32_t lo[3], const int32_t hi[3], int include_exit, uint32_t max_steps,
                      aic_rc_step *out, uint32_t *n_out, int *ended);
int aic_probe_powf(aic_ctx *ctx, const float *x, const float *y, uint32_t n, float *out);
int aic_probe_expf(aic_ctx *ctx, const float *x, uint32_t n, float *out);
int aic_probe_bloom(aic_ctx *ctx, uint32_t width, uint32_t height, const float *colorbuf, float exposure, const aic_options *options,
                    uint8_t *out_rgba8, uint16_t *out_mip0, uint32_t mip0_size[2]);
int aic_probe_light_lut(aic_ctx *ctx, float out[256]);

typedef struct aic_light_params {
    int32_t maximum_distance;
    int32_t fast;
    int32_t epsilon;
    int32_t batch;
    int32_t queue_order;
    int32_t n_queue;
    int32_t lanes_per_cube;
    int32_t hooks;
    const int32_t *queue_cubes;
    const int32_t *queue_priorities;
    uint64_t max_updates;
} aic_light_params;
#define AIC_LIGHT_HOOK_SESSION 1
#define AIC_LIGHT_HOOK_POOL_SHIFT 8
typedef struct aic_light_info {
    uint64_t updates;
    uint64_t batches;
    uint64_t cost;
    double device_ms;
    double total_ms;
    uint32_t queue_left;
    uint32_t pad;
    uint64_t bundles_visited;
} aic_light_info;
int aic_evaluate_light(aic_ctx *ctx, int layer, const aic_light_params *params, aic_light_info *info);
int aic_evaluate_light_submit(aic_ctx *ctx, int layer, const aic_light_params *params);
int aic_evaluate_light_wait(aic_ctx *ctx, int layer, aic_light_info *info);
int aic_evaluate_light_poll(aic_ctx *ctx, int layer, int *done);
int aic_light_cubes_changed(aic_ctx *ctx, int layer, uint32_t n, const int32_t *xyz, int queue_order);
int aic_read_light_volume(aic_ctx *ctx, int layer, uint8_t *out);
int aic_read_light_cubes(aic_ctx *ctx, int layer, uint32_t n, const int32_t *xyz, uint8_t *out);
uint32_t aic_light_chart(float *weights, uint32_t *children, uint32_t *depth);
int aic_probe_derived(aic_ctx *ctx, int layer, float *out, uint8_t *out_opaque);
int aic_probe_log2f(aic_ctx *ctx, const float *x, uint32_t n, float *out);
int aic_multi_evaluate_light(aic_multi *m, int layer, const aic_light_params *params, aic_light_info *info);
int aic_multi_light_cubes_changed(aic_multi *m, int layer, uint32_t n, const int32_t *xyz, int queue_order);

#ifdef __cplusplus
}
#endif
#endif
```

### rust/all-is-cubes-hip/src/ffi.rs

```rust
#![allow(non_camel_case_types, missing_docs, clippy::missing_safety_doc)]

use core::ffi::{c_char, c_int, c_void};

pub const AIC_ABI_VERSION: c_int = 3;
pub const AIC_OK: c_int = 0;
pub const AIC_ERR_INVALID: c_int = 1;
pub const AIC_ERR_NO_DEVICE: c_int = 2;
pub const AIC_ERR_OOM: c_int = 3;
pub const AIC_ERR_DEVICE: c_int = 4;
pub const AIC_ERR_UNSUPPORTED: c_int = 5;
pub const AIC_LAYER_WORLD: c_int = 0;
pub const AIC_LAYER_UI: c_int = 1;
pub const AIC_BLOCK_ONE: u32 = 1;
pub const AIC_BLOCK_AIR: u32 = 2;
pub const AIC_FLAW_UNSUPPORTED: u32 = 1;
pub const AIC_FLAW_NO_BLOOM: u32 = 2;
pub const AIC_FRAME_COUNTERS: u32 = 1;
pub const AIC_FRAME_AUX: u32 = 2;
pub const AIC_FRAME_PIXEL_CENTERS: u32 = 4;
pub const AIC_FRAME_OUT_LINEAR: u32 = 8;
pub const AIC_FRAME_OUT_COLORBUF: u32 = 16;
pub const AIC_FRAME_NO_FEEDBACK: u32 = 32;
pub const AIC_FRAME_BLOOM: u32 = 64;
pub const AIC_RAYS_NO_SKY: u32 = 128;
// ... 41 lines not shown
    pub block_sky: [[u8; 4]; 7],
}

#[repr(C)]
#[derive(Clone, Copy, Debug)]
pub struct aic_options {
    pub fog: i32,
    pub transparency: i32,
    pub threshold: f32,
    pub lighting: i32,
    pub bounce_samples: i32,
    pub antialiasing: i32,
    pub debug_pixel_cost: i32,
    pub tone_mapping: i32,
    pub maximum_intensity: f32,
    pub bloom_intensity: f32,
    pub view_distance: f64,
}

#[repr(C)]
#[derive(Clone, Copy, Debug)]
pub struct aic_camera {
    pub inverse_projection_view: [f64; 16],
    pub exposure: f32,
    pub reserved: i32,
}

#[repr(C)]
#[derive(Clone, Copy, Debug, Default)]
pub struct aic_partition {
    pub strip_rows: u32,
    pub n_parts: u32,
    pub part: u32,
    pub reserved: u32,
}

#[repr(C)]
#[derive(Clone, Copy, Debug)]
pub struct aic_frame_desc {
    pub width: u32,
    pub height: u32,
    pub world: aic_camera,
    pub ui: aic_camera,
    pub backdrop: [f32; 4],
    pub partition: aic_partition,
    pub flags: u32,
    pub tuning: u32,
}

#[repr(C)]
#[derive(Clone, Copy, Debug, Default)]
pub struct aic_frame_info {
    pub cubes_traced: u64,
    pub n_outer: u64,
    pub n_inner: u64,
    pub n_hits: u64,
    pub n_light: u64,
    pub kernel_ms: f32,
    pub total_ms: f32,
    pub rows_rendered: u32,
    pub flaws: u32,
    pub variant: u32,
    pub tile_queues: u32,
}

#[repr(C)]
#[derive(Clone, Copy, Debug, Default)]
pub struct aic_pixel_aux {
    pub hit: i32,
    pub cube: [i32; 3],
    pub voxel: [i32; 3],
    pub resolution: i32,
    pub face: i32,
    pub block_index: i32,
    pub cubes_traced: u32,
    pub layer: u32,
    pub t_distance: f64,
}

#[repr(C)]
#[derive(Clone, Copy, Debug, Default)]
pub struct aic_rc_step {
    pub cube: [i32; 3],
    pub face: i32,
    pub t_distance: f64,
    pub intersection_point: [f64; 3],
}

#[repr(C)]
pub struct aic_ctx {
    _private: [u8; 0],
}
#[repr(C)]
pub struct aic_multi {
    _private: [u8; 0],
}

#[repr(C)]
#[derive(Clone, Copy, Debug)]
pub struct aic_light_params {
    pub maximum_distance: i32,
    pub fast: i32,
    pub epsilon: i32,
    pub batch: i32,
    pub queue_order: i32,
    pub n_queue: i32,
    pub lanes_per_cube: i32,
    pub hooks: i32,
    pub queue_cubes: *const i32,
    pub queue_priorities: *const i32,
    pub max_updates: u64,
}

#[repr(C)]
#[derive(Clone, Copy, Debug, Default)]
pub struct aic_light_info {
    pub updates: u64,
    pub batches: u64,
    pub cost: u64,
    pub device_ms: f64,
    pub total_ms: f64,
    pub queue_left: u32,
    pub pad: u32,
    pub bundles_visited: u64,
}

unsafe extern "C" {
    pub fn aic_create(device_id: c_int, status: *mut c_int) -> *mut aic_ctx;
    pub fn aic_destroy(ctx: *mut aic_ctx);
    pub fn aic_last_error(ctx: *const aic_ctx) -> *const c_char;
    pub fn aic_abi_version() -> c_int;
    pub fn aic_device_name(ctx: *const aic_ctx, buf: *mut c_char, buf_len: u32) -> c_int;
    pub fn aic_upload_space(ctx: *mut aic_ctx, layer: c_int, space: *const aic_space_desc) -> c_int;
    pub fn aic_clear_space(ctx: *mut aic_ctx, layer: c_int) -> c_int;
    pub fn aic_update_cubes(ctx: *mut aic_ctx, layer: c_int, n: u32, xyz: *const i32, block_index: *const u16, light: *const u8) -> c_int;
    pub fn aic_update_light_volume(ctx: *mut aic_ctx, layer: c_int, light: *const u8) -> c_int;
    pub fn aic_replace_block(ctx: *mut aic_ctx, layer: c_int, index: u32, desc: *const aic_block_desc, voxels: *const u16, palette: *const f32) -> c_int;
    pub fn aic_replace_blocks(ctx: *mut aic_ctx, layer: c_int, n: u32, indices: *const u32, descs: *const aic_block_desc, voxels: *const *const u16, palettes: *const *const f32) -> c_int;
    pub fn aic_compact(ctx: *mut aic_ctx, layer: c_int) -> c_int;
    pub fn aic_set_options(ctx: *mut aic_ctx, layer: c_int, options: *const aic_options) -> c_int;
    pub fn aic_render(ctx: *mut aic_ctx, frame: *const aic_frame_desc, out_rgba8: *mut c_void, out_is_device: c_int, info: *mut aic_frame_info) -> c_int;
    pub fn aic_render_submit(ctx: *mut aic_ctx, frame: *const aic_frame_desc, out_device: *mut c_void, slot: u32) -> c_int;
    pub fn aic_render_wait(ctx: *mut aic_ctx, slot: u32, info: *mut aic_frame_info) -> c_int;
    pub fn aic_render_submit_batch(ctx: *mut aic_ctx, n_frames: u32, frames: *const aic_frame_desc, out_devices: *const *mut c_void, slot: u32) -> c_int;
    pub fn aic_render_wait_batch(ctx: *mut aic_ctx, slot: u32, n_frames: u32, infos: *mut aic_frame_info) -> c_int;
    pub fn aic_trace_patches(ctx: *mut aic_ctx, frame: *const aic_frame_desc, n: u32, rects: *const f64, out_rgba8: *mut c_void, aux: *mut aic_pixel_aux, info: *mut aic_frame_info) -> c_int;
    pub fn aic_partition_rows(height: u32, partition: *const aic_partition) -> u32;
    pub fn aic_assemble_strips(ctx: *mut aic_ctx, gathered_device: *const c_void, out_device: *mut c_void, width: u32, height: u32, strip_rows: u32, n_parts: u32) -> c_int;
    pub fn aic_assemble_strips_async(ctx: *mut aic_ctx, gathered_device: *const c_void, out_device: *mut c_void, width: u32, height: u32, strip_rows: u32, n_parts: u32) -> c_int;
    pub fn aic_assemble_strips_on(ctx: *mut aic_ctx, gathered_device: *const c_void, out_device: *mut c_void, width: u32, height: u32, strip_rows: u32, n_parts: u32, hip_stream: *mut c_void) -> c_int;
    pub fn aic_trace_rays(ctx: *mut aic_ctx, layer: c_int, n: u32, rays: *const f64, flags: u32, exposure: f32, out: *mut c_void, aux: *mut aic_pixel_aux, info: *mut aic_frame_info) -> c_int;
    pub fn aic_read_aux(ctx: *mut aic_ctx, out: *mut aic_pixel_aux, n_records: u64) -> c_int;
    pub fn aic_synchronize(ctx: *mut aic_ctx) -> c_int;
    pub fn aic_stream(ctx: *mut aic_ctx) -> *mut c_void;
    pub fn aic_wait_event(ctx: *mut aic_ctx, hip_event: *mut c_void) -> c_int;
    pub fn aic_stream_wait_frame(ctx: *mut aic_ctx, slot: u32, hip_stream: *mut c_void) -> c_int;
    pub fn aic_ortho_image_size(lo: *const i32, size: *const i32, resolution: c_int, width: *mut u32, height: *mut u32) -> c_int;
    pub fn aic_render_orthographic(ctx: *mut aic_ctx, layer: c_int, resolution: c_int, out_rgba8: *mut c_void, out_is_device: c_int, width: *mut u32, height: *mut u32, info: *mut aic_frame_info) -> c_int;
    pub fn aic_create_multi(n_devices: c_int, device_ids: *const c_int, status: *mut c_int) -> *mut aic_multi;
    pub fn aic_destroy_multi(m: *mut aic_multi);
    pub fn aic_multi_device_count(m: *const aic_multi) -> c_int;
    pub fn aic_multi_context(m: *mut aic_multi, i: c_int) -> *mut aic_ctx;
    pub fn aic_multi_last_error(m: *const aic_multi) -> *const c_char;
    pub fn aic_multi_upload_space(m: *mut aic_multi, layer: c_int, space: *const aic_space_desc) -> c_int;
    pub fn aic_multi_clear_space(m: *mut aic_multi, layer: c_int) -> c_int;
    pub fn aic_multi_update_cubes(m: *mut aic_multi, layer: c_int, n: u32, xyz: *const i32, block_index: *const u16, light: *const u8) -> c_int;
    pub fn aic_multi_update_light_volume(m: *mut aic_multi, layer: c_int, light: *const u8) -> c_int;
    pub fn aic_multi_replace_blocks(m: *mut aic_multi, layer: c_int, n: u32, indices: *const u32, descs: *const aic_block_desc, voxels: *const *const u16, palettes: *const *const f32) -> c_int;
    pub fn aic_multi_set_options(m: *mut aic_multi, layer: c_int, options: *const aic_options) -> c_int;
    pub fn aic_multi_render(m: *mut aic_multi, frame: *const aic_frame_desc, out_rgba8: *mut c_void, out_is_device: c_int, info: *mut aic_frame_info) -> c_int;
    pub fn aic_multi_render_submit(m: *mut aic_multi, frame: *const aic_frame_desc, out_rgba8: *mut c_void, out_is_device: c_int, slot: u32) -> c_int;
    pub fn aic_multi_render_wait(m: *mut aic_multi, slot: u32, info: *mut aic_frame_info) -> c_int;
    pub fn aic_probe_raycast(ctx: *mut aic_ctx, origin: *const f64, direction: *const f64, use_bounds: c_int, lo: *const i32, hi: *const i32, include_exit: c_int, max_steps: u32, out: *mut aic_rc_step, n_out: *mut u32, ended: *mut c_int) -> c_int;
    pub fn aic_probe_powf(ctx: *mut aic_ctx, x: *const f32, y: *const f32, n: u32, out: *mut f32) -> c_int;
    pub fn aic_probe_expf(ctx: *mut aic_ctx, x: *const f32, n: u32, out: *mut f32) -> c_int;
    pub fn aic_probe_bloom(ctx: *mut aic_ctx, width: u32, height: u32, colorbuf: *const f32, exposure: f32, options: *const aic_options, out_rgba8: *mut u8, out_mip0: *mut u16, mip0_size: *mut u32) -> c_int;
    pub fn aic_probe_light_lut(ctx: *mut aic_ctx, out: *mut f32) -> c_int;
    pub fn aic_evaluate_light(ctx: *mut aic_ctx, layer: c_int, params: *const aic_light_params, info: *mut aic_light_info) -> c_int;
    pub fn aic_evaluate_light_submit(ctx: *mut aic_ctx, layer: c_int, params: *const aic_light_params) -> c_int;
    pub fn aic_evaluate_light_wait(ctx: *mut aic_ctx, layer: c_int, info: *mut aic_light_info) -> c_int;
    pub fn aic_evaluate_light_poll(ctx: *mut aic_ctx, layer: c_int, done: *mut c_int) -> c_int;
    pub fn aic_light_cubes_changed(ctx: *mut aic_ctx, layer: c_int, n: u32, xyz: *const i32, queue_order: c_int) -> c_int;
    pub fn aic_read_light_volume(ctx: *mut aic_ctx, layer: c_int, out: *mut u8) -> c_int;
    pub fn aic_read_light_cubes(ctx: *mut aic_ctx, layer: c_int, n: u32, xyz: *const i32, out: *mut u8) -> c_int;
    pub fn aic_light_chart(weights: *mut f32, children: *mut u32, depth: *mut u32) -> u32;
    pub fn aic_probe_derived(ctx: *mut aic_ctx, layer: c_int, out: *mut f32, out_opaque: *mut u8) -> c_int;
    pub fn aic_probe_log2f(ctx: *mut aic_ctx, x: *const f32, n: u32, out: *mut f32) -> c_int;
    pub fn aic_multi_evaluate_light(m: *mut aic_multi, layer: c_int, params: *const aic_light_params, info: *mut aic_light_info) -> c_int;
    pub fn aic_multi_light_cubes_changed(m: *mut aic_multi, layer: c_int, n: u32, xyz: *const i32, queue_order: c_int) -> c_int;
}
```

Measured before the change: 6227.

## Probe hardware-concurrent streams at startup and schedule in-flight frames across lanes

At context creation, sleep kernels are launched on candidate streams and their wall-clock intervals compared, which groups streams that actually run concurrently. Distinct groups become "lanes". Each streamed frame is assigned to the least-loaded lane, and completion is detected by polling host-visible counters. The tiles-per-wave sizing now uses the lane count and unfinished frames in place of a fixed cap of 4. Cross-lane housekeeping dependencies are enforced with events. The aim is real overlap of concurrent frames on separate hardware queues, at the cost of a startup probe and more complex event ordering.

Result: no change. 6224, median of 2 (-0.1%).

```diff
diff --git a/all_is_cubes_amd/abi.py b/all_is_cubes_amd/abi.py
--- a/all_is_cubes_amd/abi.py
+++ b/all_is_cubes_amd/abi.py
@@ -44,7 +44,7 @@
 ABI_SYMBOLS = [
     "aic_abi_version", "aic_create", "aic_destroy", "aic_last_error", "aic_device_name", "aic_upload_space",
     "aic_clear_space", "aic_update_cubes", "aic_update_light_volume", "aic_replace_block", "aic_replace_blocks", "aic_compact", "aic_set_options",
-    "aic_render", "aic_render_submit", "aic_render_wait", "aic_render_submit_batch", "aic_render_wait_batch", "aic_trace_patches", "aic_trace_rays", "aic_partition_rows", "aic_assemble_strips", "aic_assemble_strips_async", "aic_assemble_strips_on", "aic_read_aux", "aic_synchronize", "aic_stream", "aic_wait_event", "aic_stream_wait_frame",
+    "aic_render", "aic_render_submit", "aic_render_wait", "aic_render_submit_batch", "aic_render_wait_batch", "aic_trace_patches", "aic_trace_rays", "aic_partition_rows", "aic_assemble_strips", "aic_assemble_strips_async", "aic_assemble_strips_on", "aic_read_aux", "aic_synchronize", "aic_stream", "aic_stream_lanes", "aic_slot_chip_parts", "aic_lane_probe_ms", "aic_wait_event", "aic_stream_wait_frame",
     "aic_probe_raycast", "aic_probe_light_lut", "aic_probe_powf", "aic_probe_expf", "aic_probe_bloom",
     "aic_ortho_image_size", "aic_render_orthographic",
     "aic_evaluate_light", "aic_evaluate_light_submit", "aic_evaluate_light_wait", "aic_evaluate_light_poll", "aic_light_cubes_changed", "aic_read_light_volume", "aic_read_light_cubes", "aic_light_chart", "aic_probe_derived", "aic_probe_log2f",
@@ -150,6 +150,12 @@
         lib.aic_last_error.argtypes = [C.c_void_p]
         lib.aic_stream.restype = C.c_void_p
         lib.aic_stream.argtypes = [C.c_void_p]
+        lib.aic_stream_lanes.restype = C.c_uint32
+        lib.aic_stream_lanes.argtypes = [C.c_void_p]
+        lib.aic_slot_chip_parts.restype = C.c_uint32
+        lib.aic_slot_chip_parts.argtypes = [C.c_void_p, C.c_uint32]
+        lib.aic_lane_probe_ms.restype = C.c_float
+        lib.aic_lane_probe_ms.argtypes = [C.c_void_p]
         lib.aic_partition_rows.restype = C.c_uint32
         lib.aic_partition_rows.argtypes = [C.c_uint32, C.POINTER(Partition)]
         lib.aic_upload_space.argtypes = [C.c_void_p, C.c_int, C.POINTER(SpaceDesc)]
@@ -485,6 +491,15 @@
     def synchronize(self) -> None:
         self._check(self._lib.aic_synchronize(self._h))
 
+    def stream_lanes(self) -> int:
+        return int(self._lib.aic_stream_lanes(self._h))
+
+    def slot_chip_parts(self, slot: int) -> int:
+        return int(self._lib.aic_slot_chip_parts(self._h, int(slot)))
+
+    def lane_probe_ms(self) -> float:
+        return float(self._lib.aic_lane_probe_ms(self._h))
+
     def stream_wait_frame(self, slot: int, hip_stream: int) -> None:
         self._check(self._lib.aic_stream_wait_frame(self._h, int(slot), C.c_void_p(hip_stream)))
 
diff --git a/all_is_cubes_amd/csrc/aic_abi.cpp b/all_is_cubes_amd/csrc/aic_abi.cpp
--- a/all_is_cubes_amd/csrc/aic_abi.cpp
+++ b/all_is_cubes_amd/csrc/aic_abi.cpp
@@ -73,6 +73,63 @@
     for (const DumpPart &d : parts)
         if (d.p && d.n) std::fwrite(d.p, 1, d.n, c->dump);
     std::fflush(c->dump);
+}
+
+__global__ void lane_probe_kernel(unsigned long long *stamps, unsigned long long spin_ticks, uint32_t max_iters) {
+    if (threadIdx.x != 0) return;
+    const unsigned long long t0 = wall_clock64();
+    unsigned long long t1 = t0;
+    for (uint32_t i = 0; i < max_iters && t1 - t0 < spin_ticks; i++) {
+        __builtin_amdgcn_s_sleep(8);
+        t1 = wall_clock64();
+    }
+    stamps[0] = t0;
+    stamps[1] = t1 > t0 ? t1 : t0 + 1ull;
+}
+
+hipError_t probe_lanes(aic_ctx *c) {
+    constexpr uint32_t n = kLaneCandidates;
+    constexpr double spin_us = 64.0;
+    int khz = 0;
+    hipError_t e = hipDeviceGetAttribute(&khz, hipDeviceAttributeWallClockRate, c->device);
+    if (e != hipSuccess) return e;
+    if (khz <= 0) khz = 100000;
+    const unsigned long long spin_ticks = (unsigned long long)((double)khz * spin_us / 1000.0);
+    unsigned long long *stamps = nullptr;
+    if ((e = hipHostMalloc((void **)&stamps, sizeof(unsigned long long) * 2 * n * kLaneTrials, hipHostMallocDefault)) != hipSuccess) return e;
+    std::memset(stamps, 0, sizeof(unsigned long long) * 2 * n * kLaneTrials);
+    auto sync_all = [&]() {
+        hipError_t r = hipSuccess;
+        for (uint32_t i = 0; i < n; i++) { const hipError_t q = hipStreamSynchronize(c->cand[i]); if (r == hipSuccess) r = q; }
+        return r;
+    };
+    for (uint32_t i = 0; i < n && e == hipSuccess; i++) {
+        hipLaunchKernelGGL(lane_probe_kernel, dim3(1), dim3(64), 0, c->cand[i], stamps + 2 * i, 0ull, 0u);
+        e = hipGetLastError();
+    }
+    if (e == hipSuccess) e = sync_all();
+    const auto t_begin = std::chrono::steady_clock::now();
+    for (uint32_t t = 0; t < kLaneTrials && e == hipSuccess; t++) {
+        for (uint32_t q = 0; q < n && e == hipSuccess; q++) {
+            const uint32_t i = (t & 1u) ? n - 1u - q : q;
+            hipLaunchKernelGGL(lane_probe_kernel, dim3(1), dim3(64), 0, c->cand[i], stamps + 2 * (t * n + i), spin_ticks, (uint32_t)(spin_us * 8.0));
+            e = hipGetLastError();
+        }
+        const hipError_t q = sync_all();
+        if (e == hipSuccess) e = q;
+    }
+    c->lane_probe_ms = std::chrono::duration<float, std::milli>(std::chrono::steady_clock::now() - t_begin).count();
+    if (e == hipSuccess) {
+        LaneInterval iv[kLaneTrials * n];
+        for (uint32_t i = 0; i < kLaneTrials * n; i++) iv[i] = {stamps[2 * i], stamps[2 * i + 1]};
+        uint32_t group[n], pick[kMaxLanes];
+        (void)lane_groups(iv, kLaneTrials, n, group);
+        c->n_lanes = lanes_from_groups(group, n, n - 1u, kMaxLanes, pick);
+        for (uint32_t k = 0; k < c->n_lanes; k++) c->lane[k] = c->cand[pick[k]];
+        if (c->n_lanes == 0) e = hipErrorUnknown;
+    }
+    (void)hipHostFree(stamps);
+    return e;
 }
 
 }
@@ -281,6 +338,7 @@
         c->sw.feedback = env_int("AIC_TILE_FEEDBACK", 1) != 0;
         c->sw.wait_whole_stream = env_int("AIC_WAIT_WHOLE_STREAM", 0) != 0;
         c->sw.tiles_per_wave = (uint32_t)std::max(0, env_int("AIC_TILES_PER_WAVE", 0));
+        c->sw.stream_lanes = env_int("AIC_STREAM_LANES", -1);
         if (const char *p = std::getenv("AIC_WAVE_PROF")) c->sw.wave_prof = p;
     }
     if (const char *path = std::getenv("AIC_DUMP")) {
@@ -292,13 +350,23 @@
         if (c->dump) std::fwrite("AICDUMP1", 1, 8, c->dump);
     }
     bool ok = hipStreamCreateWithFlags(&c->stream, hipStreamNonBlocking) == hipSuccess;
+    const bool per_slot_streams = c->sw.stream_lanes == 0;
     for (uint32_t i = 0; ok && i < 8u && i < AIC_MAX_IN_FLIGHT; i++) {
         aic_ctx::FrameSlot &fs = c->slots[i];
-        if (i == 0) fs.stream = c->stream;
-        else ok = hipStreamCreateWithFlags(&fs.stream, hipStreamNonBlocking) == hipSuccess;
-        ok = ok && hipEventCreate(&fs.ev0) == hipSuccess && hipEventCreate(&fs.ev1) == hipSuccess && hipEventCreate(&fs.ev2) == hipSuccess && fs.sub[0].counters.ensure(1) == hipSuccess;
+        if (i == 0) c->cand[i] = c->stream;
+        else ok = hipStreamCreateWithFlags(&c->cand[i], hipStreamNonBlocking) == hipSuccess;
+        fs.stream = per_slot_streams ? c->cand[i] : c->stream;
+        ok = ok && hipEventCreate(&fs.ev0) == hipSuccess && hipEventCreate(&fs.ev1) == hipSuccess && hipEventCreate(&fs.ev2) == hipSuccess &&
+             hipEventCreateWithFlags(&fs.ev3, hipEventDisableTiming) == hipSuccess && fs.sub[0].counters.ensure(1) == hipSuccess;
     }
     ok = ok && hipStreamCreateWithFlags(&c->upload_stream, hipStreamNonBlocking) == hipSuccess;
+    c->cand[kLaneCandidates - 1u] = c->upload_stream;
+    if (ok && c->sw.stream_lanes > 0) {
+        c->n_lanes = std::min((uint32_t)c->sw.stream_lanes, kMaxLanes);
+        for (uint32_t k = 0; k < c->n_lanes; k++) c->lane[k] = c->cand[k];
+    } else if (ok && !per_slot_streams) {
+        ok = probe_lanes(c) == hipSuccess;
+    }
     float lut[256];
     lut[0] = 0.f;
     for (int v = 1; v < 256; v++) {
@@ -367,9 +435,12 @@
         if (fs.ev0) (void)hipEventDestroy(fs.ev0);
         if (fs.ev1) (void)hipEventDestroy(fs.ev1);
         if (fs.ev2) (void)hipEventDestroy(fs.ev2);
+        if (fs.ev3) (void)hipEventDestroy(fs.ev3);
         fs.tile_static.release(); fs.queue_static.release();
-        if (i > 0 && fs.stream) (void)hipStreamDestroy(fs.stream);
-    }
+        if (fs.owns_stream && fs.stream) (void)hipStreamDestroy(fs.stream);
+    }
+    for (uint32_t i = 1; i + 1u < kLaneCandidates; i++)
+        if (c->cand[i]) { (void)hipStreamSynchronize(c->cand[i]); (void)hipStreamDestroy(c->cand[i]); }
     for (auto &l : c->layers) l.release();
     c->lut.release(); c->srgb_thr.release(); c->out.release(); c->aux.release(); c->staging.release(); c->ortho_views.release();
     if (c->dump) std::fclose(c->dump);
@@ -761,6 +832,17 @@
     uint32_t layer;
     DevAux *aux_target;
 };
+constexpr unsigned long long kFramePending = ~0ull;
+bool frame_seen_done(const aic_ctx::FrameSlot &fs) {
+#ifndef AIC_PROFILE
+    for (uint32_t j = 0; j < fs.n_sub; j++)
+        if (!fs.sub[j].host_counters || *const_cast<const volatile unsigned long long *>(&fs.sub[j].host_counters->bailed) == kFramePending) return false;
+    return true;
+#else
+    return hipEventQuery(fs.ev2) == hipSuccess;
+#endif
+}
+
 int submit_frames(aic_ctx *c, uint32_t k, const aic_frame_desc *frames, uint32_t *const *out_devices, uint32_t slot, bool allow_aux, const double *patches = nullptr,
                   uint32_t n_patches = 0, const DevOrthoView *ortho = nullptr, int32_t ortho_n = 0, const RayBatch *rb = nullptr) {
     if (rb) n_patches = rb->n;
@@ -839,15 +921,27 @@
     F.light_lut = c->lut.p;
     F.n_cus = c->n_cus;
     F.tiles_per_wave = c->sw.tiles_per_wave ? c->sw.tiles_per_wave : (c->streaming_submit ? 4u : 1u);
+    uint32_t unfinished_others = 0, lane_load[kMaxLanes] = {};
+    for (uint32_t i = 0; i < AIC_MAX_IN_FLIGHT; i++) {
+        aic_ctx::FrameSlot &o = c->slots[i];
+        if (i == slot) continue;
+        if (!c->n_lanes) { unfinished_others += o.busy ? 1u : 0u; continue; }
+        if (o.unfinished && frame_seen_done(o)) o.unfinished = false;
+        if (!o.unfinished) continue;
+        unfinished_others++;
+        if (o.lane >= 0 && (uint32_t)o.lane < c->n_lanes) lane_load[o.lane]++;
+    }
+    if (c->n_lanes) {
+        fs.lane = c->streaming_submit ? (int32_t)pick_lane(lane_load, c->n_lanes, &c->lane_cursor) : -1;
+        fs.stream = fs.lane >= 0 ? c->lane[fs.lane] : c->stream;
+    }
+    fs.share = 1u;
     if (!c->sw.tiles_per_wave && c->streaming_submit && k == 1u) {
-        uint32_t busy_others = 0;
-        for (uint32_t i = 0; i < AIC_MAX_IN_FLIGHT; i++) busy_others += (i != slot && c->slots[i].busy) ? 1u : 0u;
         const uint32_t resident_waves = (uint32_t)c->n_cus * 16u;
         const uint32_t tpw_full = (F.tiles_x * F.tiles_y + resident_waves - 1u) / resident_waves;
-        if (tpw_full >= 4u && busy_others > 0u) {
-            const uint32_t t = tpw_full * (busy_others < 4u ? busy_others : 4u);
-            F.tiles_per_wave = t < 32u ? t : (tpw_full > 32u ? tpw_full : 32u);
-        }
+        const uint32_t lanes = c->n_lanes ? c->n_lanes : 4u;
+        F.tiles_per_wave = streamed_tiles_per_wave(tpw_full, unfinished_others, lanes, F.tiles_per_wave);
+        if (tpw_full >= 4u && unfinished_others > 0u) fs.share = chip_share_divisor(unfinished_others, lanes);
     }
     F.srgb_thr = c->srgb_thr.p;
 
@@ -863,6 +957,18 @@
     if (allow_aux) c->aux_records = 0;
     if (!npix) return AIC_OK;
     hipError_t e;
+    if (fs.hk_stream && fs.hk_stream != fs.stream) HIP_TRY(c, hipStreamWaitEvent(fs.stream, fs.hk_event, 0));
+    const bool ev2_behind_housekeeping = c->n_lanes && c->streaming_submit;
+    struct HousekeepingMark {
+        aic_ctx *c; aic_ctx::FrameSlot &fs;
+        bool ev2_covers = false;
+        ~HousekeepingMark() {
+            if (!c->n_lanes) return;
+            if (ev2_covers) { fs.hk_event = fs.ev2; fs.hk_stream = fs.stream; }
+            else if (hipEventRecord(fs.ev3, fs.stream) == hipSuccess) { fs.hk_event = fs.ev3; fs.hk_stream = fs.stream; }
+            else { (void)hipStreamSynchronize(fs.stream); fs.hk_stream = nullptr; }
+        }
+    } housekeeping_mark{c, fs};
     if (want_aux) {
         if (rb && rb->aux_target) {
             F.aux = rb->aux_target;
@@ -982,6 +1088,9 @@
             }
         }
     }
+#ifndef AIC_PROFILE
+    for (uint32_t j = 0; j < k; j++) *const_cast<volatile unsigned long long *>(&fs.sub[j].host_counters->bailed) = kFramePending;
+#endif
     HIP_TRY(c, hipEventRecord(fs.ev0, fs.stream));
     if (ui) {
         F.pass = 1;
@@ -1042,8 +1151,9 @@
 #ifdef AIC_PROFILE
     for (uint32_t j = 0; j < k; j++) HIP_TRY(c, hipMemcpyAsync(fs.sub[j].host_counters, fs.sub[j].counters.p, sizeof(DevCounters), hipMemcpyDeviceToHost, fs.stream));
 #endif
-    HIP_TRY(c, hipEventRecord(fs.ev2, fs.stream));
+    if (!ev2_behind_housekeeping) HIP_TRY(c, hipEventRecord(fs.ev2, fs.stream));
     fs.busy = true;
+    fs.unfinished = true;
     bool cleared = false;
     if (use_feedback && n_tiles) {
         OrderJobs jobs;
@@ -1077,6 +1187,15 @@
     }
     for (uint32_t j = 0; j < k; j++) fs.sub[j].counters_clean = cleared;
     if (want_aux && !(rb && rb->aux_target)) c->aux_records = npix;
+    if (ev2_behind_housekeeping) {
+        const hipError_t e2 = hipEventRecord(fs.ev2, fs.stream);
+        if (e2 != hipSuccess) {
+            (void)hipStreamSynchronize(fs.stream);
+            fs.busy = fs.unfinished = false;
+            return hip_fail(c, "hipEventRecord(fs.ev2, fs.stream)", e2);
+        }
+        housekeeping_mark.ev2_covers = true;
+    }
     return AIC_OK;
 }
 int submit_frame(aic_ctx *c, const aic_frame_desc *f, uint32_t *out_device, uint32_t slot, bool allow_aux, const double *patches = nullptr,
@@ -1093,6 +1212,7 @@
     const uint32_t k = fs.n_sub ? fs.n_sub : 1u;
     if (fs.busy) {
         fs.busy = false;
+        fs.unfinished = false;
         if (whole_stream || c->sw.wait_whole_stream) HIP_TRY(c, hipStreamSynchronize(fs.stream));
         else HIP_TRY(c, hipEventSynchronize(fs.ev2));
         HIP_TRY(c, hipEventElapsedTime(&kernel_ms, fs.ev0, fs.ev1));
@@ -1357,9 +1477,11 @@
 
 static int ensure_slot(aic_ctx *c, uint32_t slot) {
     aic_ctx::FrameSlot &fs = c->slots[slot];
-    if (fs.stream && fs.ev0 && fs.ev1 && fs.ev2 && fs.sub[0].counters.p) return AIC_OK;
+    if (fs.stream && fs.ev0 && fs.ev1 && fs.ev2 && fs.ev3 && fs.sub[0].counters.p) return AIC_OK;
+    if (!fs.stream && c->n_lanes) fs.stream = c->stream;
     if (!fs.stream) {
         HIP_TRY(c, hipStreamCreateWithFlags(&fs.stream, hipStreamNonBlocking));
+        fs.owns_stream = true;
         hipEvent_t ev = nullptr;
         HIP_TRY(c, hipEventCreateWithFlags(&ev, hipEventDisableTiming));
         hipError_t e1 = hipEventRecord(ev, c->stream);
@@ -1370,6 +1492,7 @@
     if (!fs.ev0) HIP_TRY(c, hipEventCreate(&fs.ev0));
     if (!fs.ev1) HIP_TRY(c, hipEventCreate(&fs.ev1));
     if (!fs.ev2) HIP_TRY(c, hipEventCreate(&fs.ev2));
+    if (!fs.ev3) HIP_TRY(c, hipEventCreateWithFlags(&fs.ev3, hipEventDisableTiming));
     hipError_t e = fs.sub[0].counters.ensure(1);
     if (e != hipSuccess) return hip_fail(c, "alloc frame counters", e);
     return AIC_OK;
@@ -1457,19 +1580,29 @@
     if (!c) return AIC_ERR_INVALID;
     HIP_TRY(c, hipSetDevice(c->device));
     HIP_TRY(c, hipStreamSynchronize(c->stream));
-    for (uint32_t i = 1; i < AIC_MAX_IN_FLIGHT; i++)
-        if (c->slots[i].stream) HIP_TRY(c, hipStreamSynchronize(c->slots[i].stream));
+    for (uint32_t i = 1; i + 1u < kLaneCandidates; i++)
+        if (c->cand[i]) HIP_TRY(c, hipStreamSynchronize(c->cand[i]));
+    for (uint32_t i = 8; i < AIC_MAX_IN_FLIGHT; i++)
+        if (c->slots[i].owns_stream) HIP_TRY(c, hipStreamSynchronize(c->slots[i].stream));
     return AIC_OK;
 }
 
 void *aic_stream(aic_ctx *c) { return c ? (void *)c->stream : nullptr; }
+
+uint32_t aic_stream_lanes(aic_ctx *c) { return c ? c->n_lanes : 0u; }
+
+uint32_t aic_slot_chip_parts(aic_ctx *c, uint32_t slot) { return (c && slot < AIC_MAX_IN_FLIGHT) ? c->slots[slot].share : 0u; }
+
+float aic_lane_probe_ms(aic_ctx *c) { return c ? c->lane_probe_ms : 0.f; }
 
 int aic_wait_event(aic_ctx *c, void *hip_event) {
     if (!c || !hip_event) return fail(c, AIC_ERR_INVALID, "aic_wait_event: bad argument");
     HIP_TRY(c, hipSetDevice(c->device));
     HIP_TRY(c, hipStreamWaitEvent(c->stream, (hipEvent_t)hip_event, 0));
-    for (uint32_t i = 1; i < AIC_MAX_IN_FLIGHT; i++)
-        if (c->slots[i].stream) HIP_TRY(c, hipStreamWaitEvent(c->slots[i].stream, (hipEvent_t)hip_event, 0));
+    for (uint32_t i = 1; i + 1u < kLaneCandidates; i++)
+        if (c->cand[i]) HIP_TRY(c, hipStreamWaitEvent(c->cand[i], (hipEvent_t)hip_event, 0));
+    for (uint32_t i = 8; i < AIC_MAX_IN_FLIGHT; i++)
+        if (c->slots[i].owns_stream) HIP_TRY(c, hipStreamWaitEvent(c->slots[i].stream, (hipEvent_t)hip_event, 0));
     return AIC_OK;
 }
 
diff --git a/all_is_cubes_amd/csrc/aic_ctx.h b/all_is_cubes_amd/csrc/aic_ctx.h
--- a/all_is_cubes_amd/csrc/aic_ctx.h
+++ b/all_is_cubes_amd/csrc/aic_ctx.h
@@ -12,6 +12,7 @@
 
 #include "../../include/aic_hip.h"
 #include "aic_device.h"
+#include "aic_lanes.h"
 
 namespace aic {
 
@@ -97,6 +98,11 @@
     int device = 0;
     hipStream_t stream = nullptr;
     hipStream_t upload_stream = nullptr;
+    hipStream_t cand[kLaneCandidates] = {};
+    hipStream_t lane[kMaxLanes] = {};
+    uint32_t n_lanes = 0;
+    uint32_t lane_cursor = 0;
+    float lane_probe_ms = 0.f;
     Layer layers[2];
     DevBuf<float> lut;
     DevBuf<float> srgb_thr;
@@ -130,6 +136,13 @@
         hipStream_t stream = nullptr;
         hipEvent_t ev0 = nullptr, ev1 = nullptr;
         hipEvent_t ev2 = nullptr;
+        hipEvent_t ev3 = nullptr;
+        hipEvent_t hk_event = nullptr;
+        hipStream_t hk_stream = nullptr;
+        bool owns_stream = false;
+        bool unfinished = false;
+        int32_t lane = -1;
+        uint32_t share = 1;
         SubSlot sub[kMaxSub];
         uint32_t n_sub = 1;
         bool static_ready = false;
@@ -170,6 +183,7 @@
         bool feedback = true;
         bool wait_whole_stream = false;
         uint32_t tiles_per_wave = 0;
+        int stream_lanes = -1;
         std::string wave_prof;
     } sw;
 };
diff --git a/all_is_cubes_amd/csrc/aic_lanes.h b/all_is_cubes_amd/csrc/aic_lanes.h
--- /dev/null
+++ b/all_is_cubes_amd/csrc/aic_lanes.h
@@ -0,0 +1,75 @@
+#pragma once
+
+#include <cstdint>
+
+namespace aic {
+
+constexpr uint32_t kLaneCandidates = 9;
+constexpr uint32_t kMaxLanes = 8;
+constexpr uint32_t kLaneTrials = 2;
+
+struct LaneInterval {
+    uint64_t begin, end;
+};
+
+inline bool lane_intervals_overlap(const LaneInterval &a, const LaneInterval &b) {
+    return a.begin < a.end && b.begin < b.end && a.begin < b.end && b.begin < a.end;
+}
+
+inline uint32_t lane_groups(const LaneInterval *iv, uint32_t trials, uint32_t n, uint32_t *group) {
+    uint32_t n_groups = 0;
+    for (uint32_t i = 0; i < n; i++) {
+        uint32_t g = 0;
+        for (; g < n_groups; g++) {
+            bool apart = false;
+            for (uint32_t j = 0; j < i && !apart; j++) {
+                if (group[j] != g) continue;
+                for (uint32_t t = 0; t < trials && !apart; t++) apart = lane_intervals_overlap(iv[t * n + i], iv[t * n + j]);
+            }
+            if (!apart) break;
+        }
+        group[i] = g;
+        if (g == n_groups) n_groups++;
+    }
+    return n_groups;
+}
+
+inline uint32_t lanes_from_groups(const uint32_t *group, uint32_t n, uint32_t avoid, uint32_t max_lanes, uint32_t *lane) {
+    uint32_t n_lanes = 0;
+    uint32_t shared = n;
+    for (uint32_t i = 0; i < n; i++) {
+        if (i == avoid) continue;
+        bool first = true;
+        for (uint32_t j = 0; j < i && first; j++) first = !(j != avoid && group[j] == group[i]);
+        if (!first) continue;
+        if (avoid < n && group[i] == group[avoid]) { shared = i; continue; }
+        if (n_lanes < max_lanes) lane[n_lanes++] = i;
+    }
+    if (shared < n && n_lanes < max_lanes) lane[n_lanes++] = shared;
+    return n_lanes;
+}
+
+inline uint32_t pick_lane(const uint32_t *unfinished, uint32_t n_lanes, uint32_t *cursor) {
+    if (n_lanes == 0) return 0;
+    uint32_t best = *cursor % n_lanes;
+    for (uint32_t d = 1; d < n_lanes; d++) {
+        const uint32_t l = (*cursor + d) % n_lanes;
+        if (unfinished[l] < unfinished[best]) best = l;
+    }
+    *cursor = (best + 1u) % n_lanes;
+    return best;
+}
+
+inline uint32_t chip_share_divisor(uint32_t unfinished_others, uint32_t n_lanes) {
+    uint32_t d = unfinished_others < 4u ? unfinished_others : 4u;
+    if (d > n_lanes) d = n_lanes;
+    return d ? d : 1u;
+}
+
+inline uint32_t streamed_tiles_per_wave(uint32_t tpw_full, uint32_t unfinished_others, uint32_t n_lanes, uint32_t streamed_default) {
+    if (tpw_full < 4u || unfinished_others == 0u) return streamed_default;
+    const uint32_t t = tpw_full * chip_share_divisor(unfinished_others, n_lanes);
+    return t < 32u ? t : (tpw_full > 32u ? tpw_full : 32u);
+}
+
+}
diff --git a/all_is_cubes_amd/host/aic_host.hpp b/all_is_cubes_amd/host/aic_host.hpp
--- a/all_is_cubes_amd/host/aic_host.hpp
+++ b/all_is_cubes_amd/host/aic_host.hpp
@@ -288,6 +288,7 @@
                                      const std::vector<std::array<double, 16>> &inverse_projection_views = {});
     ImageInfo wait_rows(uint32_t slot);
     void synchronize();
+    uint32_t stream_lanes() const { return aic_stream_lanes(ctx_); }
     Viewport modified_viewport() const;
     const StandardCameras &cameras() const { return *cameras_; }
     std::string device_name() const;
diff --git a/all_is_cubes_amd/host/py_module.cpp b/all_is_cubes_amd/host/py_module.cpp
--- a/all_is_cubes_amd/host/py_module.cpp
+++ b/all_is_cubes_amd/host/py_module.cpp
@@ -258,6 +258,7 @@
         }, py::arg("device_ptrs"), py::arg("strip_rows"), py::arg("n_parts"), py::arg("part"), py::arg("slot"), py::arg("inverse_projection_views") = std::vector<std::array<double, 16>>())
         .def("wait_rows", [](HipRtRenderer &r, uint32_t slot) { py::gil_scoped_release rel; return r.wait_rows(slot); }, py::arg("slot"))
         .def("synchronize", [](HipRtRenderer &r) { py::gil_scoped_release rel; r.synchronize(); })
+        .def("stream_lanes", [](HipRtRenderer &r) { return r.stream_lanes(); })
         .def("assemble_strips", [](HipRtRenderer &r, uintptr_t gathered, uintptr_t out, uint32_t strip_rows, uint32_t n_parts, bool wait) {
             r.assemble_strips(reinterpret_cast<const void *>(gathered), reinterpret_cast<void *>(out), strip_rows, n_parts, wait);
         }, py::arg("gathered"), py::arg("out"), py::arg("strip_rows"), py::arg("n_parts"), py::arg("wait") = true)
diff --git a/include/aic_hip.h b/include/aic_hip.h
--- a/include/aic_hip.h
+++ b/include/aic_hip.h
@@ -173,6 +173,9 @@
 int aic_read_aux(aic_ctx *ctx, aic_pixel_aux *out, uint64_t n_records);
 int aic_synchronize(aic_ctx *ctx);
 void *aic_stream(aic_ctx *ctx);
+uint32_t aic_stream_lanes(aic_ctx *ctx);
+uint32_t aic_slot_chip_parts(aic_ctx *ctx, uint32_t slot);
+float aic_lane_probe_ms(aic_ctx *ctx);
 int aic_wait_event(aic_ctx *ctx, void *hip_event);
 int aic_stream_wait_frame(aic_ctx *ctx, uint32_t slot, void *hip_stream);
 
diff --git a/rust/all-is-cubes-hip/src/ffi.rs b/rust/all-is-cubes-hip/src/ffi.rs
--- a/rust/all-is-cubes-hip/src/ffi.rs
+++ b/rust/all-is-cubes-hip/src/ffi.rs
@@ -217,6 +217,9 @@
     pub fn aic_trace_rays(ctx: *mut aic_ctx, layer: c_int, n: u32, rays: *const f64, flags: u32, exposure: f32, out: *mut c_void, aux: *mut aic_pixel_aux, info: *mut aic_frame_info) -> c_int;
     pub fn aic_read_aux(ctx: *mut aic_ctx, out: *mut aic_pixel_aux, n_records: u64) -> c_int;
     pub fn aic_synchronize(ctx: *mut aic_ctx) -> c_int;
+    pub fn aic_stream_lanes(ctx: *mut aic_ctx) -> u32;
+    pub fn aic_slot_chip_parts(ctx: *mut aic_ctx, slot: u32) -> u32;
+    pub fn aic_lane_probe_ms(ctx: *mut aic_ctx) -> f32;
     pub fn aic_stream(ctx: *mut aic_ctx) -> *mut c_void;
     pub fn aic_wait_event(ctx: *mut aic_ctx, hip_event: *mut c_void) -> c_int;
     pub fn aic_stream_wait_frame(ctx: *mut aic_ctx, slot: u32, hip_stream: *mut c_void) -> c_int;
```
